# OpenBMB/VisRAG

Measured on AMD Instinct MI355X. Metric: page-images embedded/sec (VisRAG-Ret encode, 448x448, bf16 MFMA) + queries/sec@top-10 over 100k-page index, higher is better.
Workload: dtype bf16; 1 GPU; VisRAG-Ret (SigLIP-so400m 26 blk + resampler + MiniCPM-2B 40 layers) bf16 encode batch=32 page images 448x448 per GPU; index 100000 rows x 2304 sharded 1 way(s), 1000 queries top-10; batch_per_gpu=32, global_batch=32, parallelism=dp1 (pages sharded, no data-path collective)

## Files before the change

include/visrag_hip.h:

```cpp
#ifndef VISRAG_HIP_H
#define VISRAG_HIP_H

#include <stddef.h>
#include <stdint.h>

#ifdef __cplusplus
extern "C" {
#endif

#define VR_OK 0
#define VR_ERR_INVALID 1
#define VR_ERR_HIP 2
#define VR_ERR_STATE 3
#define VR_ERR_CAPACITY 4

#define VR_DTYPE_F32 0
#define VR_DTYPE_BF16 1

typedef struct vr_model_s* vr_model_t;
typedef struct vr_index_s* vr_index_t;

typedef struct vr_config {
    int32_t patch_size;
    int32_t vit_dim;
    int32_t vit_depth;
    int32_t vit_heads;
    int32_t vit_hidden;
    int32_t vit_pos_grid;
    float   vit_ln_eps;
    int32_t query_num;
    float   resampler_ln_eps;
    int32_t hidden_size;
    int32_t num_layers;
    int32_t num_heads;
    int32_t intermediate_size;
    int32_t vocab_size;
    float   rms_norm_eps;
    float   rope_theta;
    float   scale_emb;
    float   residual_scale;
    int32_t max_images;
    int32_t max_patches;
    int32_t max_tokens;
    int32_t max_seqs;
    int32_t text_split_precision;
} vr_config_t;

const char* vr_version(void);
const char* vr_last_error(void);
int vr_device_count(int* count);

int vr_model_create(int device_id, const vr_config_t* cfg, vr_model_t* out);
int vr_model_destroy(vr_model_t m);

int vr_model_load_weight(vr_model_t m, const char* name, const void* data,
                         const int64_t* shape, int32_t ndim, int32_t dtype, int32_t on_device);
int vr_model_finalize(vr_model_t m);
int vr_model_clone(vr_model_t src, vr_model_t* out);

int vr_encode(vr_model_t m,
              const uint8_t* const* slices, const int32_t* slice_hw, int32_t n_slices,
              int32_t slices_on_device,
              const int32_t* input_ids, const int32_t* seq_offsets, int32_t B,
              const int32_t* vision_rows,
              float* out_reps, int32_t out_on_device, void* stream);

int vr_encode_hidden(vr_model_t m,
                     const uint8_t* const* slices, const int32_t* slice_hw, int32_t n_slices,
                     int32_t slices_on_device,
                     const int32_t* input_ids, const int32_t* seq_offsets, int32_t B,
                     const int32_t* vision_rows,
                     float* out_reps, int32_t out_on_device,
                     float* out_hidden, int32_t hidden_len, void* stream);

#define VR_POOL_WMEAN 0
#define VR_POOL_MEAN 1
#define VR_POOL_LASTTOKEN 2
#define VR_POOL_CLS 3
int vr_model_set_pooling(vr_model_t m, int32_t mode);

int vr_model_tap(vr_model_t m, const char* name, float* out, int64_t rows, int64_t cols);
int vr_model_set_taps(vr_model_t m, int32_t enable);

#define VR_PROF_VIT_QKV 0
#define VR_PROF_VIT_ATTN 1
#define VR_PROF_VIT_PROJ 2
#define VR_PROF_VIT_FC1 3
#define VR_PROF_VIT_FC2 4
#define VR_PROF_RESAMPLER 5
#define VR_PROF_DECODER 6
#define VR_PROF_DEC_QKV 7
#define VR_PROF_DEC_ATTN 8
#define VR_PROF_DEC_O 9
#define VR_PROF_DEC_GU 10
#define VR_PROF_DEC_DOWN 11
#define VR_PROF_DEC_NORM 12
#define VR_PROF_CLASSES 13
int vr_model_set_profile(vr_model_t m, int32_t enable);
int vr_model_get_profile(vr_model_t m, int32_t cls, double* total_ms, int64_t* launches,
                         double* total_flops);

typedef struct vr_chat_s* vr_chat_t;
typedef struct vr_chat_config {
    int32_t max_len;
    int32_t max_rows;
    float   dim_model_base;
    int32_t max_slots;
    int32_t max_new;
} vr_chat_config_t;
#define VR_CHAT_GREEDY 0
#define VR_CHAT_BEAM 1
#define VR_CHAT_SAMPLE 2
int vr_chat_create(vr_model_t m, const vr_chat_config_t* cfg, vr_chat_t* out);
int vr_chat_destroy(vr_chat_t ch);
int vr_chat_load_head(vr_chat_t ch, const void* data, const int64_t* shape, int32_t ndim, int32_t dtype, int32_t on_device);
int vr_chat_prefill(vr_chat_t ch, int32_t slot, int32_t row, const uint8_t* const* slices, const int32_t* slice_hw,
                    int32_t n_slices, int32_t slices_on_device, const int32_t* input_ids, int32_t T,
                    const int32_t* vision_rows, void* stream);
int vr_chat_prefill_batch(vr_chat_t ch, int32_t B, const int32_t* slots, const int32_t* rows, const uint8_t* const* slices,
                          const int32_t* slice_hw, int32_t n_slices, int32_t slices_on_device, const int32_t* input_ids,
                          const int32_t* seq_offsets, const int32_t* vision_rows, void* stream);
int vr_chat_step(vr_chat_t ch, int32_t n, const int32_t* slots, const int32_t* rows, const int32_t* tokens, void* stream);
int vr_chat_select(vr_chat_t ch, int32_t mode, int32_t n_groups, const int32_t* group_offsets, const int32_t* rows,
                   const float* beam_scores, int32_t k, float repetition_penalty, float temperature, int32_t top_k,
                   uint64_t seed, int32_t step, float* out_scores, int32_t* out_tokens, int32_t* out_parents, void* stream);
int vr_chat_sample(vr_chat_t ch, int32_t n, const int32_t* rows, float repetition_penalty, float temperature, int32_t top_k,
                   double top_p, uint64_t seed, int32_t step, float* out_scores, int32_t* out_tokens, int32_t* out_kept,
                   int32_t* out_cut, void* stream);
int vr_chat_reorder(vr_chat_t ch, int32_t n, const int32_t* rows, const int32_t* parents, void* stream);
int vr_chat_logits(vr_chat_t ch, int32_t row, float* out, void* stream);
int vr_chat_row_len(vr_chat_t ch, int32_t row, int32_t* slot, int32_t* generated);

int vr_index_create(int device_id, int32_t dim, int64_t capacity, vr_index_t* out);
int vr_index_destroy(vr_index_t ix);
int vr_index_reset(vr_index_t ix);
int vr_index_add(vr_index_t ix, const float* reps, int64_t n, int32_t on_device, void* stream);
int vr_index_size(vr_index_t ix, int64_t* n);
int vr_index_search(vr_index_t ix, const float* queries, int32_t nq, int32_t k,
                    float* out_scores, int64_t* out_ids, int32_t on_device, void* stream);
int vr_index_set_search_eps(vr_index_t ix, float eps_rel);
int vr_index_error_model(vr_index_t ix, float* out4);
int vr_index_search_stats(vr_index_t ix, int64_t* out6, int32_t reset);
int vr_index_search_plan(vr_index_t ix, int32_t nq, int32_t* out5);
int vr_index_set_search_profile(vr_index_t ix, int32_t enable);
int vr_index_get_search_profile(vr_index_t ix, double* ms5, int64_t* calls);
int vr_index_search_keys(vr_index_t ix, const float* queries, int32_t nq, int32_t k, int64_t id_offset,
                         uint64_t* out_keys, int32_t on_device, void* stream);
int vr_index_set_groups(vr_index_t ix, const int64_t* group_offsets, int64_t n_groups);
int vr_index_search_groups(vr_index_t ix, const float* queries, int32_t nq, int32_t k,
                           float* out_scores, int64_t* out_ids, int64_t* out_groups,
                           int32_t on_device, void* stream);
int vr_index_group_search_stats(vr_index_t ix, int64_t* out3, int32_t reset);
int vr_index_set_filters(vr_index_t ix, const uint32_t* bits, int32_t n_filters, int32_t on_device, void* stream);
int vr_index_search_filtered(vr_index_t ix, const float* queries, int32_t nq, int32_t k,
                             const int32_t* filter_of_query,
                             float* out_scores, int64_t* out_ids, int32_t on_device, void* stream);
int vr_index_filter_search_stats(vr_index_t ix, int64_t* out3, int32_t reset);
int vr_index_search_diverse(vr_index_t ix, const float* queries, int32_t nq, int32_t k, int32_t pool, float lambda,
                            const int32_t* filter_of_query ,
                            float* out_scores, int64_t* out_ids, int32_t on_device, void* stream);
int vr_index_search_range(vr_index_t ix, const float* queries, int32_t nq,
                          const float* thresholds,
                          const int32_t* filter_of_query,
                          int64_t max_total,
                          int64_t* out_lims,
                          int64_t* total,
                          int32_t on_device, void* stream);
int vr_index_range_results(vr_index_t ix, float* out_scores, int64_t* out_ids, int64_t n,
                           int32_t on_device, void* stream);
int vr_index_range_search_stats(vr_index_t ix, int64_t* out3, int32_t reset);
int vr_index_rank_rows(vr_index_t ix, const float* queries, int32_t nq,
                       const int64_t* lims,
                       const int64_t* ids,
                       const int32_t* filter_of_query,
                       float* out_scores, int64_t* out_ranks,
                       int32_t on_device, void* stream);
int vr_index_count_range(vr_index_t ix, const float* queries, int32_t nq,
                         const int64_t* lims,
                         const float* thresholds,
                         int32_t strict,
                         const int32_t* filter_of_query,
                         int64_t* out_counts,
                         int32_t on_device, void* stream);
int vr_index_rank_search_stats(vr_index_t ix, int64_t* out3, int32_t reset);
int vr_index_search_window(vr_index_t ix, const float* queries, int32_t nq,
                           const int64_t* offsets,
                           int32_t k,
                           const int32_t* filter_of_query,
                           float* out_scores, int64_t* out_ids,
                           int32_t on_device, void* stream);
int vr_index_window_search_stats(vr_index_t ix, int64_t* out3, int32_t reset);
int vr_index_search_groups_window(vr_index_t ix, const float* queries, int32_t nq,
                                  const int64_t* offsets,
                                  int32_t k,
                                  const int32_t* filter_of_query,
                                  float* out_scores, int64_t* out_ids, int64_t* out_groups,
                                  int32_t on_device, void* stream);
int vr_index_group_window_search_stats(vr_index_t ix, int64_t* out3, int32_t reset);
int vr_index_rank_groups(vr_index_t ix, const float* queries, int32_t nq,
                         const int64_t* lims,
                         const int64_t* groups,
                         const int32_t* filter_of_query,
                         float* out_scores, int64_t* out_rows, int64_t* out_ranks,
                         int32_t on_device, void* stream);
int vr_index_count_groups_range(vr_index_t ix, const float* queries, int32_t nq,
                                const int64_t* lims,
                                const float* thresholds,
                                int32_t strict,
                                const int32_t* filter_of_query,
                                int64_t* out_counts,
                                int32_t on_device, void* stream);
int vr_index_group_rank_search_stats(vr_index_t ix, int64_t* out3, int32_t reset);
int vr_index_search_groups_range(vr_index_t ix, const float* queries, int32_t nq,
                                 const float* thresholds,
                                 const int32_t* filter_of_query,
                                 int64_t max_total,
                                 int64_t* out_lims,
                                 int64_t* total,
                                 int32_t on_device, void* stream);
int vr_index_group_range_results(vr_index_t ix, float* out_scores, int64_t* out_rows, int64_t* out_groups, int64_t n,
                                 int32_t on_device, void* stream);
int vr_index_group_range_search_stats(vr_index_t ix, int64_t* out3, int32_t reset);
int vr_index_search_multi(vr_index_t ix, const float* queries, int32_t n_sub,
                          const int64_t* lims,
                          int32_t n_groups, int32_t k,
                          int32_t fuse,
                          const int32_t* filter_of_group,
                          float* out_scores, int64_t* out_ids, int32_t* out_which,
                          int32_t on_device, void* stream);
int vr_index_multi_search_stats(vr_index_t ix, int64_t* out3, int32_t reset);
int vr_index_search_multi_groups(vr_index_t ix, const float* queries, int32_t n_sub,
                                 const int64_t* lims,
                                 int32_t n_groups, int32_t k,
                                 int32_t fuse,
                                 const int32_t* filter_of_group,
                                 float* out_scores, int64_t* out_rows, int64_t* out_docs, int32_t* out_which,
                                 float* out_ev_scores, int64_t* out_ev_rows,
                                 int32_t on_device, void* stream);
int vr_index_multi_group_search_stats(vr_index_t ix, int64_t* out3, int32_t reset);
int vr_rrf_fuse(int device_id, const int64_t* ids, int32_t n_lists, int32_t depth,
                const int64_t* lims,
                int32_t n_groups, int32_t k, float c,
                const float* weights,
                float* out_scores, int64_t* out_ids, int32_t* out_hits,
                int32_t on_device, void* stream);
int vr_rrf_max_entries(void);
int vr_index_search_rrf(vr_index_t ix, const float* queries, int32_t n_sub,
                        const int64_t* lims,
                        int32_t n_groups, int32_t k, int32_t depth, float c,
                        const float* weights,
                        const int32_t* filter_of_group,
                        int32_t by_groups,
                        float* out_scores, int64_t* out_ids, int32_t* out_hits,
                        int32_t on_device, void* stream);
int vr_index_rrf_search_stats(vr_index_t ix, int64_t* out3, int32_t reset);
int vr_index_remove(vr_index_t ix, const int64_t* ids, int64_t n, int64_t* removed, void* stream);
int vr_index_update(vr_index_t ix, const int64_t* ids, const float* reps, int64_t n, int32_t on_device, void* stream);
int vr_index_get_rows(vr_index_t ix, const int64_t* ids, int64_t n, float* out_f32, uint16_t* out_bf16, int32_t on_device,
                      void* stream);
int vr_topk_merge(int device_id, const float* scores, const int64_t* ids, int32_t n_parts,
                  int32_t nq, int32_t k, float* out_scores, int64_t* out_ids, void* stream);
int vr_topk_merge_keys(int device_id, const uint64_t* keys, int32_t n_parts, int32_t nq, int32_t k,
                       float* out_scores, int64_t* out_ids, void* stream);

int vr_synth_pages(int device_id, uint8_t* out, int32_t n, int32_t size, int64_t seed, int64_t first, void* stream);

int vr_streams_overlap(int device_id, void* stream_a, void* stream_b, int32_t* overlap);

int vr_resize_bicubic(int device_id, const uint8_t* src, int32_t src_on_device, int32_t H, int32_t W,
                      uint8_t* dst, int32_t out_h, int32_t out_w, void* stream);

int vr_op_gemm(int device_id, const void* A, int32_t lda, const void* W, int32_t ldw,
               int32_t M, int32_t N, int32_t K, int32_t epilogue, const float* bias,
               const float* resid, float alpha, void* out, int32_t ldo,
               const int32_t* rope_pos, const float* rope_table, int32_t rope_cols,
               int32_t variant, void* stream);
typedef struct vr_gemm_extras {
    const int32_t* rowmap;
    const float* rowbias;
    int32_t rowbias_period, rowbias_ld, rowbias_cols;
    float col_scale;
    int32_t col_scale_n;
    int32_t ksplit;
    int64_t split_stride;
    const int32_t* m_dev;
    int32_t m_sub;
    int32_t raster_gm;
} vr_gemm_extras_t;
int vr_op_gemm_ex(int device_id, const void* A, int32_t lda, const void* W, int32_t ldw,
                  int32_t M, int32_t N, int32_t K, int32_t epilogue, const float* bias,
                  const float* resid, float alpha, void* out, int32_t ldo,
                  const int32_t* rope_pos, const float* rope_table, int32_t rope_cols,
                  int32_t variant, const vr_gemm_extras_t* extras, void* stream);
int vr_op_gemm_warm(int device_id, const void* A, int32_t lda, const void* W, int32_t ldw,
                    int32_t M, int32_t N, int32_t K, int32_t epilogue, const float* bias,
                    const float* resid, float alpha, void* out, int32_t ldo,
                    const int32_t* rope_pos, const float* rope_table, int32_t rope_cols,
                    int32_t variant, const vr_gemm_extras_t* extras, const void* warm, uint64_t warm_bytes, void* stream);
int vr_op_norm(int device_id, int32_t kind, const float* x, int32_t rows, int32_t dim,
               const float* weight, const float* bias, float eps, void* out, int32_t ldo,
               void* stream);
int vr_op_norm_ex(int device_id, int32_t kind, const float* x, int32_t rows, int32_t dim, int32_t ldx, const float* weight,
                  const float* bias, float eps, void* out, int32_t ldo, void* stream);

int vr_op_text_rmsnorm_split(int device_id, const float* x, int32_t rows, int32_t dim, const float* weight, float eps, void* hi,
                             void* lo, void* stream);
int vr_op_text_rope(int device_id, float* qkv, int32_t T, int32_t ld, int32_t rope_cols, const int32_t* pos, const float* table,
                    void* stream);
int vr_op_text_attention(int device_id, const float* qkv, int32_t ld, int32_t E, const int32_t* seq_offsets, int32_t B, int32_t T,
                         int32_t heads, float scale, float* out, void* stream);
int vr_op_text_swiglu_split(int device_id, const float* gu, int32_t T, int32_t ld_gu, int32_t I, int32_t ld_act, void* hi, void* lo,
                            void* stream);
int vr_op_embed_gather(int device_id, const int32_t* ids, int32_t T, const void* table, const void* table_lo, int32_t dim,
                       float scale, float* out, void* stream);
int vr_op_pool(int device_id, const float* h, const int32_t* seq_offsets, int32_t B, int32_t dim, const float* norm_w, float eps,
               float* out, float* tap, int32_t mode, void* stream);
int vr_op_convert(int device_id, int32_t kind, const void* in, void* out, void* out2, int64_t n, int64_t n_total, int32_t* aux,
                  void* stream);
int vr_op_planes_sum(int device_id, const float* parts, int32_t n_parts, int64_t stride, int32_t ldp, int32_t T, int32_t N,
                     float* out, int32_t ldo, float alpha, int32_t accumulate, void* stream);
int vr_op_patch_embed(int device_id, const void* const* imgs, int32_t n, int32_t H, int32_t W, int32_t P, const float* weight,
                      int32_t D, int32_t K, const float* bias, const float* pos, int32_t ld_pos, float* out, int32_t ldo,
                      void* stream);
int vr_op_attention(int device_id, const void* q, int32_t ldq, const void* k, int32_t ldk,
                    const void* v, int32_t ldv, void* out, int32_t ldo,
                    const int32_t* cu_q, const int32_t* cu_kv, int32_t B, int32_t heads,
                    int32_t head_dim, int32_t max_q, int32_t causal, int32_t q_shared,
                    float scale, void* stream);
typedef struct vr_attn_extras {
    int32_t kv_group;
    const int32_t* kv_end;
    const int32_t* q_in_rows;
    int32_t q_head_stride;
    int32_t q_prescaled;
    float* lse;
} vr_attn_extras_t;
int vr_op_attention_ex(int device_id, const void* q, int32_t ldq, const void* k, int32_t ldk,
                       const void* v, int32_t ldv, void* out, int32_t ldo,
                       const int32_t* cu_q, const int32_t* cu_kv, int32_t B, int32_t heads,
                       int32_t head_dim, int32_t max_q, int32_t causal, int32_t q_shared,
                       float scale, const vr_attn_extras_t* extras, void* stream);
#define VR_ATTN_ROUTE_REFUSED (-1)
#define VR_ATTN_ROUTE_NONE 0
#define VR_ATTN_ROUTE_SMALL 1
#define VR_ATTN_ROUTE_72W 2
#define VR_ATTN_ROUTE_TILED(head_dim, qf, pipe) (100000 + (head_dim) * 100 + (qf) * 10 + (pipe))
int vr_op_attention_route(int device_id, const void* q, int32_t ldq, const void* k, int32_t ldk,
                          const void* v, int32_t ldv, void* out, int32_t ldo,
                          const int32_t* cu_q, const int32_t* cu_kv, int32_t B, int32_t heads,
                          int32_t head_dim, int32_t max_q, int32_t causal, int32_t q_shared,
                          float scale, const vr_attn_extras_t* extras);
int vr_op_attn_combine(int device_id, const void* part, const float* lse, int32_t S, const int32_t* S_dev, int32_t heads,
                       int32_t group, int32_t n_rows, void* out, int32_t ld_out, const void* W, int32_t ldw, int32_t M,
                       int32_t N, int32_t K, int32_t ksplit, int32_t planes, int32_t ldo, int64_t split_stride, void* stream);
int vr_op_gemm_skinny(int device_id, const void* A, int32_t lda, const void* W, int32_t ldw, int32_t M, int32_t N,
                      int32_t K, int32_t ksplit, const float* bias, int32_t swiglu, void* out, int32_t ldo,
                      int64_t split_stride, void* stream);
int vr_op_plane_sum(int device_id, int32_t kind, const float* parts, int32_t nsplit, int64_t split_stride, int32_t ldp,
                    int32_t rows, int32_t dim, float* x, int32_t ldx, float alpha, const float* weight, float eps,
                    void* out, int32_t ldo, void* stream);
int vr_op_chat_attention(int device_id, const void* q, const void* prompt, const void* tails, int32_t layers, int32_t l,
                         int32_t E, int32_t slots, int32_t max_len, int32_t rows, int32_t max_new, int32_t n,
                         const int32_t* step_row, const int32_t* step_slot, const int32_t* step_tail,
                         const int32_t* slot_plen, int32_t force_splits, void* att, void* stream);
int vr_op_chat_select(int device_id, int32_t mode, const float* logits, int32_t ld, int32_t V, const uint32_t* seen,
                      int32_t words, int32_t n_groups, const int32_t* group_offsets, const float* beam_scores, int32_t K,
                      int32_t kout, float repetition_penalty, float temperature, uint64_t seed, int32_t step,
                      float* out_scores, int32_t* out_tokens, int32_t* out_parents, void* stream);
int vr_op_chat_sample(int device_id, const float* logits, int32_t ld, int32_t V, const uint32_t* seen, int32_t words, int32_t n,
                      float repetition_penalty, float temperature, int32_t top_k, double top_p, uint64_t seed, int32_t step,
                      float* out_scores, int32_t* out_tokens, int32_t* out_kept, int32_t* out_cut, void* stream);
int vr_op_chat_prompt_scatter(int device_id, const void* qkv, int32_t ld, int32_t E, int32_t B, const int32_t* seq_offsets,
                              const int32_t* slots, int32_t n_slots, int32_t max_len, void* kplane, void* vplane, void* stream);

int vr_op_gen_mrope_cache(int device_id, const void* src_bf16, const float* parts, int32_t n_parts, int64_t plane_stride,
                          const float* bias, int32_t ld, int32_t T, int32_t H, int32_t KV, const int32_t* pos3, int32_t pos_stride,
                          int32_t sec_t, int32_t sec_h, const float* inv_freq, void* q_out, int32_t ldq, void* k_cache, void* v_cache,
                          int32_t ld_cache, int32_t cache_row0, const int32_t* row0_dev, const int32_t* cache_rows, int32_t* cu_kv,
                          void* stream);
int vr_op_gen_rope2d(int device_id, void* qkv, int32_t ld, int32_t T, int32_t n_slots, int32_t hh, const int32_t* pos_h,
                     const int32_t* pos_w, int32_t sec_h, const float* freq, void* stream);
int vr_op_gen_sample(int device_id, const float* logits, int32_t vocab, uint32_t* seen, float repetition_penalty, float temperature,
                     uint64_t seed, int32_t step, int32_t* state, int32_t step_from_state, int32_t advance, int32_t* out_token,
                     void* stream);
int vr_op_gen_mark_seen(int device_id, const int32_t* ids, int32_t n, uint32_t* seen, int32_t vocab, void* stream);
int vr_op_gen_decode_begin(int device_id, int32_t* state, int32_t q_rows, void* stream);
int vr_op_gen_rows(int device_id, int32_t kind, const float* src, const int32_t* row_idx, int32_t n, int32_t dim, void* dst,
                   int32_t ld, const void* const* pages, const int32_t* page_w, int32_t n_pages, const int32_t* img, const int32_t* ph,
                   const int32_t* pw, int32_t P, int32_t tp, const float* mean3, const float* std3, void* stream);

#ifdef __cplusplus
}
#endif
#endif
```

visrag_amd/_lib.py:

```python
from __future__ import annotations

import ctypes as C
import os
from typing import Optional

_HERE = os.path.dirname(os.path.abspath(__file__))
LIB_PATH = os.path.join(_HERE, "libvisrag_hip.so")

VR_DTYPE_F32, VR_DTYPE_BF16 = 0, 1


class VRConfig(C.Structure):
    _fields_ = [
        ("patch_size", C.c_int32), ("vit_dim", C.c_int32), ("vit_depth", C.c_int32),
        ("vit_heads", C.c_int32), ("vit_hidden", C.c_int32), ("vit_pos_grid", C.c_int32),
        ("vit_ln_eps", C.c_float), ("query_num", C.c_int32), ("resampler_ln_eps", C.c_float),
        ("hidden_size", C.c_int32), ("num_layers", C.c_int32), ("num_heads", C.c_int32),
        ("intermediate_size", C.c_int32), ("vocab_size", C.c_int32), ("rms_norm_eps", C.c_float),
        ("rope_theta", C.c_float), ("scale_emb", C.c_float), ("residual_scale", C.c_float),
        ("max_images", C.c_int32), ("max_patches", C.c_int32), ("max_tokens", C.c_int32),
        ("max_seqs", C.c_int32), ("text_split_precision", C.c_int32),
    ]


class VRChatConfig(C.Structure):
    _fields_ = [("max_len", C.c_int32), ("max_rows", C.c_int32), ("dim_model_base", C.c_float), ("max_slots", C.c_int32),
                ("max_new", C.c_int32)]


class VGConfig(C.Structure):
    _fields_ = [
        ("hidden_size", C.c_int32), ("num_layers", C.c_int32), ("num_heads", C.c_int32), ("num_kv_heads", C.c_int32),
        ("intermediate_size", C.c_int32), ("vocab_size", C.c_int32), ("max_len", C.c_int32), ("max_prefill", C.c_int32),
        ("rms_norm_eps", C.c_float), ("rope_theta", C.c_float), ("mrope_section", C.c_int32 * 3), ("max_seqs", C.c_int32),
    ]


class VGVisionConfig(C.Structure):
    _fields_ = [
        ("depth", C.c_int32), ("hidden_size", C.c_int32), ("num_heads", C.c_int32), ("intermediate_size", C.c_int32),
        ("out_hidden_size", C.c_int32), ("in_channels", C.c_int32), ("patch_size", C.c_int32), ("temporal_patch_size", C.c_int32),
        ("spatial_merge_size", C.c_int32), ("window_size", C.c_int32), ("n_fullatt", C.c_int32), ("fullatt_blocks", C.c_int32 * 16),
        ("max_rows", C.c_int32), ("rms_norm_eps", C.c_float),
    ]


class VRGemmExtras(C.Structure):
    _fields_ = [("rowmap", C.c_void_p), ("rowbias", C.c_void_p), ("rowbias_period", C.c_int32), ("rowbias_ld", C.c_int32),
                ("rowbias_cols", C.c_int32), ("col_scale", C.c_float), ("col_scale_n", C.c_int32), ("ksplit", C.c_int32),
                ("split_stride", C.c_int64), ("m_dev", C.c_void_p), ("m_sub", C.c_int32), ("raster_gm", C.c_int32)]


class VRAttnExtras(C.Structure):
    _fields_ = [("kv_group", C.c_int32), ("kv_end", C.c_void_p), ("q_in_rows", C.c_void_p), ("q_head_stride", C.c_int32),
                ("q_prescaled", C.c_int32), ("lse", C.c_void_p)]


class VisragHipError(RuntimeError):
    pass


_lib: Optional[C.CDLL] = None

_vp, _i32, _i64, _f32 = C.c_void_p, C.c_int32, C.c_int64, C.c_float
SIGNATURES = {
    "vr_version": (C.c_char_p, []),
    "vr_last_error": (C.c_char_p, []),
    "vr_device_count": (C.c_int, [C.POINTER(C.c_int)]),
    "vr_model_create": (C.c_int, [C.c_int, C.POINTER(VRConfig), C.POINTER(_vp)]),
    "vr_model_destroy": (C.c_int, [_vp]),
    "vr_model_load_weight": (C.c_int, [_vp, C.c_char_p, _vp, C.POINTER(_i64), _i32, _i32, _i32]),
    "vr_model_finalize": (C.c_int, [_vp]),
    "vr_model_clone": (C.c_int, [_vp, C.POINTER(C.c_void_p)]),
    "vr_encode": (C.c_int, [_vp, C.POINTER(_vp), C.POINTER(_i32), _i32, _i32, C.POINTER(_i32),
                            C.POINTER(_i32), _i32, C.POINTER(_i32), _vp, _i32, _vp]),
    "vr_encode_hidden": (C.c_int, [_vp, C.POINTER(_vp), C.POINTER(_i32), _i32, _i32, C.POINTER(_i32),
                                   C.POINTER(_i32), _i32, C.POINTER(_i32), _vp, _i32, _vp, _i32, _vp]),
    "vr_model_tap": (C.c_int, [_vp, C.c_char_p, _vp, _i64, _i64]),
    "vr_model_set_taps": (C.c_int, [_vp, _i32]),
    "vr_model_set_pooling": (C.c_int, [_vp, _i32]),
    "vr_model_set_profile": (C.c_int, [_vp, _i32]),
    "vr_model_get_profile": (C.c_int, [_vp, _i32, C.POINTER(C.c_double), C.POINTER(_i64), C.POINTER(C.c_double)]),
    "vr_index_create": (C.c_int, [C.c_int, _i32, _i64, C.POINTER(_vp)]),
    "vr_index_destroy": (C.c_int, [_vp]),
    "vr_index_reset": (C.c_int, [_vp]),
    "vr_index_add": (C.c_int, [_vp, _vp, _i64, _i32, _vp]),
    "vr_index_size": (C.c_int, [_vp, C.POINTER(_i64)]),
    "vr_index_search": (C.c_int, [_vp, _vp, _i32, _i32, _vp, _vp, _i32, _vp]),
    "vr_topk_merge": (C.c_int, [C.c_int, _vp, _vp, _i32, _i32, _i32, _vp, _vp, _vp]),
    "vr_index_set_search_eps": (C.c_int, [_vp, _f32]),
    "vr_index_search_stats": (C.c_int, [_vp, C.POINTER(_i64), _i32]),
    "vr_index_error_model": (C.c_int, [_vp, C.POINTER(_f32)]),
    "vr_index_search_plan": (C.c_int, [_vp, _i32, C.POINTER(_i32)]),
    "vr_synth_pages": (C.c_int, [C.c_int, _vp, _i32, _i32, _i64, _i64, _vp]),
    "vr_streams_overlap": (C.c_int, [C.c_int, _vp, _vp, C.POINTER(C.c_int32)]),
    "vr_index_set_search_profile": (C.c_int, [_vp, _i32]),
    "vr_index_get_search_profile": (C.c_int, [_vp, C.POINTER(C.c_double), C.POINTER(_i64)]),
    "vr_index_search_keys": (C.c_int, [_vp, _vp, _i32, _i32, _i64, _vp, _i32, _vp]),
    "vr_index_set_groups": (C.c_int, [_vp, C.POINTER(_i64), _i64]),
    "vr_index_search_groups": (C.c_int, [_vp, _vp, _i32, _i32, _vp, _vp, _vp, _i32, _vp]),
    "vr_index_group_search_stats": (C.c_int, [_vp, C.POINTER(_i64), _i32]),
    "vr_index_set_filters": (C.c_int, [_vp, _vp, _i32, _i32, _vp]),
    "vr_index_search_filtered": (C.c_int, [_vp, _vp, _i32, _i32, _vp, _vp, _vp, _i32, _vp]),
    "vr_index_filter_search_stats": (C.c_int, [_vp, C.POINTER(_i64), _i32]),
    "vr_index_search_range": (C.c_int, [_vp, _vp, _i32, _vp, _vp, _i64, _vp, C.POINTER(_i64), _i32, _vp]),
    "vr_index_range_results": (C.c_int, [_vp, _vp, _vp, _i64, _i32, _vp]),
    "vr_index_range_search_stats": (C.c_int, [_vp, C.POINTER(_i64), _i32]),
    "vr_index_rank_rows": (C.c_int, [_vp, _vp, _i32, _vp, _vp, _vp, _vp, _vp, _i32, _vp]),
    "vr_index_count_range": (C.c_int, [_vp, _vp, _i32, _vp, _vp, _i32, _vp, _vp, _i32, _vp]),
    "vr_index_rank_search_stats": (C.c_int, [_vp, C.POINTER(_i64), _i32]),
    "vr_index_search_window": (C.c_int, [_vp, _vp, _i32, _vp, _i32, _vp, _vp, _vp, _i32, _vp]),
    "vr_index_window_search_stats": (C.c_int, [_vp, C.POINTER(_i64), _i32]),
    "vr_index_search_groups_window": (C.c_int, [_vp, _vp, _i32, _vp, _i32, _vp, _vp, _vp, _vp, _i32, _vp]),
    "vr_index_group_window_search_stats": (C.c_int, [_vp, C.POINTER(_i64), _i32]),
    "vr_index_rank_groups": (C.c_int, [_vp, _vp, _i32, _vp, _vp, _vp, _vp, _vp, _vp, _i32, _vp]),
    "vr_index_count_groups_range": (C.c_int, [_vp, _vp, _i32, _vp, _vp, _i32, _vp, _vp, _i32, _vp]),
    "vr_index_group_rank_search_stats": (C.c_int, [_vp, C.POINTER(_i64), _i32]),
    "vr_index_search_groups_range": (C.c_int, [_vp, _vp, _i32, _vp, _vp, _i64, _vp, C.POINTER(_i64), _i32, _vp]),
    "vr_index_group_range_results": (C.c_int, [_vp, _vp, _vp, _vp, _i64, _i32, _vp]),
    "vr_index_group_range_search_stats": (C.c_int, [_vp, C.POINTER(_i64), _i32]),
    "vr_index_search_multi": (C.c_int, [_vp, _vp, _i32, _vp, _i32, _i32, _i32, _vp, _vp, _vp, _vp, _i32, _vp]),
    "vr_index_multi_search_stats": (C.c_int, [_vp, C.POINTER(_i64), _i32]),
    "vr_index_search_multi_groups": (C.c_int, [_vp, _vp, _i32, _vp, _i32, _i32, _i32, _vp, _vp, _vp, _vp, _vp, _vp, _vp, _i32, _vp]),
    "vr_index_multi_group_search_stats": (C.c_int, [_vp, C.POINTER(_i64), _i32]),
    "vr_rrf_fuse": (C.c_int, [C.c_int, _vp, _i32, _i32, _vp, _i32, _i32, _f32, _vp, _vp, _vp, _vp, _i32, _vp]),
    "vr_rrf_max_entries": (C.c_int, []),
    "vr_index_search_rrf": (C.c_int, [_vp, _vp, _i32, _vp, _i32, _i32, _i32, _f32, _vp, _vp, _i32, _vp, _vp, _vp, _i32, _vp]),
    "vr_index_rrf_search_stats": (C.c_int, [_vp, C.POINTER(_i64), _i32]),
    "vr_index_search_diverse": (C.c_int, [_vp, _vp, _i32, _i32, _i32, _f32, _vp, _vp, _vp, _i32, _vp]),
    "vr_index_remove": (C.c_int, [_vp, C.POINTER(_i64), _i64, C.POINTER(_i64), _vp]),
    "vr_index_update": (C.c_int, [_vp, C.POINTER(_i64), _vp, _i64, _i32, _vp]),
    "vr_index_get_rows": (C.c_int, [_vp, C.POINTER(_i64), _i64, _vp, _vp, _i32, _vp]),
    "vr_topk_merge_keys": (C.c_int, [C.c_int, _vp, _i32, _i32, _i32, _vp, _vp, _vp]),
    "vr_resize_bicubic": (C.c_int, [C.c_int, _vp, _i32, _i32, _i32, _vp, _i32, _i32, _vp]),
    "vr_op_gemm": (C.c_int, [C.c_int, _vp, _i32, _vp, _i32, _i32, _i32, _i32, _i32, _vp, _vp, _f32,
                             _vp, _i32, _vp, _vp, _i32, _i32, _vp]),
    "vr_op_gemm_ex": (C.c_int, [C.c_int, _vp, _i32, _vp, _i32, _i32, _i32, _i32, _i32, _vp, _vp, _f32,
                                _vp, _i32, _vp, _vp, _i32, _i32, C.POINTER(VRGemmExtras), _vp]),
    "vr_op_gemm_warm": (C.c_int, [C.c_int, _vp, _i32, _vp, _i32, _i32, _i32, _i32, _i32, _vp, _vp, _f32,
                                  _vp, _i32, _vp, _vp, _i32, _i32, C.POINTER(VRGemmExtras), _vp, C.c_uint64, _vp]),
    "vr_op_norm": (C.c_int, [C.c_int, _i32, _vp, _i32, _i32, _vp, _vp, _f32, _vp, _i32, _vp]),
    "vr_op_norm_ex": (C.c_int, [C.c_int, _i32, _vp, _i32, _i32, _i32, _vp, _vp, _f32, _vp, _i32, _vp]),
    "vr_op_text_rmsnorm_split": (C.c_int, [C.c_int, _vp, _i32, _i32, _vp, _f32, _vp, _vp, _vp]),
    "vr_op_text_rope": (C.c_int, [C.c_int, _vp, _i32, _i32, _i32, _vp, _vp, _vp]),
    "vr_op_text_attention": (C.c_int, [C.c_int, _vp, _i32, _i32, _vp, _i32, _i32, _i32, _f32, _vp, _vp]),
    "vr_op_text_swiglu_split": (C.c_int, [C.c_int, _vp, _i32, _i32, _i32, _i32, _vp, _vp, _vp]),
    "vr_op_embed_gather": (C.c_int, [C.c_int, _vp, _i32, _vp, _vp, _i32, _f32, _vp, _vp]),
    "vr_op_pool": (C.c_int, [C.c_int, _vp, _vp, _i32, _i32, _vp, _f32, _vp, _vp, _i32, _vp]),
    "vr_op_convert": (C.c_int, [C.c_int, _i32, _vp, _vp, _vp, _i64, _i64, _vp, _vp]),
    "vr_op_planes_sum": (C.c_int, [C.c_int, _vp, _i32, _i64, _i32, _i32, _i32, _vp, _i32, _f32, _i32, _vp]),
    "vr_op_patch_embed": (C.c_int, [C.c_int, C.POINTER(_vp), _i32, _i32, _i32, _i32, _vp, _i32, _i32, _vp, _vp, _i32, _vp, _i32, _vp]),
    "vr_op_attention": (C.c_int, [C.c_int, _vp, _i32, _vp, _i32, _vp, _i32, _vp, _i32, _vp, _vp, _i32,
                                  _i32, _i32, _i32, _i32, _i32, _f32, _vp]),
    "vr_op_attention_ex": (C.c_int, [C.c_int, _vp, _i32, _vp, _i32, _vp, _i32, _vp, _i32, _vp, _vp, _i32,
                                     _i32, _i32, _i32, _i32, _i32, _f32, C.POINTER(VRAttnExtras), _vp]),
    "vr_op_attention_route": (C.c_int, [C.c_int, _vp, _i32, _vp, _i32, _vp, _i32, _vp, _i32, _vp, _vp, _i32,
                                        _i32, _i32, _i32, _i32, _i32, _f32, C.POINTER(VRAttnExtras)]),
    "vr_op_attn_combine": (C.c_int, [C.c_int, _vp, _vp, _i32, _vp, _i32, _i32, _i32, _vp, _i32, _vp, _i32, _i32, _i32, _i32, _i32,
                                     _i32, _i32, _i64, _vp]),
    "vr_op_gemm_skinny": (C.c_int, [C.c_int, _vp, _i32, _vp, _i32, _i32, _i32, _i32, _i32, _vp, _i32, _vp, _i32, _i64, _vp]),
    "vr_op_plane_sum": (C.c_int, [C.c_int, _i32, _vp, _i32, _i64, _i32, _i32, _i32, _vp, _i32, _f32, _vp, _f32, _vp, _i32, _vp]),
    "vr_op_chat_attention": (C.c_int, [C.c_int, _vp, _vp, _vp, _i32, _i32, _i32, _i32, _i32, _i32, _i32, _i32, C.POINTER(_i32),
                                       C.POINTER(_i32), C.POINTER(_i32), C.POINTER(_i32), _i32, _vp, _vp]),
    "vr_op_chat_select": (C.c_int, [C.c_int, _i32, _vp, _i32, _i32, _vp, _i32, _i32, C.POINTER(_i32), C.POINTER(_f32), _i32, _i32,
                                    _f32, _f32, C.c_uint64, _i32, C.POINTER(_f32), C.POINTER(_i32), C.POINTER(_i32), _vp]),
    "vr_op_chat_sample": (C.c_int, [C.c_int, _vp, _i32, _i32, _vp, _i32, _i32, _f32, _f32, _i32, C.c_double, C.c_uint64, _i32,
                                    C.POINTER(_f32), C.POINTER(_i32), C.POINTER(_i32), C.POINTER(_i32), _vp]),
    "vr_op_chat_prompt_scatter": (C.c_int, [C.c_int, _vp, _i32, _i32, _i32, C.POINTER(_i32), C.POINTER(_i32), _i32, _i32, _vp, _vp, _vp]),
    "vr_op_gen_mrope_cache": (C.c_int, [C.c_int, _vp, _vp, _i32, _i64, _vp, _i32, _i32, _i32, _i32, _vp, _i32, _i32, _i32, _vp, _vp, _i32,
                                        _vp, _vp, _i32, _i32, _vp, _vp, _vp, _vp]),
    "vr_op_gen_rope2d": (C.c_int, [C.c_int, _vp, _i32, _i32, _i32, _i32, _vp, _vp, _i32, _vp, _vp]),
    "vr_op_gen_sample": (C.c_int, [C.c_int, _vp, _i32, _vp, _f32, _f32, C.c_uint64, _i32, _vp, _i32, _i32, C.POINTER(_i32), _vp]),
    "vr_op_gen_mark_seen": (C.c_int, [C.c_int, _vp, _i32, _vp, _i32, _vp]),
    "vr_op_gen_decode_begin": (C.c_int, [C.c_int, _vp, _i32, _vp]),
    "vr_op_gen_rows": (C.c_int, [C.c_int, _i32, _vp, _vp, _i32, _i32, _vp, _i32, C.POINTER(_vp), C.POINTER(_i32), _i32, _vp, _vp, _vp,
                                 _i32, _i32, C.POINTER(_f32), C.POINTER(_f32), _vp]),
    "vr_chat_create": (C.c_int, [_vp, C.POINTER(VRChatConfig), C.POINTER(_vp)]),
    "vr_chat_destroy": (C.c_int, [_vp]),
    "vr_chat_load_head": (C.c_int, [_vp, _vp, C.POINTER(_i64), _i32, _i32, _i32]),
    "vr_chat_prefill": (C.c_int, [_vp, _i32, _i32, C.POINTER(_vp), C.POINTER(_i32), _i32, _i32, C.POINTER(_i32), _i32,
                                  C.POINTER(_i32), _vp]),
    "vr_chat_prefill_batch": (C.c_int, [_vp, _i32, C.POINTER(_i32), C.POINTER(_i32), C.POINTER(_vp), C.POINTER(_i32), _i32, _i32,
                                        C.POINTER(_i32), C.POINTER(_i32), C.POINTER(_i32), _vp]),
    "vr_chat_step": (C.c_int, [_vp, _i32, C.POINTER(_i32), C.POINTER(_i32), C.POINTER(_i32), _vp]),
    "vr_chat_select": (C.c_int, [_vp, _i32, _i32, C.POINTER(_i32), C.POINTER(_i32), C.POINTER(_f32), _i32, _f32, _f32, _i32,
                                 C.c_uint64, _i32, C.POINTER(_f32), C.POINTER(_i32), C.POINTER(_i32), _vp]),
    "vr_chat_sample": (C.c_int, [_vp, _i32, C.POINTER(_i32), _f32, _f32, _i32, C.c_double, C.c_uint64, _i32, C.POINTER(_f32),
                                 C.POINTER(_i32), C.POINTER(_i32), C.POINTER(_i32), _vp]),
    "vr_chat_reorder": (C.c_int, [_vp, _i32, C.POINTER(_i32), C.POINTER(_i32), _vp]),
    "vr_chat_logits": (C.c_int, [_vp, _i32, _vp, _vp]),
    "vr_chat_row_len": (C.c_int, [_vp, _i32, C.POINTER(_i32), C.POINTER(_i32)]),
}
GEN_SIGNATURES = {
    "vg_create": (C.c_int, [C.c_int, C.POINTER(VGConfig), C.POINTER(_vp)]),
    "vg_destroy": (C.c_int, [_vp]),
    "vg_load_weight": (C.c_int, [_vp, C.c_char_p, _vp, C.POINTER(_i64), _i32, _i32, _i32]),
    "vg_finalize": (C.c_int, [_vp]),
    "vg_prefill": (C.c_int, [_vp, _vp, _i32, _vp, _vp, _i32, _vp, _vp]),
    "vg_sample": (C.c_int, [_vp, _f32, _f32, C.c_uint64, _i32, C.POINTER(_i32), _vp]),
    "vg_decode": (C.c_int, [_vp, _i32, C.POINTER(_i32), _vp]),
    "vg_logits": (C.c_int, [_vp, _vp, _vp]),
    "vg_select": (C.c_int, [_vp, _i32]),
    "vg_decode_batch": (C.c_int, [_vp, _i32, C.POINTER(_i32), C.POINTER(_i32), C.POINTER(_i32), _vp]),
    "vg_sample_batch": (C.c_int, [_vp, _i32, C.POINTER(_i32), _f32, _f32, C.c_uint64, _i32, C.POINTER(_i32), _vp]),
    "vg_cache_len": (C.c_int, [_vp, C.POINTER(_i32)]),
    "vg_run_begin": (C.c_int, [_vp, _i32, _f32, _f32, C.c_uint64, _i32, _vp]),
    "vg_run_step": (C.c_int, [_vp]),
    "vg_run_token": (C.c_int, [_vp, _i32, C.POINTER(_i32)]),
    "vg_run_end": (C.c_int, [_vp]),
    "vg_vision_create": (C.c_int, [_vp, C.POINTER(VGVisionConfig)]),
    "vg_vision_encode": (C.c_int, [_vp, _vp, _vp, _i32, _vp, _vp]),
    "vg_vision_encode_pages": (C.c_int, [_vp, C.POINTER(_vp), _i32, C.POINTER(_f32), C.POINTER(_f32), _vp, _i32, _vp, _vp]),
    "vg_vision_plan": (C.c_int, [C.POINTER(VGVisionConfig), _vp, _i32, _vp, _vp, C.POINTER(_i32), _vp]),
}


def load(path: Optional[str] = None) -> C.CDLL:
    global _lib
    if _lib is not None and path is None:
        return _lib
    p = path or os.environ.get("VISRAG_HIP_LIB") or LIB_PATH
    if not os.path.exists(p):
        raise VisragHipError(
            f"{p} not found: the HIP extension is not built. Run `python -m visrag_amd.build` "
            "(or __graft_entry__.build()); there is no CPU fallback.")
    import torch
    lib = C.CDLL(p)
    for name, (res, args) in list(SIGNATURES.items()) + list(GEN_SIGNATURES.items()):
        fn = getattr(lib, name)
        fn.restype = res
        fn.argtypes = args
    if path is None:
        _lib = lib
    return lib


def check(status: int, what: str = "") -> None:
    if status != 0:
        msg = load().vr_last_error()
        raise VisragHipError(f"{what or 'visrag_hip'} failed (status {status}): "
                             f"{msg.decode() if msg else '?'}")


def make_config(cfg, max_images: int, max_patches: int, max_tokens: int, max_seqs: int) -> VRConfig:
    return VRConfig(
        patch_size=cfg.patch_size, vit_dim=cfg.vit_dim, vit_depth=cfg.vit_depth, vit_heads=cfg.vit_heads,
        vit_hidden=cfg.vit_hidden, vit_pos_grid=cfg.vit_pos_grid, vit_ln_eps=cfg.vit_ln_eps,
        query_num=cfg.query_num, resampler_ln_eps=cfg.resampler_ln_eps, hidden_size=cfg.hidden_size,
        num_layers=cfg.num_layers, num_heads=cfg.num_heads, intermediate_size=cfg.intermediate_size,
        vocab_size=cfg.vocab_size, rms_norm_eps=cfg.rms_norm_eps, rope_theta=cfg.rope_theta,
        scale_emb=cfg.scale_emb, residual_scale=cfg.residual_scale, max_images=max_images,
        max_patches=max_patches, max_tokens=max_tokens, max_seqs=max_seqs,
        text_split_precision=int(getattr(cfg, "text_split_precision", True)))
```

visrag_amd/config.py:

```python
from dataclasses import dataclass, asdict
import math


@dataclass
class VisRAGRetConfig:
    patch_size: int = 14
    vit_dim: int = 1152
    vit_depth: int = 26
    vit_heads: int = 16
    vit_mlp_ratio: float = 3.7362
    vit_pos_grid: int = 27
    vit_ln_eps: float = 1e-6
    query_num: int = 64
    resampler_ln_eps: float = 1e-6
    hidden_size: int = 2304
    num_layers: int = 40
    num_heads: int = 36
    intermediate_size: int = 5760
    vocab_size: int = 122753
    rms_norm_eps: float = 1e-5
    rope_theta: float = 10000.0
    scale_emb: float = 12.0
    scale_depth: float = 1.4
    scale_resolution: int = 448
    max_slice_nums: int = 9
    slice_mode: bool = True
    text_split_precision: int = True
    pooling: str = "wmean"

    @property
    def vit_head_dim(self) -> int:
        return self.vit_dim // self.vit_heads

    @property
    def vit_hidden(self) -> int:
        return int(self.vit_dim * self.vit_mlp_ratio)

    @property
    def resampler_heads(self) -> int:
        return self.hidden_size // 128

    @property
    def head_dim(self) -> int:
        return self.hidden_size // self.num_heads

    @property
    def residual_scale(self) -> float:
        return self.scale_depth / math.sqrt(self.num_layers)

    def to_dict(self):
        return asdict(self)

    def flops_vit(self, n_patches: int) -> float:
        N, D, F = n_patches, self.vit_dim, self.vit_hidden
        pe = 2.0 * N * (3 * self.patch_size ** 2) * D
        blk = 2.0 * N * D * 3 * D + 4.0 * N * N * D + 2.0 * N * D * D + 4.0 * N * D * F
        return pe + self.vit_depth * blk

    def flops_resampler(self, n_patches: int) -> float:
        N, D, E, Q = n_patches, self.vit_dim, self.hidden_size, self.query_num
        return 2.0 * N * D * E + 4.0 * N * E * E + 6.0 * Q * E * E + 4.0 * Q * N * E

    def flops_decoder(self, L: int) -> float:
        E, I = self.hidden_size, self.intermediate_size
        return self.num_layers * (L * (8.0 * E * E + 6.0 * E * I) + 4.0 * L * L * E)

    def flops_page(self, n_patches: int = 1024, L: int = 68) -> float:
        return self.flops_vit(n_patches) + self.flops_resampler(n_patches) + self.flops_decoder(L)


def full_config() -> VisRAGRetConfig:
    return VisRAGRetConfig()


def tiny_config() -> VisRAGRetConfig:
    return VisRAGRetConfig(
        vit_dim=288, vit_depth=2, vit_heads=4, vit_pos_grid=6,
        hidden_size=256, num_layers=2, num_heads=4, intermediate_size=640,
        vocab_size=1000, scale_resolution=112,
    )
```

visrag_amd/csrc/attention.hip:

```cpp
#include "attention_body.h"

namespace vr {

template <int HD, int QF, int PIPE>
__global__ __launch_bounds__(256, QF >= 4 ? 1 : (PIPE == 3 ? 3 : 2)) void attention_kernel(AttnArgs p) {
    __shared__ __attribute__((aligned(16))) char smem[attn_smem_bytes<HD, PIPE>()];
    const int q_tiles = (p.max_q + 64 * QF - 1) / (64 * QF);
    attention_body<HD, QF, PIPE>(p, xcd_remap(blockIdx.x, p.B * p.heads * q_tiles), smem);
}

template <int HD, int QF, int PIPE>
static hipError_t launch_t(const AttnArgs& a, hipStream_t s) {
    const int q_tiles = (a.max_q + 64 * QF - 1) / (64 * QF);
    hipLaunchKernelGGL((attention_kernel<HD, QF, PIPE>), dim3(a.B * a.heads * q_tiles), dim3(256), 0, s, a);
    return hipGetLastError();
}

bool attention_small_ok(const AttnArgs& a);
hipError_t launch_attention_small(const AttnArgs& a, hipStream_t s);
bool attention72w_ok(const AttnArgs& a);
hipError_t launch_attention72w(const AttnArgs& a, hipStream_t s);

AttnRoute attention_route(const AttnArgs& a) {
    if (a.B <= 0 || a.max_q <= 0) return {ATTN_ROUTE_NONE, 0, 0, 0};
    if ((a.ldq | a.ldk | a.ldv) % 8 || a.ldo % 4) return {ATTN_ROUTE_REFUSED, 0, 0, 0};
    if (attention_small_ok(a)) return {ATTN_ROUTE_SMALL, 64, 0, 0};
    if (attention72w_ok(a)) return {ATTN_ROUTE_72W, 72, 0, 0};
    const bool big = a.max_q > 64;
    const bool tiny = a.max_q <= 128;
    switch (a.head_dim) {
        case 64: case 72: case 80:
            if (tiny) return {ATTN_ROUTE_TILED, a.head_dim, big ? 2 : 1, 0};
            return {ATTN_ROUTE_TILED, a.head_dim, 2, 3};
        case 128: return {ATTN_ROUTE_TILED, 128, 1, 0};
        default:  return {ATTN_ROUTE_REFUSED, 0, 0, 0};
    }
}

hipError_t launch_attention(const AttnArgs& a_in, hipStream_t s) {
    const AttnRoute r = attention_route(a_in);
    if (r.kind == ATTN_ROUTE_NONE) return hipSuccess;
    if (r.kind == ATTN_ROUTE_REFUSED) return hipErrorInvalidValue;
    AttnArgs a = a_in;
    if (a.q_prescaled && r.kind != ATTN_ROUTE_72W) a.scale = 1.0f / 1.44269504088896340736f;
    if (r.kind == ATTN_ROUTE_SMALL) return launch_attention_small(a, s);
    if (r.kind == ATTN_ROUTE_72W) return launch_attention72w(a, s);
#define VR_TILED(HD_, QF_, PIPE_) \
    if (r.head_dim == HD_ && r.qf == QF_ && r.pipe == PIPE_) return launch_t<HD_, QF_, PIPE_>(a, s);
    VR_TILED(64, 1, 0) VR_TILED(64, 2, 0) VR_TILED(64, 2, 3)
    VR_TILED(72, 1, 0) VR_TILED(72, 2, 0) VR_TILED(72, 2, 3)
    VR_TILED(80, 1, 0) VR_TILED(80, 2, 0) VR_TILED(80, 2, 3)
    VR_TILED(128, 1, 0)
#undef VR_TILED
    return hipErrorInvalidValue;
}

}
```

visrag_amd/csrc/attention_w.hip:

```cpp
#include <type_traits>

#include "common.h"
#include "kernels.h"

namespace vr {

#define AW_FOR_EACH_ACC(X) \
    X(0, "a[0:3]", "a0", "a1", "a2", "a3") \
    X(1, "a[4:7]", "a4", "a5", "a6", "a7") \
    X(2, "a[8:11]", "a8", "a9", "a10", "a11") \
    X(3, "a[12:15]", "a12", "a13", "a14", "a15") \
    X(4, "a[16:19]", "a16", "a17", "a18", "a19") \
    X(5, "a[20:23]", "a20", "a21", "a22", "a23") \
    X(6, "a[24:27]", "a24", "a25", "a26", "a27") \
    X(7, "a[28:31]", "a28", "a29", "a30", "a31") \
    X(8, "a[32:35]", "a32", "a33", "a34", "a35") \
    X(9, "a[36:39]", "a36", "a37", "a38", "a39") \
    X(10, "a[40:43]", "a40", "a41", "a42", "a43") \
    X(11, "a[44:47]", "a44", "a45", "a46", "a47") \
    X(12, "a[48:51]", "a48", "a49", "a50", "a51") \
    X(13, "a[52:55]", "a52", "a53", "a54", "a55") \
    X(14, "a[56:59]", "a56", "a57", "a58", "a59") \
    X(15, "a[60:63]", "a60", "a61", "a62", "a63") \
    X(16, "a[64:67]", "a64", "a65", "a66", "a67") \
    X(17, "a[68:71]", "a68", "a69", "a70", "a71") \
    X(18, "a[72:75]", "a72", "a73", "a74", "a75") \
    X(19, "a[76:79]", "a76", "a77", "a78", "a79")

namespace {

typedef short s16x4 __attribute__((ext_vector_type(4)));

constexpr int AW_HD = 72, AW_PITCH = 160, AW_KV = 64, AW_QT = 256, AW_DF = 5;
constexpr int AW_SLOT = AW_KV * AW_PITCH;
constexpr int AW_NSLOT = 6;
constexpr int AW_VRING = AW_NSLOT * AW_SLOT;
constexpr int AW_SMEM = 2 * AW_NSLOT * AW_SLOT;
constexpr int AW_OPITCH = 144;
constexpr int AW_SMEM_ALL = AW_SMEM + AW_QT * AW_OPITCH;
constexpr int AW_NPIECE = AW_SLOT / 1024;
#ifndef AW_DBG
#define AW_DBG 0
#endif
constexpr float AW_SLACK = 8.0f;

template <int I, int N, class F>
__device__ __forceinline__ void static_for(F&& f) {
    if constexpr (I < N) {
        f(std::integral_constant<int, I>{});
        static_for<I + 1, N>(f);
    }
}

__device__ __forceinline__ void aw_mfma32_first(f32x4& d, const u32x4& a, const bf16x8& b, const f32x4& c) {
    asm volatile("v_mfma_f32_16x16x32_bf16 %0, %1, %2, %3" : "=&v"(d) : "v"(a), "v"(b), "v"(c));
}
__device__ __forceinline__ void aw_mfma32_acc(f32x4& d, const u32x4& a, const bf16x8& b) {
    asm volatile("v_mfma_f32_16x16x32_bf16 %0, %1, %2, %0" : "+v"(d) : "v"(a), "v"(b));
}
__device__ __forceinline__ void aw_mfma16_acc(f32x4& d, const u32x2& a, const s16x4& b) {
    asm volatile("v_mfma_f32_16x16x16_bf16 %0, %1, %2, %0" : "+v"(d) : "v"(a), "v"(b));
}

__device__ __forceinline__ float aw_exp2(float x) { asm volatile("v_exp_f32 %0, %0" : "+v"(x)); return x; }
__device__ __forceinline__ unsigned aw_cvt_pk(float lo, float hi) {
    unsigned r;
    asm volatile("v_cvt_pk_bf16_f32 %0, %1, %2" : "=v"(r) : "v"(lo), "v"(hi));
    return r;
}
__device__ __forceinline__ void aw_max3(float& m, float a, float b, float c) { asm volatile("v_max3_f32 %0, %1, %2, %3" : "=v"(m) : "v"(a), "v"(b), "v"(c)); }
__device__ __forceinline__ void aw_max2(float& m, float a, float b) { asm volatile("v_max_f32 %0, %1, %2" : "=v"(m) : "v"(a), "v"(b)); }

__device__ __forceinline__ float aw_sub_inplace(float x, float d) { asm volatile("v_sub_f32 %0, %0, %1" : "+v"(x) : "v"(d)); return x; }
__device__ __forceinline__ float aw_mask_inplace(float x, int key, int kv_len) {
    asm volatile("v_cmp_le_i32 vcc, %2, %1\n\tv_cndmask_b32 %0, %0, %3, vcc" : "+v"(x) : "v"(key), "s"(kv_len), "v"(-INFINITY) : "vcc");
    return x;
}
__device__ __forceinline__ unsigned aw_scale_pk_inplace(unsigned w, float alpha) {
    unsigned t;
    asm volatile("v_lshlrev_b32 %1, 16, %0\n\tv_and_b32 %0, 0xffff0000, %0\n\tv_mul_f32 %1, %1, %2\n\tv_mul_f32 %0, %0, %2\n\t"
                 "v_cvt_pk_bf16_f32 %0, %1, %0" : "+v"(w), "=&v"(t) : "v"(alpha));
    return w;
}

template <int N>
__device__ __forceinline__ void aw_pv_mfma(const bf16x8& va, const u32x4& pb) {
#define AW_X(n, R, C0, C1, C2, C3) \
    if constexpr (N == n) asm volatile("v_mfma_f32_16x16x32_bf16 " R ", %0, %1, " R : : "v"(va), "v"(pb) : C0, C1, C2, C3);
    AW_FOR_EACH_ACC(AW_X)
#undef AW_X
}
template <int N>
__device__ __forceinline__ void aw_acc_zero() {
#define AW_X(n, R, C0, C1, C2, C3) \
    if constexpr (N == n) asm volatile("v_accvgpr_write_b32 " C0 ", 0\n\tv_accvgpr_write_b32 " C1 ", 0\n\tv_accvgpr_write_b32 " C2 \
                                       ", 0\n\tv_accvgpr_write_b32 " C3 ", 0" : : : C0, C1, C2, C3);
    AW_FOR_EACH_ACC(AW_X)
#undef AW_X
}
template <int N>
__device__ __forceinline__ void aw_acc_read(f32x4& v) {
#define AW_X(n, R, C0, C1, C2, C3) \
    if constexpr (N == n) asm volatile("v_accvgpr_read_b32 %0, " C0 "\n\tv_accvgpr_read_b32 %1, " C1 "\n\tv_accvgpr_read_b32 %2, " C2 \
                                       "\n\tv_accvgpr_read_b32 %3, " C3 : "=v"(v[0]), "=v"(v[1]), "=v"(v[2]), "=v"(v[3]));
    AW_FOR_EACH_ACC(AW_X)
#undef AW_X
}
template <int N>
__device__ __forceinline__ void aw_acc_write(const f32x4& v) {
#define AW_X(n, R, C0, C1, C2, C3) \
    if constexpr (N == n) asm volatile("v_accvgpr_write_b32 " C0 ", %0\n\tv_accvgpr_write_b32 " C1 ", %1\n\tv_accvgpr_write_b32 " C2 \
                                       ", %2\n\tv_accvgpr_write_b32 " C3 ", %3" : : "v"(v[0]), "v"(v[1]), "v"(v[2]), "v"(v[3]) : C0, C1, C2, C3);
    AW_FOR_EACH_ACC(AW_X)
#undef AW_X
}

__device__ __forceinline__ float aw_col4_max(float v) {
    const auto a = __builtin_amdgcn_permlane16_swap(__float_as_uint(v), __float_as_uint(v), false, false);
    v = fmaxf(__uint_as_float(a[0]), __uint_as_float(a[1]));
    const auto b = __builtin_amdgcn_permlane32_swap(__float_as_uint(v), __float_as_uint(v), false, false);
    return fmaxf(__uint_as_float(b[0]), __uint_as_float(b[1]));
}

#define AW_DS_B128(dst, addr, off) asm volatile("ds_read_b128 %0, %1 offset:%2" : "=v"(dst) : "v"(addr), "i"(off))
#define AW_DS_B64(dst, addr, off) asm volatile("ds_read_b64 %0, %1 offset:%2" : "=v"(dst) : "v"(addr), "i"(off))
#define AW_DS_TR(dst, addr, off) asm volatile("ds_read_b64_tr_b16 %0, %1 offset:%2" : "=v"(dst) : "v"(addr), "i"(off))

}

template <int NF, int NW>
__device__ __forceinline__ void attention72w_body(const AttnArgs& p) {
    static_assert(NF * NW == 16 && (NF == 2 || NF == 4), "256 query rows per workgroup");
    constexpr int NS = 11 * NF;
    constexpr int S_TAIL = 4 * NF, S_PV = 6 * NF;
    constexpr int PW = (2 * AW_NPIECE + NW - 1) / NW;
    constexpr int NV = 8 * NF;
    constexpr int S_CHECK = NF == 4 ? S_PV + 3 : S_PV + 2, S_KREAD = NF == 4 ? S_PV + 7 : S_PV + 3;
    static_assert(S_CHECK + NV / 2 <= NS && S_KREAD + 6 <= NS, "schedule fits");
    extern __shared__ __attribute__((aligned(16))) char smem[];
    const int tid = threadIdx.x, lane = tid & 63;
    const int wave = __builtin_amdgcn_readfirstlane(tid >> 6);
    const int fr = lane & 15, fq = lane >> 4;

    const int q_tiles = (p.max_q + AW_QT - 1) / AW_QT;
    const int total = p.B * p.heads * q_tiles;
    const int nwg = gridDim.x;
    const int lw = xcd_remap(blockIdx.x, nwg);
    const float sc = p.scale * 1.44269504088896340736f;
    const unsigned tile_step = (unsigned)(AW_KV * p.ldk) * 2u;
    const unsigned vdelta = (unsigned)((const char*)p.v - (const char*)p.k);

    struct Unit { int u, ok, h, qs, q_len, kv_len, q_row0, kv0, T; };
    auto get_unit = [&](int u) -> Unit {
        Unit x{u, 0, 0, 0, 0, 0, 0, 0, 0};
        if (u >= total) return x;
        const int qt = u % q_tiles, bh = u / q_tiles, b = bh / p.heads;
        x.h = bh % p.heads;
        x.kv0 = p.cu_kv[b]; x.kv_len = p.cu_kv[b + 1] - x.kv0;
        x.q_row0 = p.cu_q[b]; x.q_len = p.cu_q[b + 1] - x.q_row0;
        x.qs = qt * AW_QT;
        x.T = (x.kv_len + AW_KV - 1) / AW_KV;
        x.ok = x.qs < x.q_len && x.kv_len > 0;
        return x;
    };
    auto next_valid = [&](int u) -> Unit {
        Unit x = get_unit(u);
        while (!x.ok && u < total) { u += nwg; x = get_unit(u); }
        return x;
    };
    auto unit_rsrc = [&](const Unit& x) {
        const bf16_t* kb = (const bf16_t*)p.k + (size_t)x.kv0 * p.ldk + x.h * AW_HD;
        return __builtin_amdgcn_make_buffer_rsrc((void*)kb, 0, x.ok ? vdelta + ((x.kv_len - 1) * p.ldv + AW_HD) * 2 : 0, 0x00020000);
    };

    Unit cur = next_valid(lw);
    if (!cur.ok) return;

    unsigned doff[PW];
    int dbase[PW];
    auto doff_reset = [&]() {
#pragma unroll
        for (int i = 0; i < PW; ++i) {
            int j = wave + NW * i;
            if (j >= 2 * AW_NPIECE) j -= 2 * AW_NPIECE;
            const int isv = j >= AW_NPIECE;
            const int c = (j - isv * AW_NPIECE) * 64 + lane;
            const int row = c / 10, ch = c % 10;
            doff[i] = (unsigned)(row * p.ldk + ch * 8) * 2u + (isv ? vdelta : 0u);
            dbase[i] = __builtin_amdgcn_readfirstlane(isv * AW_VRING + (j - isv * AW_NPIECE) * 1024);
        }
    };
    auto ldrsrc = unit_rsrc(cur);
    auto dma_piece = [&](int i, int slot_off) {
        __builtin_amdgcn_raw_ptr_buffer_load_lds(ldrsrc, VR_LDS(smem + dbase[i] + slot_off), 16, doff[i], 0, 0, 0);
        doff[i] += tile_step;
    };
    constexpr int P_LEAD = (PW + 1) / 2;
    int slot_ld = 0;

    u32x4 qraw[NF][2];
    u32x2 qtraw[NF];
    auto q_load = [&](const Unit& x) {
        const bf16_t* qbase = (const bf16_t*)p.q + (size_t)x.q_row0 * p.ldq + x.h * AW_HD;
#pragma unroll
        for (int f = 0; f < NF; ++f) {
            const int q = x.qs + (wave * NF + f) * 16 + fr;
            const bool ok = x.ok && q < x.q_len && !(AW_DBG & 128);
#pragma unroll
            for (int ks = 0; ks < 2; ++ks) {
                qraw[f][ks] = u32x4{0, 0, 0, 0};
                if (ok) qraw[f][ks] = *reinterpret_cast<const u32x4*>(qbase + (size_t)q * p.ldq + ks * 32 + fq * 8);
            }
            qtraw[f] = u32x2{0, 0};
            if (ok && 64 + fq * 4 < AW_HD) qtraw[f] = *reinterpret_cast<const u32x2*>(qbase + (size_t)q * p.ldq + 64 + fq * 4);
        }
    };
    bf16x8 qf[NF][2];
    s16x4 qtail[NF];
    auto q_scale = [&]() {
        if (p.q_prescaled) {
#pragma unroll
            for (int f = 0; f < NF; ++f) {
                qf[f][0] = __builtin_bit_cast(bf16x8, qraw[f][0]); qf[f][1] = __builtin_bit_cast(bf16x8, qraw[f][1]);
                qtail[f] = __builtin_bit_cast(s16x4, qtraw[f]);
            }
            return;
        }
#pragma unroll
        for (int f = 0; f < NF; ++f) {
#pragma unroll
            for (int ks = 0; ks < 2; ++ks) {
                const bf16x8 v = __builtin_bit_cast(bf16x8, qraw[f][ks]);
#pragma unroll
                for (int e = 0; e < 8; ++e) qf[f][ks][e] = f2bf(bf2f(v[e]) * sc);
            }
            const bf16x4 t4 = __builtin_bit_cast(bf16x4, qtraw[f]);
            bf16x4 t;
#pragma unroll
            for (int e = 0; e < 4; ++e) t[e] = f2bf(bf2f(t4[e]) * sc);
            qtail[f] = __builtin_bit_cast(s16x4, t);
        }
    };

    f32x4 negm4[NF];
    f32x4 sA[NF][2], sB[NF][2];
    u32x4 pbA[NF], pbB[NF];

    const unsigned lds0 = (unsigned)(uintptr_t)(__attribute__((address_space(3))) char*)VR_LDS(smem);
    const unsigned k_lane = lds0 + (unsigned)(fr * AW_PITCH + fq * 16);
    const unsigned kt_lane = lds0 + (unsigned)(fr * AW_PITCH + 128 + fq * 8);
    const unsigned v_lane = lds0 + (unsigned)(AW_VRING + (fq * 4 + (fr >> 2)) * AW_PITCH + (fr & 3) * 8);
    const bool row8 = fr == 8;
    int kv_len = cur.kv_len;

#ifdef AW_TIMING
    unsigned long long tm_start = __builtin_amdgcn_s_memtime(), tm_wait = 0, tm_loop0 = 0, tm_loop1 = 0;
    unsigned long long* tmrec = (unsigned long long*)p.lse + ((size_t)cur.u * NW + wave) * 64;
    int tm_nb = 0;
#endif
    u32x4 ka[2][2];
    u32x2 kt[2];
    u32x2 vlo[AW_DF], vhi[AW_DF];
    float mxall = 0.f, mxb = 0.f;

    auto k_read = [&](auto u_c, auto hf_c, unsigned ka_addr, unsigned kta_addr) {
        (void)&ka; (void)&kt;
        constexpr int u = decltype(u_c)::value, hf = decltype(hf_c)::value;
        constexpr int kf = u / 3, pc = u % 3, row = (hf * 2 + kf) * 16 * AW_PITCH;
        if constexpr (pc == 0) AW_DS_B128(ka[kf][0], ka_addr, row);
        else if constexpr (pc == 1) AW_DS_B128(ka[kf][1], ka_addr, row + 64);
        else AW_DS_B64(kt[kf], kta_addr, row);
    };
    auto k_wait = [&]() {
        asm volatile("s_waitcnt lgkmcnt(0)" : "+v"(ka[0][0]), "+v"(ka[0][1]), "+v"(ka[1][0]), "+v"(ka[1][1]), "+v"(kt[0]), "+v"(kt[1]));
    };
    auto v_read = [&](auto u_c, auto hf_c, unsigned v_addr) {
        (void)&vlo; (void)&vhi;
        constexpr int u = decltype(u_c)::value, hf = decltype(hf_c)::value;
        constexpr int d = u / 2, off = hf * 32 * AW_PITCH + d * 32;
        if constexpr ((u & 1) == 0) AW_DS_TR(vlo[d], v_addr, off);
        else AW_DS_TR(vhi[d], v_addr, off + 16 * AW_PITCH);
    };
    auto v_wait = [&]() {
        asm volatile("s_waitcnt lgkmcnt(0)" : "+v"(vlo[0]), "+v"(vhi[0]), "+v"(vlo[1]), "+v"(vhi[1]), "+v"(vlo[2]), "+v"(vhi[2]),
                     "+v"(vlo[3]), "+v"(vhi[3]), "+v"(vlo[4]), "+v"(vhi[4]));
    };

    auto mask_half = [&](f32x4 (&s)[NF][2], int hh) {
        float mx = -INFINITY;
#pragma unroll
        for (int f = 0; f < NF; ++f)
#pragma unroll
            for (int kf = 0; kf < 2; ++kf)
#pragma unroll
                for (int r = 0; r < 4; ++r) {
                    s[f][kf][r] = aw_mask_inplace(s[f][kf][r], hh * 32 + kf * 16 + fq * 4 + r, kv_len);
                    mx = fmaxf(mx, s[f][kf][r]);
                }
        mxall = mx;
    };

    auto raise = [&](f32x4 (&s)[NF][2], u32x4 (&pbn)[NF], auto force_c) {
        constexpr bool force = decltype(force_c)::value;
        if constexpr (!force) asm volatile("s_nop 15\n\ts_nop 15\n\ts_nop 15" ::: "memory");
#pragma unroll
        for (int f = 0; f < NF; ++f) {
            float mx = fmaxf(fmaxf(fmaxf(s[f][0][0], s[f][0][1]), fmaxf(s[f][0][2], s[f][0][3])),
                             fmaxf(fmaxf(s[f][1][0], s[f][1][1]), fmaxf(s[f][1][2], s[f][1][3])));
            mx = aw_col4_max(mx);
// ... 334 lines not shown
```

visrag_amd/csrc/encode.hip:

```cpp
#include <hip/hip_runtime.h>

#include <algorithm>
#include <cmath>
#include <cstring>
#include <vector>

#include "model.h"

static int run_vision_group(vr_model_s* m, const uint8_t* const* dev_imgs_hostarray, int n, int H, int W,
                            const int32_t* rowmap_host , bool first_group, hipStream_t s) {
    const vr_config_t& c = m->c;
    const int P = c.patch_size, gh = H / P, gw = W / P, N = gh * gw;
    const int D = m->D, Dp = m->Dp, E = m->E, Q = m->Q;
    const int M = n * N;
    GridTables* g = nullptr;
    VRCHK(get_grid(m, gh, gw, &g));

    HIPCHK(hipMemcpyAsync(m->w_imgptr.p, dev_imgs_hostarray, (size_t)n * 8, hipMemcpyHostToDevice, s));
    int* cu = (int*)arena_take(m, (size_t)2 * (n + 1) * 4);
    for (int i = 0; i <= n; ++i) { cu[i] = i * N; cu[n + 1 + i] = i * Q; }
    HIPCHK(hipMemcpyAsync(m->w_cu.p, cu, (size_t)2 * (n + 1) * 4, hipMemcpyHostToDevice, s));
    HIPCHK(hipMemcpyAsync(m->w_rowmap.p, rowmap_host, (size_t)n * Q * 4, hipMemcpyHostToDevice, s));
    const int* cu_tok = m->w_cu.as<int>();
    const int* cu_qry = m->w_cu.as<int>() + (n + 1);

    float* h = m->w_hvit.as<float>();
    {
        GemmArgs a = gemm_args(nullptr, 0, m->patch, M, h, Dp);
        a.rowbias = g->vit_pos.as<float>(); a.rowbias_period = N; a.rowbias_ld = Dp; a.rowbias_cols = Dp;
        HIPCHK(launch_patch_embed((const uint8_t* const*)m->w_imgptr.p, n, H, W, P, a, m->Kpe, s));
    }
    if (first_group) VRCHK(tap_store(m, "vit_embed", h, N, D, Dp, false, s));
    const int ldqkv = pad128(3 * D);
    const int vit_hd = c.vit_dim / c.vit_heads;
    const int vit_qscale_n = D % 64 == 0 ? D : 0;
    const float vit_qscale = (1.0f / sqrtf((float)vit_hd)) * 1.44269504088896340736f;
    for (int l = 0; l < c.vit_depth; ++l) {
        const VitBlock& b = m->blocks[l];
        HIPCHK(launch_layernorm(h, M, D, Dp, b.n1w.v.as<float>(), b.n1b.v.as<float>(), c.vit_ln_eps, m->w_xn.p, Dp, s));
        VRCHK(prof_begin(m, VR_PROF_VIT_QKV, s));
        {
            GemmArgs a = gemm_args(m->w_xn.p, Dp, b.qkv, M, m->w_qkv.p, ldqkv);
            a.col_scale = vit_qscale; a.col_scale_n = vit_qscale_n;
            HIPCHK(launch_gemm(a, EPI_BF16, GEMM_VARIANT_AUTO, s));
        }
        VRCHK(prof_end(m, VR_PROF_VIT_QKV, 2.0 * M * D * 3 * D, s));
        {
            AttnArgs a{};
            a.q = m->w_qkv.p; a.ldq = ldqkv;
            a.k = (const char*)m->w_qkv.p + (size_t)D * 2; a.ldk = ldqkv;
            a.v = (const char*)m->w_qkv.p + (size_t)2 * D * 2; a.ldv = ldqkv;
            a.out = m->w_att.p; a.ldo = Dp; a.cu_q = cu_tok; a.cu_kv = cu_tok; a.B = n; a.heads = c.vit_heads;
            a.head_dim = vit_hd; a.max_q = N; a.causal = 0; a.q_shared = 0; a.scale = 1.0f / sqrtf((float)vit_hd); a.q_prescaled = vit_qscale_n > 0;
            VRCHK(prof_begin(m, VR_PROF_VIT_ATTN, s));
            HIPCHK(launch_attention(a, s));
            VRCHK(prof_end(m, VR_PROF_VIT_ATTN, 4.0 * n * (double)N * N * D, s));
        }
        VRCHK(prof_begin(m, VR_PROF_VIT_PROJ, s));
        {
            GemmArgs a = gemm_args(m->w_att.p, Dp, b.proj, M, h, Dp); a.resid = h;
            HIPCHK(launch_gemm(a, EPI_RESID, GEMM_VARIANT_AUTO, s));
        }
        VRCHK(prof_end(m, VR_PROF_VIT_PROJ, 2.0 * M * D * D, s));
        HIPCHK(launch_layernorm(h, M, D, Dp, b.n2w.v.as<float>(), b.n2b.v.as<float>(), c.vit_ln_eps, m->w_xn.p, Dp, s));
        VRCHK(prof_begin(m, VR_PROF_VIT_FC1, s));
        { GemmArgs a = gemm_args(m->w_xn.p, Dp, b.fc1, M, m->w_mlp.p, m->Fp); HIPCHK(launch_gemm(a, EPI_GELU, GEMM_VARIANT_AUTO, s)); }
        VRCHK(prof_end(m, VR_PROF_VIT_FC1, 2.0 * M * D * m->F, s));
        VRCHK(prof_begin(m, VR_PROF_VIT_FC2, s));
        {
            GemmArgs a = gemm_args(m->w_mlp.p, m->Fp, b.fc2, M, h, Dp); a.resid = h;
            HIPCHK(launch_gemm(a, EPI_RESID, GEMM_VARIANT_AUTO, s));
        }
        VRCHK(prof_end(m, VR_PROF_VIT_FC2, 2.0 * M * D * m->F, s));
        if (l == 0 && first_group) VRCHK(tap_store(m, "vit_block0", h, N, D, Dp, false, s));
    }
    HIPCHK(launch_layernorm(h, M, D, Dp, m->vit_nw.v.as<float>(), m->vit_nb.v.as<float>(), c.vit_ln_eps, m->w_xn.p, Dp, s));
    if (first_group) VRCHK(tap_store(m, "vit_out", m->w_xn.p, N, D, Dp, true, s));

    VRCHK(prof_begin(m, VR_PROF_RESAMPLER, s));
    { GemmArgs a = gemm_args(m->w_xn.p, Dp, m->r_kvproj, M, m->w_kv32.p, E); HIPCHK(launch_gemm(a, EPI_F32, GEMM_VARIANT_AUTO, s)); }
    HIPCHK(launch_layernorm(m->w_kv32.as<float>(), M, E, E, m->r_lnkv_w.v.as<float>(), m->r_lnkv_b.v.as<float>(),
                            c.resampler_ln_eps, m->w_xkv.p, E, s));
    {
        GemmArgs a = gemm_args(m->w_xkv.p, E, m->r_kv, M, m->w_KV.p, 2 * E);
        a.rowbias = g->pos_k.as<float>(); a.rowbias_period = N; a.rowbias_ld = E; a.rowbias_cols = E;
        HIPCHK(launch_gemm(a, EPI_BF16, GEMM_VARIANT_AUTO, s));
    }
    {
        AttnArgs a{};
        a.q = m->r_q.p; a.ldq = E; a.k = m->w_KV.p; a.ldk = 2 * E; a.v = (const char*)m->w_KV.p + (size_t)E * 2; a.ldv = 2 * E;
        a.out = m->w_ratt.p; a.ldo = E; a.cu_q = cu_qry; a.cu_kv = cu_tok; a.B = n; a.heads = E / 128; a.head_dim = 128;
        a.max_q = Q; a.causal = 0; a.q_shared = 1; a.scale = 1.0f / sqrtf(128.0f);
        HIPCHK(launch_attention(a, s));
    }
    const int R = n * Q;
    { GemmArgs a = gemm_args(m->w_ratt.p, E, m->r_out, R, m->w_rout.p, E); HIPCHK(launch_gemm(a, EPI_F32, GEMM_VARIANT_AUTO, s)); }
    HIPCHK(launch_layernorm(m->w_rout.as<float>(), R, E, E, m->r_lnpost_w.v.as<float>(), m->r_lnpost_b.v.as<float>(),
                            c.resampler_ln_eps, m->w_rln.p, E, s));
    if (first_group && m->taps_on) {
        GemmArgs a = gemm_args(m->w_rln.p, E, m->r_proj, Q, m->w_rout.p, E);
        HIPCHK(launch_gemm(a, EPI_F32, GEMM_VARIANT_AUTO, s));
        VRCHK(tap_store(m, "resampler_out", m->w_rout.p, Q, E, E, false, s));
    }
    {
        GemmArgs a = gemm_args(m->w_rln.p, E, m->r_proj, R, m->w_h.p, E);
        a.rowmap = m->w_rowmap.as<int>();
        HIPCHK(launch_gemm(a, EPI_F32, GEMM_VARIANT_AUTO, s));
    }
    VRCHK(prof_end(m, VR_PROF_RESAMPLER, 2.0 * M * D * E + 4.0 * M * E * (double)E + 4.0 * R * (double)N * E + 4.0 * R * E * (double)E, s));
    return VR_OK;
}

static int hp_gemm_tiles(vr_model_s* m, const void* a_hi, const void* a_lo, const Linear& L, const Linear& Llo, int lda, int T, float* out,
                         int ldo, bool into_resid, float alpha, hipStream_t s) {
    const size_t plane = (size_t)T * L.n_pad;
    const int n_planes = Llo.has_w ? 3 : 2;
    if (!L.has_b && (const char*)a_lo == (const char*)a_hi + (size_t)T * lda * 2 && m->w_hp_planes.reserve((size_t)n_planes * plane * 4) == VR_OK) {
        float* part = m->w_hp_planes.as<float>();
        {
            GemmArgs a = gemm_args(a_hi, lda, L, 2 * T, part, L.n_pad);
            a.bias = nullptr;
            HIPCHK(launch_gemm(a, EPI_F32, GEMM_VARIANT_AUTO, s));
        }
        if (Llo.has_w) {
            GemmArgs a = gemm_args(a_hi, lda, Llo, T, part + 2 * plane, L.n_pad);
            a.bias = nullptr;
            HIPCHK(launch_gemm(a, EPI_F32, GEMM_VARIANT_AUTO, s));
        }
        HIPCHK(launch_planes_sum(part, n_planes, plane, L.n_pad, T, std::min(L.n_pad, ldo), out, ldo, into_resid ? alpha : 1.0f, into_resid, s));
        return VR_OK;
    }
    {
        GemmArgs a = gemm_args(a_hi, lda, L, T, out, ldo);
        if (into_resid) { a.resid = out; a.alpha = alpha; }
        HIPCHK(launch_gemm(a, into_resid ? EPI_RESID : EPI_F32, GEMM_VARIANT_AUTO, s));
    }
    {
        GemmArgs a = gemm_args(a_lo, lda, L, T, out, ldo);
        a.bias = nullptr;
        a.resid = out; a.alpha = into_resid ? alpha : 1.0f;
        HIPCHK(launch_gemm(a, EPI_RESID, GEMM_VARIANT_AUTO, s));
    }
    if (Llo.has_w) {
        GemmArgs a = gemm_args(a_hi, lda, Llo, T, out, ldo);
        a.bias = nullptr;
        a.resid = out; a.alpha = into_resid ? alpha : 1.0f;
        HIPCHK(launch_gemm(a, EPI_RESID, GEMM_VARIANT_AUTO, s));
    }
    return VR_OK;
}

static int hp_gemm_stream(vr_model_s* m, const void* a_hi, const void* a_lo, const Linear& L, const Linear& Llo, int lda, int T, float* out,
                          int ldo, bool into_resid, float alpha, hipStream_t s) {
    const int ks = stream_ksplit(L.n_pad, L.k_pad);
    const size_t plane = (size_t)T * L.n_pad;
    const int n_pass = Llo.has_w ? 3 : 2;
    if ((size_t)n_pass * ks * plane * 4 > m->w_hp_part.bytes) return fail(VR_ERR_CAPACITY, "split-K planes exceed the workspace");
    float* part = m->w_hp_part.as<float>();
    for (int pass = 0; pass < n_pass; ++pass) {
        GemmArgs a = gemm_args(pass == 1 ? a_lo : a_hi, lda, pass == 2 ? Llo : L, T, part + (size_t)pass * ks * plane, L.n_pad);
        a.bias = nullptr;
        a.ksplit = ks; a.split_stride = plane;
        HIPCHK(launch_gemm_skinny(a, s));
    }
    HIPCHK(launch_planes_sum(part, n_pass * ks, plane, L.n_pad, T, std::min(L.n_pad, ldo), out, ldo, into_resid ? alpha : 1.0f, into_resid, s));
    return VR_OK;
}
static bool hp_stream_ok(const vr_model_s* m, int T) {
    if (T > 32) return false;
    for (const DecLayer& L : m->layers)
        for (const Linear* l : {&L.qkv, &L.o, &L.gu, &L.down})
            if (l->n_pad % 256 || l->k_pad % 64 || l->has_b) return false;
    return true;
}

static int run_decoder_hp(vr_model_s* m, int T, int B, int max_len, hipStream_t s) {
    (void)max_len;
    const vr_config_t& c = m->c;
    const int E = m->E, I = m->I, Ip = m->Ip;
    float* h = m->w_h.as<float>();
    float* qkv = m->w_hp_qkv.as<float>();
    float* att = m->w_hp_att.as<float>();
    float* gu = m->w_hp_gu.as<float>();
    const int ld_gu = pad128(2 * I);
    HIPCHK(launch_seq_of(m->w_seq.as<int>(), B, m->w_seqof.as<int>(), s));
    const bool stream = hp_stream_ok(m, T);
    void* const hi = m->w_hp_hi.p;
    auto lo = [&](int lda) -> void* { return (char*)hi + (size_t)T * lda * 2; };
    auto hp_gemm = [&](vr_model_s* mm, const Linear& L, const Linear& Llo, int lda, int TT, float* out, int ldo, bool into_resid,
                       float alpha, hipStream_t ss) -> int {
        return stream ? hp_gemm_stream(mm, hi, lo(lda), L, Llo, lda, TT, out, ldo, into_resid, alpha, ss)
                      : hp_gemm_tiles(mm, hi, lo(lda), L, Llo, lda, TT, out, ldo, into_resid, alpha, ss);
    };
    for (int l = 0; l < c.num_layers; ++l) {
        const DecLayer& L = m->layers[l];
        HIPCHK(launch_rmsnorm_split(h, T, E, L.ln1.v.as<float>(), c.rms_norm_eps, hi, lo(E), s));
        VRCHK(hp_gemm(m, L.qkv, L.qkv_lo, E, T, qkv, 3 * E, false, 1.0f, s));
        HIPCHK(launch_rope_f32(qkv, T, 3 * E, 2 * E, m->w_pos.as<int>(), m->rope.as<float>(), s));
        HIPCHK(launch_attn_f32(qkv, 3 * E, E, m->w_seqof.as<int>(), m->w_seq.as<int>(), T, c.num_heads, 1.0f / sqrtf(64.0f), att, s));
        HIPCHK(launch_split_bf16(att, hi, lo(E), (size_t)T * E, s));
        VRCHK(hp_gemm(m, L.o, L.o_lo, E, T, h, E, true, c.residual_scale, s));
        HIPCHK(launch_rmsnorm_split(h, T, E, L.ln2.v.as<float>(), c.rms_norm_eps, hi, lo(E), s));
        VRCHK(hp_gemm(m, L.gu, L.gu_lo, E, T, gu, ld_gu, false, 1.0f, s));
        HIPCHK(launch_swiglu_split(gu, T, ld_gu, I, Ip, hi, lo(Ip), s));
        VRCHK(hp_gemm(m, L.down, L.down_lo, Ip, T, h, E, true, c.residual_scale, s));
        if (l == 0) VRCHK(tap_store(m, "dec_layer0", h, T, E, E, false, s));
    }
    return VR_OK;
}


struct DecRoute { int ks; int proj_variant; bool proj_128w; };
static DecRoute dec_route(int T, int E, int Ip, bool taps_on) {
    DecRoute r{1, GEMM_VARIANT_256W, false};
    const long t192 = (long)((T + 255) / 256) * (E / 192);
    if (E % 192 == 0 && t192 * 2 <= 256 && t192 * 2 > 160 && E % 128 == 0 && Ip % 128 == 0) {
        r.ks = 2;
        r.proj_variant = GEMM_VARIANT_192W;
    } else {
        const long tiles = (long)((T + 255) / 256) * ((E + 255) / 256);
        for (int cand = DEC_KSPLIT_MAX; cand > 1; --cand)
            if (tiles * cand <= 256 && E % (cand * 64) == 0 && Ip % (cand * 64) == 0) { r.ks = cand; break; }
    }
    if (taps_on) r.ks = 1;
    const long t128 = (long)((T + 127) / 128) * (E / 192);
    r.proj_128w = E % 192 == 0 && t128 > 128 && t128 <= 256;
    if (r.proj_128w) r.ks = 1;
    return r;
}

extern "C" int vr_encode(vr_model_t m, const uint8_t* const* slices, const int32_t* slice_hw, int32_t n_slices,
                         int32_t slices_on_device, const int32_t* input_ids, const int32_t* seq_offsets, int32_t B,
                         const int32_t* vision_rows, float* out_reps, int32_t out_on_device, void* stream) {
    if (!m) return fail(VR_ERR_INVALID, "NULL model");
    m->arena_open = false;
    const int rc = encode_impl(m, slices, slice_hw, n_slices, slices_on_device, input_ids, seq_offsets, B, vision_rows,
                               out_reps, out_on_device, stream);
    arena_close(m, stream);
// ... 222 lines not shown
```

visrag_amd/csrc/gemm.hip:

```cpp
#include "gemm_core.h"
#include "gemm_core_il.h"
#include "kernels.h"
#include "gemm_epilogue.h"

namespace vr {

template <int EPI>
__global__ __launch_bounds__(256) void gemm_bf16_kernel(GemmArgs p) {
    extern __shared__ __attribute__((aligned(16))) char smem[];
    const int tiles_n = p.N / GEMM_BN;
    const int tiles_m = (p.M + GEMM_BM - 1) / GEMM_BM;
    const int t = xcd_remap(blockIdx.x, tiles_m * tiles_n);
    const int GM = p.raster_gm > 0 ? p.raster_gm : 1;
    const int gsz = GM * tiles_n;
    const int g = t / gsz, r = t % gsz;
    const int gm = min(GM, tiles_m - g * GM);
    const int m0 = (g * GM + r % gm) * GEMM_BM, n0 = (r / gm) * GEMM_BN;

    gemm_acc_t acc;
    gemm_zero(acc);
    gemm_mainloop(acc, (const bf16_t*)p.A, p.lda, (const bf16_t*)p.W, p.ldw, m0, n0, p.K, smem);

    const int lane = threadIdx.x & 63, wave = threadIdx.x >> 6;
    const int wm = wave >> 1, wn = wave & 1;
    if constexpr (EPI == EPI_RESID) {
        if (!p.rowmap) { gemm_epilogue_resid_tile<4, 4, 4>(acc, p, m0 + wm * 64 + (lane & 15), n0 + wn * 64, lane >> 4); return; }
    }
    if constexpr (EPI == EPI_BF16 || EPI == EPI_GELU || EPI == EPI_SWIGLU || EPI == EPI_ROPE) {
        if ((p.N & 7) == 0 && (p.ldo & 7) == 0) {
            gemm_epilogue_tile_lds<EPI, 4>(acc, p, m0 + wm * 64, n0 + wn * 64, lane, smem + wave * 8192);
            return;
        }
    }
#pragma unroll
    for (int i = 0; i < 4; ++i)
        gemm_epilogue_row<EPI>(acc[i], p, m0 + wm * 64 + i * 16 + (lane & 15), n0 + wn * 64, lane >> 4);
}

template <int EPI>
__global__ __launch_bounds__(512, 2) void gemm256_bf16_kernel(GemmArgs p) {
    extern __shared__ __attribute__((aligned(16))) char smem[];
    const int tiles_n = (p.N + G256_BN - 1) / G256_BN;
    const int tiles_m = (p.M + G256_BM - 1) / G256_BM;
    const int ks = p.ksplit > 1 ? p.ksplit : 1;
    const int tt = xcd_remap(blockIdx.x, tiles_m * tiles_n * ks);
    const int split = tt / (tiles_m * tiles_n);
    const int t = tt - split * (tiles_m * tiles_n);
    const int GM = p.raster_gm > 0 ? p.raster_gm : 1;
    const int gsz = GM * tiles_n;
    const int g = t / gsz, r = t % gsz;
    const int gm = min(GM, tiles_m - g * GM);
    const int m0 = (g * GM + r % gm) * G256_BM, n0 = (r / gm) * G256_BN;
    if (p.m_dev && m0 >= p.m_dev[0] - p.m_sub) return;

    gemm256_acc_t acc;
    gemm256_zero(acc);
    const int Ks = p.K / ks;
    const bf16_t* Ap = (const bf16_t*)p.A + (size_t)split * Ks;
    const bf16_t* Wp = (const bf16_t*)p.W + (size_t)split * Ks;
    gemm256_mainloop_il(acc, Ap, p.lda, Wp, p.ldw, m0, n0, Ks, smem);

    if constexpr (EPI == EPI_F32) {
        if (ks > 1) {
            GemmArgs ps = p;
            ps.out = (float*)p.out + (size_t)split * p.split_stride;
            if (split > 0) ps.bias = nullptr;
            const int lane = threadIdx.x & 63, wave = threadIdx.x >> 6;
#pragma unroll
            for (int i = 0; i < 8; ++i)
                gemm_epilogue_row<EPI_F32>(acc[i], ps, m0 + (wave >> 2) * 128 + i * 16 + (lane & 15), n0 + (wave & 3) * 64, lane >> 4);
            return;
        }
    }

    const int lane = threadIdx.x & 63, wave = threadIdx.x >> 6;
    const int wm = wave >> 2, wn = wave & 3;
    if constexpr (EPI == EPI_RESID) {
        if (!p.rowmap) { gemm_epilogue_resid_tile<8, 4, 4>(acc, p, m0 + wm * 128 + (lane & 15), n0 + wn * 64, lane >> 4); return; }
    }
    if constexpr (EPI == EPI_BF16 || EPI == EPI_GELU || EPI == EPI_SWIGLU || EPI == EPI_ROPE) {
        if ((p.N & 7) == 0 && (p.ldo & 7) == 0) {
            gemm_epilogue_tile_lds<EPI, 8>(acc, p, m0 + wm * 128, n0 + wn * 64, lane, smem + wave * 16384);
            return;
        }
    }
#pragma unroll
    for (int i = 0; i < 8; ++i)
        gemm_epilogue_row<EPI>(acc[i], p, m0 + wm * 128 + i * 16 + (lane & 15), n0 + wn * 64, lane >> 4);
}

template <int EPI>
static hipError_t launch_epi(const GemmArgs& a_in, int variant, hipStream_t s) {
    GemmArgs a = a_in;
    if (variant == GEMM_VARIANT_256IL) {
        const int tn = (a.N + G256_BN - 1) / G256_BN, tm = (a.M + G256_BM - 1) / G256_BM;
        if (a.raster_gm <= 0) a.raster_gm = tm <= 16 ? tm : 4;
        auto k = gemm256_bf16_kernel<EPI>;
        static unsigned long long attr = 0;
        set_max_dynamic_lds((const void*)k, G256_SMEM_BYTES, attr);
        int grid = tn * tm;
        if (a.ksplit > 1) grid *= a.ksplit;
        hipLaunchKernelGGL(k, dim3(grid), dim3(512), G256_SMEM_BYTES, s, a);
        return hipGetLastError();
    }
    if (variant != GEMM_VARIANT_GLDS) return hipErrorInvalidValue;
    const int tiles = (a.N / GEMM_BN) * ((a.M + GEMM_BM - 1) / GEMM_BM);
    if (a.raster_gm <= 0) {
        const int tm = (a.M + GEMM_BM - 1) / GEMM_BM;
        a.raster_gm = tm <= 32 ? tm : 4;
    }
    auto k = gemm_bf16_kernel<EPI>;
    static unsigned long long attr = 0;
    set_max_dynamic_lds((const void*)k, GEMM_SMEM_BYTES, attr);
    hipLaunchKernelGGL(k, dim3(tiles), dim3(256), GEMM_SMEM_BYTES, s, a);
    return hipGetLastError();
}

bool gemm_args_refused(const GemmArgs& a, int epi, int variant) {
    if (a.col_scale_n != 0 && (epi != EPI_BF16 || a.col_scale_n < 0 || a.col_scale_n % 64 != 0)) return true;
    const bool half_tile = variant == GEMM_VARIANT_128W_192 || variant == GEMM_VARIANT_128W_256;
    const bool split_tile = variant == GEMM_VARIANT_256IL || variant == GEMM_VARIANT_256W || variant == GEMM_VARIANT_192W;
    if (half_tile && (a.rowmap || a.rowbias)) return true;
    if (a.rowbias && ((epi != EPI_BF16 && epi != EPI_GELU && epi != EPI_F32) || a.rowbias_period < 1)) return true;
    if (a.ksplit > 1 && (!split_tile || epi != EPI_F32 || a.K % (a.ksplit * GEMM_BK) || a.rowmap || a.rowbias)) return true;
    if (a.m_dev && variant != GEMM_VARIANT_256IL) return true;
    if (a.warm && a.warm_bytes && (variant != GEMM_VARIANT_256W || a.warm_bytes >= WARM_MAX_BYTES)) return true;
    return false;
}

int gemm_auto_variant(const GemmArgs& a, int epi) {
    if (a.N % 192 == 0 && a.N % 256 != 0 && a.N <= 1536 && a.M >= 4096 && epi <= EPI_RESID) {
        if (epi == EPI_RESID && !a.rowmap && gemm256w_fits(a, 192)) return GEMM_VARIANT_192W;
        return GEMM_VARIANT_192;
    }
    const bool n_ok = (a.N % 256 == 0) || a.N >= 2048;
    const long t256 = (long)((a.N + 255) / 256) * ((a.M + 255) / 256);
    const long t128 = (long)(a.N / 128) * ((a.M + 127) / 128);
    const double e256 = 1.45 * (double)t256 / (double)(((t256 + 255) / 256) * 256);
    const double e128 = (double)t128 / (double)(((t128 + 511) / 512) * 512);
    const bool w_ok = gemm256w_fits(a, 256);
    return (n_ok && e256 > e128) ? (w_ok ? GEMM_VARIANT_256W : GEMM_VARIANT_256IL) : GEMM_VARIANT_GLDS;
}

hipError_t launch_gemm(const GemmArgs& a, int epi, int variant, hipStream_t s) {
    if (a.M <= 0) return hipSuccess;
    if (variant == GEMM_VARIANT_AUTO) variant = gemm_auto_variant(a, epi);
    if (variant == GEMM_VARIANT_192) return launch_gemm192(a, epi, s);
    if (variant == GEMM_VARIANT_256W) return launch_gemm256w(a, epi, s);
    if (variant == GEMM_VARIANT_192W) return launch_gemm192w(a, epi, s);
    if (variant == GEMM_VARIANT_128W_192) return launch_gemm128w(a, epi, 192, s);
    if (variant == GEMM_VARIANT_128W_256) return launch_gemm128w(a, epi, 256, s);
    if (gemm_args_refused(a, epi, variant)) return hipErrorInvalidValue;
    switch (epi) {
        case EPI_BF16: return launch_epi<EPI_BF16>(a, variant, s);
        case EPI_GELU: return launch_epi<EPI_GELU>(a, variant, s);
        case EPI_F32: return launch_epi<EPI_F32>(a, variant, s);
        case EPI_RESID: return launch_epi<EPI_RESID>(a, variant, s);
        case EPI_SWIGLU: return launch_epi<EPI_SWIGLU>(a, variant, s);
        case EPI_ROPE: return launch_epi<EPI_ROPE>(a, variant, s);
        default: return hipErrorInvalidValue;
    }
}

}
```

visrag_amd/csrc/gemm256w_kernel.h:

```cpp
W_KERNEL_TEMPLATE
__global__ __launch_bounds__(256) __attribute__((amdgpu_waves_per_eu(1, 1))) void W_KERNEL_NAME(GemmArgs p) {
    static_assert(NJ == 8 || (NJ == 6 && !PLAIN), "wave tile 128 x 128 or 128 x 96");
    constexpr int BN = 32 * NJ;
    constexpr int NS = 8 * NJ;
    constexpr int NR = 8 + NJ;
    constexpr int DS = NJ == 8 ? 5 : 4;
    constexpr int SB1 = NS * 5 / 8;
    constexpr int D1 = (NS - 1 - (SB1 + 2)) / DS + 1;
    constexpr int SB2 = NJ;
    constexpr int NF = NJ / 2;
    static_assert(SB2 + 3 + DS * (NR - D1 - 1) < NS && SB2 + 2 + 2 * (NR - 1) < NS && 2 * NR - 2 < SB1, "schedule fits");
    extern __shared__ __attribute__((aligned(16))) char smem[];
#ifdef VR_W_TIMING
    const unsigned long long tm0 = __builtin_amdgcn_s_memrealtime();
    unsigned long long tm1 = 0, tm2 = 0, cy1 = 0, cy2 = 0;
#endif
    const int tiles_n = (p.N + BN - 1) / BN;
    const int tiles_m = (p.M + G256_BM - 1) / G256_BM;
    const int ks = p.ksplit > 1 ? p.ksplit : 1;
    const int total = tiles_m * tiles_n * ks;
    const int Ks = p.K / ks;
    const int nk = Ks / GEMM_BK;

    const int my_first = xcd_remap(blockIdx.x, total);
    const int GM = p.raster_gm > 0 ? p.raster_gm : 1;
    auto coords = [&](int tt, int& m0, int& n0, int& split) {
        split = tt / (tiles_m * tiles_n);
        const int t = tt - split * (tiles_m * tiles_n);
        const int gsz = GM * tiles_n;
        const int g = t / gsz, r = t % gsz;
        const int gm = min(GM, tiles_m - g * GM);
        m0 = __builtin_amdgcn_readfirstlane((g * GM + r % gm) * G256_BM);
        n0 = __builtin_amdgcn_readfirstlane((r / gm) * BN);
        split = __builtin_amdgcn_readfirstlane(split);
    };

    const int lane = threadIdx.x & 63, wave = __builtin_amdgcn_readfirstlane(threadIdx.x >> 6);
    const int wm = wave >> 1, wn = wave & 1, fr = lane & 15, fq = lane >> 4;

    const auto arsrc = __builtin_amdgcn_make_buffer_rsrc((void*)p.A, 0, 0x7FFFFFFF, 0x00020000);
    const auto wrsrc = __builtin_amdgcn_make_buffer_rsrc((void*)p.W, 0, 0x7FFFFFFF, 0x00020000);
    const unsigned lchunk = (unsigned)(((lane & 7) ^ (lane >> 3)) << 4);
    const unsigned lofA = (unsigned)(lane >> 3) * (unsigned)p.lda * 2u + lchunk;
    const unsigned lofW = (unsigned)(lane >> 3) * (unsigned)p.ldw * 2u + lchunk;
    const unsigned rgA = (unsigned)p.lda * 16u, rgW = (unsigned)p.ldw * 16u;
    const unsigned sA0 = (unsigned)wave * 8u * rgA, sW0 = (unsigned)wave * (unsigned)NJ * rgW;
    char* const dmaA = smem + wave * 8192;
    char* const dmaW = smem + G256_TILE_BYTES + wave * (NJ * 1024);
    auto tile_off_a = [&](int m0, int split) { return ((unsigned)m0 * (unsigned)p.lda + (unsigned)split * (unsigned)Ks) * 2u; };
    auto tile_off_w = [&](int n0, int split) { return ((unsigned)n0 * (unsigned)p.ldw + (unsigned)split * (unsigned)Ks) * 2u; };

    auto dma = [&](int stage, int d, unsigned vA, unsigned vW) {
        if (d < 8) __builtin_amdgcn_raw_ptr_buffer_load_lds(arsrc, VR_LDS(dmaA + stage * W_STAGE + d * 1024), 16, vA, sA0 + d * rgA, 0, 0);
        else __builtin_amdgcn_raw_ptr_buffer_load_lds(wrsrc, VR_LDS(dmaW + stage * W_STAGE + (d - 8) * 1024), 16, vW, sW0 + (d - 8) * rgW, 0, 0);
    };

    typedef const __attribute__((address_space(3))) bf16x8* frag_p;
    frag_p pA[2][2], pW[2][2];
#pragma unroll
    for (int st = 0; st < 2; ++st)
#pragma unroll
        for (int kk = 0; kk < 2; ++kk) {
            const int ch = ((kk * 4 + fq) ^ (fr & 7)) << 4;
            pA[st][kk] = (frag_p)VR_LDS(smem + st * W_STAGE + (wm * 128 + fr) * 128 + ch);
            pW[st][kk] = (frag_p)VR_LDS(smem + st * W_STAGE + G256_TILE_BYTES + (wn * 16 * NJ + fr) * 128 + ch);
            asm volatile("" : "+v"(pA[st][kk]), "+v"(pW[st][kk]));
        }

    bf16x8 a0[8], w0[NJ], a1[8], w1[NJ];
    int m0, n0, split;
    coords(my_first, m0, n0, split);
    unsigned curA = tile_off_a(m0, split), curW = tile_off_w(n0, split);
    unsigned warm_lo = 0, warm_hi = 0;

    {
        const unsigned k1 = nk > 1 ? (unsigned)(GEMM_BK * 2) : W_OOB;
#pragma unroll
        for (int d = 0; d < NR; ++d) dma(0, d, lofA + curA, lofW + curW);
#pragma unroll
        for (int d = 0; d < NR; ++d) dma(1, d, lofA + curA + k1, lofW + curW + k1);
        if constexpr (NJ == 8) {
            if (p.warm && p.warm_bytes) {
                const WarmShare sh = warm_share(p.warm_bytes, (unsigned)my_first, (unsigned)total, (unsigned)wave);
                warm_lo = (unsigned)__builtin_amdgcn_readfirstlane((int)sh.first);
                warm_hi = (unsigned)__builtin_amdgcn_readfirstlane((int)sh.end);
            }
        }
        W_FOR_EACH_ACC(W_ZERO)
        if constexpr (NJ == 8) VR_WAIT_VM_BARRIER(16); else VR_WAIT_VM_BARRIER(14);
#pragma unroll
        for (int j = 0; j < NJ; ++j) w0[j] = pW[0][0][j * 128];
#pragma unroll
        for (int i = 0; i < 8; ++i) a0[i] = pA[0][0][i * 128];
    }
#ifdef VR_W_TIMING
    asm volatile("s_waitcnt lgkmcnt(0)" ::: "memory");
    tm1 = __builtin_amdgcn_s_memrealtime();
    cy1 = __builtin_amdgcn_s_memtime();
#endif

    {
        const unsigned nxtA = W_OOB, nxtW = W_OOB;

        auto step = [&](auto stage_c, int kt) {
            constexpr int S = decltype(stage_c)::value;
            const int k2 = kt + 2;
            const unsigned vA = lofA + (k2 < nk ? curA + (unsigned)k2 * (GEMM_BK * 2) : nxtA + (unsigned)(k2 - nk) * (GEMM_BK * 2));
            const unsigned vW = lofW + (k2 < nk ? curW + (unsigned)k2 * (GEMM_BK * 2) : nxtW + (unsigned)(k2 - nk) * (GEMM_BK * 2));
            __builtin_amdgcn_sched_barrier(0);
            auto aux1 = [&](int sl) {
                if (sl < 2 * NR && (sl & 1) == 0) {
                    const int q = sl >> 1;
                    if (q < NJ) w1[q] = pW[S][1][q * 128];
                    else a1[q - NJ] = pA[S][1][(q - NJ) * 128];
                }
                if (sl == SB1) asm volatile("s_waitcnt lgkmcnt(0)\n\ts_barrier" ::: "memory");
                if (sl >= SB1 + 2 && (sl - (SB1 + 2)) % DS == 0) dma(S, (sl - (SB1 + 2)) / DS, vA, vW);
                __builtin_amdgcn_sched_barrier(0);
            };
            auto aux2 = [&](int sl) {
                if (sl == SB2) { if constexpr (D1 == 5) VR_WAIT_VM_BARRIER(5); else VR_WAIT_VM_BARRIER(4); }
                if (sl >= SB2 + 3 && (sl - (SB2 + 3)) % DS == 0 && D1 + (sl - (SB2 + 3)) / DS < NR)
                    dma(S, D1 + (sl - (SB2 + 3)) / DS, vA, vW);
                if (sl >= SB2 + 2 && sl < SB2 + 2 + 2 * NR && ((sl - SB2) & 1) == 0) {
                    const int q = (sl - (SB2 + 2)) >> 1;
                    if (q < NJ) w0[q] = pW[S ^ 1][0][q * 128];
                    else a0[q - NJ] = pA[S ^ 1][0][(q - NJ) * 128];
                }
                __builtin_amdgcn_sched_barrier(0);
            };
#define W_P1(n, R, C0, C1, C2, C3) \
            if (((n) & 7) < NJ) { W_MFMA(R, C0, C1, C2, C3, w0[(n) & 7], a0[(n) >> 3]); aux1(((n) >> 3) * NJ + ((n) & 7)); }
#define W_P2(n, R, C0, C1, C2, C3) \
            if (((n) & 7) < NJ) { W_MFMA(R, C0, C1, C2, C3, w1[(n) & 7], a1[(n) >> 3]); aux2(((n) >> 3) * NJ + ((n) & 7)); }
            W_FOR_EACH_ACC(W_P1)
            W_FOR_EACH_ACC(W_P2)
#undef W_P1
#undef W_P2
        };

        for (int kt = 0; kt < nk; kt += 2) {
            step(std::integral_constant<int, 0>{}, kt);
            if (kt + 1 >= nk) break;
            step(std::integral_constant<int, 1>{}, kt + 1);
        }
        asm volatile("s_nop 15\n\ts_nop 15" ::: "memory");
#ifdef VR_W_TIMING
        tm2 = __builtin_amdgcn_s_memrealtime();
        cy2 = __builtin_amdgcn_s_memtime();
#endif

        const int mrow0 = m0 + wm * 128, nb0 = n0 + wn * (16 * NJ);
        char* const wl0 = smem + 2 * W_STAGE + wave * W_STAGING;
        bool plain_resid = false;
        if constexpr (EPI == EPI_RESID) plain_resid = !p.rowmap;
        auto uni32 = [](unsigned v) { return (unsigned)__builtin_amdgcn_readfirstlane((int)v); };
        auto uni_ptr = [&](const void* q) {
            const unsigned long long a = (unsigned long long)q;
            return (void*)(((unsigned long long)uni32((unsigned)(a >> 32)) << 32) | uni32((unsigned)a));
        };
        auto warm_requests = [&]() {
            if constexpr (NJ == 8) {
                if (warm_lo < warm_hi) {
                    const unsigned long long wa = (unsigned long long)uni_ptr(p.warm);
                    const auto wrs = __builtin_amdgcn_make_buffer_rsrc((void*)wa, 0, uni32((unsigned)p.warm_bytes), 0x00020000);
                    const unsigned pad = (0u - (unsigned)wa) & 3u;
                    char* const dump = smem + 2 * W_STAGE + 4 * W_STAGING + wave * W_WARM_DUMP;
                    auto request = [&](unsigned l) {
                        const unsigned line = l + (unsigned)lane;
                        __builtin_amdgcn_raw_ptr_buffer_load_lds(wrs, VR_LDS(dump), 4, line < warm_hi ? line * WARM_LINE + pad : W_OOB, 0, 0, 0);
                    };
                    __builtin_amdgcn_sched_barrier(0);
                    request(warm_lo);
                    request(warm_lo + 64);
                    __builtin_amdgcn_sched_barrier(0);
#pragma nounroll
                    for (unsigned l = warm_lo + 128; l < warm_hi; l += 64) request(l);
                }
            }
        };
        bool buf_tile = false;
        if constexpr (EPI == EPI_RESID) buf_tile = plain_resid && n0 + BN <= p.N;
        if constexpr (EPI == EPI_F32) buf_tile = !p.rowmap && !p.rowbias && n0 + BN <= p.N;
        if constexpr (EPI == EPI_RESID || EPI == EPI_F32) {
            if (buf_tile) {
// ... 233 lines not shown
```

visrag_amd/csrc/kernels.h:

```cpp
#pragma once
#include <hip/hip_runtime.h>
#include <stdint.h>

#include "gemm_warm.h"

namespace vr {

enum GemmEpilogue { EPI_BF16 = 0, EPI_GELU = 1, EPI_F32 = 2, EPI_RESID = 3, EPI_SWIGLU = 4, EPI_ROPE = 5 };
enum GemmVariant { GEMM_VARIANT_GLDS = 0, GEMM_VARIANT_AUTO = 3, GEMM_VARIANT_192 = 7, GEMM_VARIANT_256IL = 9, GEMM_VARIANT_256W = 12,
                   GEMM_VARIANT_192W = 13, GEMM_VARIANT_128W_192 = 14, GEMM_VARIANT_128W_256 = 15 };

struct GemmArgs {
    const void* A; int lda;
    const void* W; int ldw;
    int M, N, K;
    const float* bias;
    const float* resid;
    float alpha;
    void* out; int ldo;
    const int* rowmap;
    const float* rowbias;
    int rowbias_period, rowbias_ld, rowbias_cols;
    const int* rope_pos;
    const float* rope_table;
    int rope_cols;
    int raster_gm;
    int ksplit;
    size_t split_stride;
    float col_scale; int col_scale_n;
    const int* m_dev; int m_sub;
    const void* warm; size_t warm_bytes;
};
hipError_t launch_gemm(const GemmArgs& a, int epilogue, int variant, hipStream_t s);
bool gemm_args_refused(const GemmArgs& a, int epilogue, int variant);
int gemm_auto_variant(const GemmArgs& a, int epilogue);
hipError_t launch_gemm192(const GemmArgs& a, int epilogue, hipStream_t s);
hipError_t launch_gemm256w(const GemmArgs& a, int epilogue, hipStream_t s);
bool gemm256w_fits(const GemmArgs& a, int tile_cols);
hipError_t launch_gemm192w(const GemmArgs& a, int epilogue, hipStream_t s);
hipError_t launch_gemm128w(const GemmArgs& a, int epilogue, int tile_cols, hipStream_t s);
bool gemm128w_fits(const GemmArgs& a, int tile_cols);

struct SkinnyCombine { const void* part; const float* lse; int S; int heads; int group; const int* S_dev; };
hipError_t launch_gemm_skinny(const GemmArgs& a, hipStream_t s, bool swiglu = false, const struct SkinnyCombine* combine = nullptr);
hipError_t launch_swiglu_sum(const float* parts, int n_parts, size_t plane_stride, int ldp, int M, int I, void* act, int lda,
                             hipStream_t s);

hipError_t launch_layernorm(const float* x, int rows, int dim, int ldx, const float* w, const float* b,
                            float eps, void* out, int ldo, hipStream_t s);
hipError_t launch_rmsnorm_accum(float* x, int rows, int dim, int ldx, const float* partial, int nsplit,
                                size_t split_stride, int ldp, float alpha, const float* w, float eps, void* out,
                                int ldo, hipStream_t s);
hipError_t launch_rmsnorm(const float* x, int rows, int dim, int ldx, const float* w, float eps,
                          void* out, int ldo, hipStream_t s);

struct AttnArgs {
    const void* q; int ldq;
    const void* k; int ldk;
    const void* v; int ldv;
    void* out; int ldo;
    const int* cu_q;
    const int* cu_kv;
    int B, heads, head_dim, max_q;
    int causal, q_shared;
    float scale;
    int kv_group;
    const int* kv_end;
    const int* q_in_rows;
    int q_head_stride;
    int q_prescaled;
    float* lse;
};
hipError_t launch_attention(const AttnArgs& a, hipStream_t s);
enum AttnRouteKind { ATTN_ROUTE_REFUSED = -1, ATTN_ROUTE_NONE = 0, ATTN_ROUTE_SMALL = 1, ATTN_ROUTE_72W = 2, ATTN_ROUTE_TILED = 3 };
struct AttnRoute { int kind, head_dim, qf, pipe; };
AttnRoute attention_route(const AttnArgs& a);

constexpr int CHAT_MAX_ROWS = 16;
constexpr int CHAT_ATT_SPLITS = 8;
constexpr int CHAT_KEYS = 256;
constexpr int CHAT_SEL_WGS = 64;
constexpr int CHAT_TOPK_MAX = 64;
enum ChatSelMode { CHAT_SEL_GREEDY = 0, CHAT_SEL_BEAM = 1, CHAT_SEL_SAMPLE = 2 };
struct ChatStep {
    int n, groups;
    int row[CHAT_MAX_ROWS], slot[CHAT_MAX_ROWS], tail[CHAT_MAX_ROWS], pos[CHAT_MAX_ROWS], token[CHAT_MAX_ROWS];
    int g_lo[CHAT_MAX_ROWS + 1], plen[CHAT_MAX_ROWS];
    int gsplit[CHAT_MAX_ROWS], rsplit[CHAT_MAX_ROWS];
};
struct ChatCaps { int slots, len, rows, tail; };
struct ChatMove { int n; int src[CHAT_MAX_ROWS], dst[CHAT_MAX_ROWS], len[CHAT_MAX_ROWS]; };
struct ChatSel {
    int n, groups;
    int lrow[CHAT_MAX_ROWS], srow[CHAT_MAX_ROWS], g_lo[CHAT_MAX_ROWS + 1];
    float bscore[CHAT_MAX_ROWS];
};
int chat_step_groups(ChatStep& st, const int* slot_plen, int max_slots, int force_splits = 0);
hipError_t launch_chat_embed(const ChatStep& st, const void* table, int E, float scale, float* h, unsigned* seen, int words, hipStream_t s);
hipError_t launch_chat_qkv(const ChatStep& st, const float* parts, int n_parts, size_t plane, int ldp, const float* rope, int E, int heads,
                           void* q_out, void* tails, int l, int max_rows, int max_new, hipStream_t s);
hipError_t launch_chat_attn(const ChatStep& st, const void* q, const void* prompt, const void* tails, int l, int E, int heads,
                            const ChatCaps& cap, int S_max, float* po, float* pml, void* att, hipStream_t s);
hipError_t launch_chat_prompt_kv(const void* qkv, int ld, int T, int E, void* kdst, void* vdst, hipStream_t s);
struct ChatBatch { int n; int off[CHAT_MAX_ROWS + 1], idx[CHAT_MAX_ROWS]; };
hipError_t launch_chat_prompt_scatter(const ChatBatch& bt, const void* qkv, int ld, int E, int max_len, void* kplane, void* vplane,
                                      hipStream_t s);
hipError_t launch_chat_last_rows(const ChatBatch& bt, const float* h, int E, const float* w, float eps, void* out, hipStream_t s);
hipError_t launch_chat_move(const ChatMove& mv, void* tails, void* scratch, int layers, int max_rows, int max_new, int E, int max_tail,
                            unsigned* seen, unsigned* seen_scratch, int words, hipStream_t s);
hipError_t launch_chat_select(const ChatSel& sel, int mode, const float* logits, int ld, int V, const unsigned* seen, int words, float pen,
                              float temperature, int K, int kout, unsigned long long seed, unsigned step, float* lse,
                              unsigned long long* part, float* o_score, int* o_tok, int* o_par, hipStream_t s);
hipError_t launch_chat_sample(const ChatSel& sel, const float* logits, int ld, int V, const unsigned* seen, int words, float pen,
                              float temperature, int top_k, double top_p, unsigned long long seed, unsigned step, float* o_score,
                              int* o_tok, int* o_kept, int* o_cut, hipStream_t s);

constexpr int GEN_ATT_SPLITS = 16;
struct GenState {
    int token;
    int pos[3];
    int len;
    int step;
    int splits;
    int pad;
    int cu_q[GEN_ATT_SPLITS + 1], cu_kv[GEN_ATT_SPLITS + 1];
};
struct KvSplit { int splits, chunk; };
__host__ __device__ inline KvSplit gen_kv_split(int L) {
    int splits = min(GEN_ATT_SPLITS, max(1, (L + 127) / 128));
    const int chunk = ((L + splits - 1) / splits + 63) / 64 * 64;
    splits = (L + chunk - 1) / chunk;
    return KvSplit{splits, chunk};
}
struct GenBatch {
    int token[16];
    int pos[3][16];
    int cache_row[16];
    int splits[16];
    int cu_q[16 * GEN_ATT_SPLITS + 1];
    int kv_lo[16 * GEN_ATT_SPLITS], kv_hi[16 * GEN_ATT_SPLITS];
    int q_in[16 * GEN_ATT_SPLITS];
    int sampled[16];
};
hipError_t launch_decode_begin(GenState* st, int q_rows, hipStream_t s);
hipError_t launch_mrope_cache(const void* src_bf16, const float* parts, int n_parts, size_t plane_stride, const float* bias,
                              int ld, int T, int H, int KV, const int* pos3, int pos_stride, int sec_t, int sec_h,
                              const float* inv_freq, void* q_out, int ldq, void* k_cache, void* v_cache, int ld_cache,
                              int cache_row0, int* cu_kv, hipStream_t s, const int* row0_dev = nullptr,
                              const int* cache_rows = nullptr);
hipError_t launch_rope2d_table(const int* pos_h, const int* pos_w, int T, int sec_h, const float* freq, void* cs, hipStream_t s);
hipError_t launch_rope2d_inplace(void* qkv, int ld, int T, int n_slots, int hh, const void* cs, hipStream_t s);
hipError_t launch_mark_seen(const int* ids, int n, unsigned* seen, int vocab, hipStream_t s);
hipError_t launch_sample(const float* logits, int vocab, unsigned* seen, float penalty, float temperature,
                         unsigned long long seed, unsigned step, int* token_out, unsigned long long* scratch64, hipStream_t s,
                         GenState* st = nullptr, int step_from_state = 0, int advance = 0);
hipError_t launch_scatter_rows(const float* src, const int* row_idx, int n, int dim, float* dst, int ld, hipStream_t s);
hipError_t launch_gather_rows_bf16(const float* src, const int* row_idx, int n, int dim, void* dst, int ld, hipStream_t s);
hipError_t launch_patch_rows_u8(const uint8_t* const* pages, const int* page_w, const int* img, const int* ph, const int* pw, int n,
                                int P, int tp, const float* mean3, const float* std3, void* dst, int ld, hipStream_t s);
hipError_t launch_attn_combine(const void* part, const float* lse, int S, int heads, int group, void* out, hipStream_t s,
                               const int* S_dev = nullptr,
                               int n_rows = 1, int ld_out = 0);

hipError_t launch_patch_embed(const uint8_t* const* imgs, int n_imgs, int H, int W, int P, const GemmArgs& g, int Kreal,
                              hipStream_t s);
hipError_t launch_embed_gather(const int* ids, int T, const void* table, int dim, float scale,
                               float* out, hipStream_t s);
hipError_t launch_pool(const float* h, const int* seq_offsets, int B, int dim, const float* norm_w,
                       float eps, float* out, float* tap_hidden, hipStream_t s, int mode = 0);
hipError_t launch_f32_to_bf16(const float* in, void* out, size_t n, hipStream_t s);
hipError_t launch_f32_to_bf16_pad(const float* in, void* out, size_t n, size_t n_total, hipStream_t s,
                                  int* zero_word = nullptr);
hipError_t launch_split_bf16(const float* in, void* hi, void* lo, size_t n, hipStream_t s);
hipError_t launch_iota_pos(const int* seq_offsets, int B, int* pos, hipStream_t s);
hipError_t launch_any_nonzero16(const void* p, size_t n, int* flag, hipStream_t s);

hipError_t launch_rmsnorm_split(const float* x, int rows, int dim, const float* w, float eps, void* hi, void* lo, hipStream_t s);
hipError_t launch_rope_f32(float* qkv, int T, int ld, int rope_cols, const int* pos, const float* table, hipStream_t s);
hipError_t launch_attn_f32(const float* qkv, int ld, int E, const int* seq_of, const int* seq_offsets, int T, int heads,
                           float scale, float* out, hipStream_t s);
hipError_t launch_swiglu_split(const float* gu, int T, int ld_gu, int I, int ld_act, void* hi, void* lo, hipStream_t s);
hipError_t launch_embed_gather_hp(const int* ids, int T, const void* table_hi, const void* table_lo, int dim, float scale,
                                  float* out, hipStream_t s);
hipError_t launch_seq_of(const int* seq_offsets, int B, int* seq_of, hipStream_t s);
hipError_t launch_planes_sum(const float* parts, int n_parts, size_t stride, int ldp, int T, int N, float* out, int ldo, float alpha,
                             bool accumulate, hipStream_t s);

hipError_t launch_synth_pages(uint8_t* out, int n, int size, long long seed, long long first, hipStream_t s);

}
#include <vector>
namespace vr {
int resize_coeffs(int in_size, int out_size, std::vector<int>& bounds, std::vector<int>& kk);
hipError_t launch_resize_h(const uint8_t* in, int in_w, int rows, uint8_t* out, int out_w, const int* bounds,
                           const int* kk, int ksize, hipStream_t s);
hipError_t launch_resize_v(const uint8_t* in, int w, uint8_t* out, int out_h, const int* bounds, const int* kk,
                           int ksize, hipStream_t s);

struct SearchArgs {
    const void* index_bf16;
    const float* index_f32;
    int64_t n_docs;
    int dim;
    const void* q_bf16;
    int convert_q;
    const float* q_f32;
    int nq, k;
    float* cand_scores; int* cand_ids; int n_chunks;
    float* out_scores; int64_t* out_ids;
    float* thr_init;
    int pre_own_chunks;
    float* thr_cert;
    unsigned long long* cand_keys;
    float* score_rows; size_t ld_scores;
    int exact_follows;
    int* huge_seen;
    const float* thr_used;
    float eps_rel;
    int eps_data;
    float acc_rel;
    const float* dmax;
    int* flag_count; int* flag_list;
    float* flag_tau;
    void* flag_q;
// ... 238 lines not shown
```

visrag_amd/csrc/model.hip:

```cpp
#include <hip/hip_runtime.h>

#include <algorithm>
#include <cmath>
#include <cstdio>
#include <cstring>

#include "model.h"

extern "C" const char* vr_version(void) { return "visrag_hip 0.1.0 (gfx950)"; }
extern "C" const char* vr_last_error(void) { return g_err.c_str(); }
extern "C" int vr_device_count(int* count) {
    if (!count) return fail(VR_ERR_INVALID, "count is NULL");
    HIPCHK(hipGetDeviceCount(count));
    return VR_OK;
}

extern "C" int vr_model_create(int device_id, const vr_config_t* cfg, vr_model_t* out) {
    if (!cfg || !out) return fail(VR_ERR_INVALID, "cfg/out is NULL");
    const vr_config_t& c = *cfg;
    if (c.vit_dim % c.vit_heads || c.vit_dim / c.vit_heads != 72)
        return fail(VR_ERR_INVALID, "ViT head_dim must be 72 (vit_dim %d / heads %d)", c.vit_dim, c.vit_heads);
    if (c.hidden_size % 128) return fail(VR_ERR_INVALID, "hidden_size %d must be a multiple of 128", c.hidden_size);
    if (c.hidden_size % c.num_heads || c.hidden_size / c.num_heads != 64)
        return fail(VR_ERR_INVALID, "decoder head_dim must be 64");
    if (c.intermediate_size % 64) return fail(VR_ERR_INVALID, "intermediate_size must be a multiple of 64");
    if (c.query_num != 64) return fail(VR_ERR_INVALID, "query_num must be 64");
    if (c.vit_dim % 4 || c.hidden_size > 2560 || c.vit_dim > 2560) return fail(VR_ERR_INVALID, "dims out of range");
    if (c.max_images <= 0 || c.max_patches <= 0 || c.max_tokens <= 0 || c.max_seqs <= 0)
        return fail(VR_ERR_INVALID, "workspace limits must be positive");
    VRCHK(set_dev(device_id));
    vr_model_s* m = new vr_model_s();
    m->device = device_id;
    m->c = c;
    m->D = c.vit_dim; m->Dp = pad128(c.vit_dim);
    m->F = c.vit_hidden; m->Fp = pad128(c.vit_hidden);
    m->E = c.hidden_size; m->I = c.intermediate_size; m->Ip = pad128(c.intermediate_size);
    m->Kpe = 3 * c.patch_size * c.patch_size; m->Kpe_p = pad128(m->Kpe);
    m->Q = c.query_num;
    m->blocks.resize(c.vit_depth);
    m->layers.resize(c.num_layers);
    *out = m;
    return VR_OK;
}

extern "C" int vr_model_destroy(vr_model_t m) {
    if (!m) return VR_OK;
    (void)hipSetDevice(m->device);
    (void)hipDeviceSynchronize();
    if (!m->borrowed) {
        auto fl = [](Linear& l) { l.w.free(); l.b.free(); };
        fl(m->patch); fl(m->r_kvproj); fl(m->r_kv); fl(m->r_out); fl(m->r_proj);
        for (auto& b : m->blocks) {
            fl(b.qkv); fl(b.proj); fl(b.fc1); fl(b.fc2); b.n1w.v.free(); b.n1b.v.free(); b.n2w.v.free(); b.n2b.v.free();
        }
        for (auto& l : m->layers) { fl(l.qkv); fl(l.o); fl(l.gu); fl(l.down); fl(l.qkv_lo); fl(l.o_lo); fl(l.gu_lo); fl(l.down_lo); l.ln1.v.free(); l.ln2.v.free(); }
        for (Vec* v : {&m->vit_nw, &m->vit_nb, &m->r_lnq_w, &m->r_lnq_b, &m->r_lnkv_w, &m->r_lnkv_b, &m->r_lnpost_w, &m->r_lnpost_b, &m->final_norm}) v->v.free();
        for (DevBuf* b : {&m->r_q, &m->embed, &m->embed_lo, &m->rope}) b->free();
    }
    for (auto& g : m->grids) { g.second.vit_pos.free(); g.second.pos_k.free(); }
    for (auto& pc : m->prof) for (hipEvent_t e : pc.ev) (void)hipEventDestroy(e);
    if (m->arena) (void)hipHostFree(m->arena);
    if (m->arena_ev) (void)hipEventDestroy(m->arena_ev);
    for (DevBuf* b : {&m->w_hvit, &m->w_xn, &m->w_qkv, &m->w_att, &m->w_mlp,
                      &m->w_kv32, &m->w_xkv, &m->w_KV, &m->w_ratt, &m->w_rout, &m->w_rln, &m->w_h, &m->w_dxn, &m->w_part, &m->w_dqkv,
                      &m->w_datt, &m->w_dact, &m->w_cu, &m->w_ids, &m->w_seq, &m->w_pos, &m->w_rowmap, &m->w_imgptr,
                      &m->w_pix, &m->w_out, &m->w_hp_hi, &m->w_hp_planes, &m->w_hp_qkv, &m->w_hp_att, &m->w_hp_gu, &m->w_seqof, &m->w_hp_part, &m->w_hidden})
        b->free();
    delete m;
    return VR_OK;
}

extern "C" int vr_model_load_weight(vr_model_t m, const char* name_c, const void* data, const int64_t* shape,
                                    int32_t ndim, int32_t dtype, int32_t on_device) {
    if (!m || !name_c || !data || !shape) return fail(VR_ERR_INVALID, "NULL argument");
    if (dtype != VR_DTYPE_F32 && dtype != VR_DTYPE_BF16) return fail(VR_ERR_INVALID, "bad dtype %d", dtype);
    VRCHK(set_dev(m->device));
    const std::string name(name_c);
    const int bf = dtype == VR_DTYPE_BF16;
    size_t numel = 1;
    for (int i = 0; i < ndim; ++i) numel *= (size_t)shape[i];
    const vr_config_t& c = m->c;
    const int D = m->D, F = m->F, E = m->E, I = m->I;
    auto bad_shape = [&]() { return fail(VR_ERR_INVALID, "unexpected shape for %s", name_c); };

    if (name.rfind("llm.lm_head.", 0) == 0 || name.rfind("vpm.attn_pool.", 0) == 0 ||
        name == "resampler.pos_embed" || name.find("rotary_emb") != std::string::npos)
        return VR_OK;

    Staged st;
    VRCHK(stage(data, numel * (bf ? 2 : 4), on_device, st));
    const void* src = st.dev;
    m->finalized = false;

    if (name == "vpm.patch_embed.proj.weight") {
        if (!shape_is(shape, ndim, {D, 3, c.patch_size, c.patch_size})) return bad_shape();
        Linear& L = m->patch;
        if (!L.w.p) { L.n = D; L.k = m->Kpe; L.n_pad = pad128(D); L.k_pad = pad128(m->Kpe); VRCHK(L.w.alloc((size_t)pad256(D) * L.k_pad * 2)); }
        HIPCHK(launch_pack_patch_weight(src, bf, D, c.patch_size, L.w.p, L.k_pad, 0));
        HIPCHK(hipDeviceSynchronize());
        L.has_w = true;
        return VR_OK;
    }
    if (name == "vpm.patch_embed.proj.bias") { if (numel != (size_t)D) return bad_shape(); return load_bias_part(m->patch, D, src, bf, D, 0); }
    if (name == "vpm.pos_embed") {
        if (numel != (size_t)c.vit_pos_grid * c.vit_pos_grid * D) return bad_shape();
        m->has_pos = true;
        m->grids.clear();
        return to_host_f32(src, bf, numel, m->pos_embed_host);
    }
    if (name == "vpm.norm.weight") { if (numel != (size_t)D) return bad_shape(); return load_vec(m->vit_nw, src, bf, D, m->Dp); }
    if (name == "vpm.norm.bias") { if (numel != (size_t)D) return bad_shape(); return load_vec(m->vit_nb, src, bf, D, m->Dp); }
    if (name.rfind("vpm.blocks.", 0) == 0) {
        int n = -1, off = 0;
        if (sscanf(name.c_str(), "vpm.blocks.%d.%n", &n, &off) < 1) return fail(VR_ERR_INVALID, "bad key %s", name_c);
        if (n >= c.vit_depth) return VR_OK;
        const std::string sub = name.substr(off);
        VitBlock& b = m->blocks[n];
        if (sub == "norm1.weight") { if (numel != (size_t)D) return bad_shape(); return load_vec(b.n1w, src, bf, D, m->Dp); }
        if (sub == "norm1.bias") { if (numel != (size_t)D) return bad_shape(); return load_vec(b.n1b, src, bf, D, m->Dp); }
        if (sub == "norm2.weight") { if (numel != (size_t)D) return bad_shape(); return load_vec(b.n2w, src, bf, D, m->Dp); }
        if (sub == "norm2.bias") { if (numel != (size_t)D) return bad_shape(); return load_vec(b.n2b, src, bf, D, m->Dp); }
        if (sub == "attn.qkv.weight") { if (!shape_is(shape, ndim, {3 * D, D})) return bad_shape(); return load_linear_part(b.qkv, 3 * D, D, src, bf, 3 * D, D, 0, 3 * D, 0, 0); }
        if (sub == "attn.qkv.bias") { if (numel != (size_t)3 * D) return bad_shape(); return load_bias_part(b.qkv, 3 * D, src, bf, 3 * D, 0); }
        if (sub == "attn.proj.weight") { if (!shape_is(shape, ndim, {D, D})) return bad_shape(); return load_linear_part(b.proj, D, D, src, bf, D, D, 0, D, 0, 0); }
        if (sub == "attn.proj.bias") { if (numel != (size_t)D) return bad_shape(); return load_bias_part(b.proj, D, src, bf, D, 0); }
        if (sub == "mlp.fc1.weight") { if (!shape_is(shape, ndim, {F, D})) return bad_shape(); return load_linear_part(b.fc1, F, D, src, bf, F, D, 0, F, 0, 0); }
        if (sub == "mlp.fc1.bias") { if (numel != (size_t)F) return bad_shape(); return load_bias_part(b.fc1, F, src, bf, F, 0); }
        if (sub == "mlp.fc2.weight") { if (!shape_is(shape, ndim, {D, F})) return bad_shape(); return load_linear_part(b.fc2, D, F, src, bf, D, F, 0, D, 0, 0); }
        if (sub == "mlp.fc2.bias") { if (numel != (size_t)D) return bad_shape(); return load_bias_part(b.fc2, D, src, bf, D, 0); }
        return fail(VR_ERR_INVALID, "unknown ViT key %s", name_c);
    }
    if (name.rfind("resampler.", 0) == 0) {
        const std::string sub = name.substr(10);
        if (sub == "query") { if (!shape_is(shape, ndim, {m->Q, E})) return bad_shape(); m->has_query = true; return to_host_f32(src, bf, numel, m->r_query_host); }
        if (sub == "kv_proj.weight") { if (!shape_is(shape, ndim, {E, D})) return bad_shape(); return load_linear_part(m->r_kvproj, E, D, src, bf, E, D, 0, E, 0, 0); }
        if (sub == "attn.in_proj_weight") {
            if (!shape_is(shape, ndim, {3 * E, E})) return bad_shape();
            std::vector<float> all;
            VRCHK(to_host_f32(src, bf, (size_t)E * E, all));
            m->r_wq_host.swap(all);
            m->has_inproj = true;
            const char* kv_src = (const char*)src + (size_t)E * E * (bf ? 2 : 4);
            return load_linear_part(m->r_kv, 2 * E, E, kv_src, bf, 2 * E, E, 0, 2 * E, 0, 0);
        }
        if (sub == "attn.in_proj_bias") {
            if (numel != (size_t)3 * E) return bad_shape();
            VRCHK(to_host_f32(src, bf, (size_t)E, m->r_bq_host));
            m->has_inproj_b = true;
            const char* kv_src = (const char*)src + (size_t)E * (bf ? 2 : 4);
            return load_bias_part(m->r_kv, 2 * E, kv_src, bf, 2 * E, 0);
        }
        if (sub == "attn.out_proj.weight") { if (!shape_is(shape, ndim, {E, E})) return bad_shape(); return load_linear_part(m->r_out, E, E, src, bf, E, E, 0, E, 0, 0); }
        if (sub == "attn.out_proj.bias") { if (numel != (size_t)E) return bad_shape(); return load_bias_part(m->r_out, E, src, bf, E, 0); }
        if (sub == "proj") { if (!shape_is(shape, ndim, {E, E})) return bad_shape(); return load_linear_part(m->r_proj, E, E, src, bf, E, E, 1, E, 0, 0); }
        Vec* v = nullptr;
        if (sub == "ln_q.weight") v = &m->r_lnq_w; else if (sub == "ln_q.bias") v = &m->r_lnq_b;
        else if (sub == "ln_kv.weight") v = &m->r_lnkv_w; else if (sub == "ln_kv.bias") v = &m->r_lnkv_b;
        else if (sub == "ln_post.weight") v = &m->r_lnpost_w; else if (sub == "ln_post.bias") v = &m->r_lnpost_b;
        if (!v) return fail(VR_ERR_INVALID, "unknown resampler key %s", name_c);
        if (numel != (size_t)E) return bad_shape();
        return load_vec(*v, src, bf, E, E);
    }
    if (name == "llm.model.embed_tokens.weight") {
        if (!shape_is(shape, ndim, {c.vocab_size, E})) return bad_shape();
        VRCHK(m->embed.alloc(numel * 2));
        HIPCHK(launch_pack_weight(src, bf, c.vocab_size, E, E, 0, m->embed.p, E, c.vocab_size, 0, 0, 0));
        m->has_embed_lo = false;
        if (!bf && c.text_split_precision) {
            VRCHK(m->embed_lo.alloc(numel * 2));
            HIPCHK(launch_pack_weight(src, bf, c.vocab_size, E, E, 0, m->embed_lo.p, E, c.vocab_size, 0, 0, 0, 1));
            m->has_embed_lo = true;
        }
        HIPCHK(hipDeviceSynchronize());
        m->has_embed = true;
        return VR_OK;
    }
    if (name == "llm.model.norm.weight") { if (numel != (size_t)E) return bad_shape(); return load_vec(m->final_norm, src, bf, E, E); }
    if (name.rfind("llm.model.layers.", 0) == 0) {
        int n = -1, off = 0;
        if (sscanf(name.c_str(), "llm.model.layers.%d.%n", &n, &off) < 1) return fail(VR_ERR_INVALID, "bad key %s", name_c);
        if (n >= c.num_layers) return fail(VR_ERR_INVALID, "layer index %d out of range", n);
        const std::string sub = name.substr(off);
// ... 379 lines not shown
```

visrag_amd/csrc/norm.hip:

```cpp
#include "common.h"
#include "gen_math.h"
#include "kernels.h"

namespace vr {

constexpr int NORM_MAXV = 14;
constexpr int NORM_STDV = 10;
constexpr int NORM_VITV = 5;

template <bool RMS, int MAXV = NORM_STDV, int RPW = 1>
__global__ __launch_bounds__(256) void norm_kernel(const float* __restrict__ x, int rows, int dim, int ldx,
                                                   const float* __restrict__ w,
                                                   const float* __restrict__ b, float eps,
                                                   bf16_t* __restrict__ out, int ldo) {
    const int lane = threadIdx.x & 63;
    const int row0 = (blockIdx.x * 4 + (threadIdx.x >> 6)) * RPW;
    if (row0 >= rows) return;
    const int nv = dim >> 2;
    f32x4 v[RPW][MAXV];
    float mu[RPW], rstd[RPW];
#pragma unroll
    for (int r = 0; r < RPW; ++r) {
        const f32x4* xr = reinterpret_cast<const f32x4*>(x + (size_t)min(row0 + r, rows - 1) * ldx);
#pragma unroll
        for (int i = 0; i < MAXV; ++i) {
            const int c = lane + i * 64;
            v[r][i] = (c < nv) ? xr[c] : f32x4{0.f, 0.f, 0.f, 0.f};
        }
    }
#pragma unroll
    for (int r = 0; r < RPW; ++r) {
        float s = 0.f;
#pragma unroll
        for (int i = 0; i < MAXV; ++i) {
            if constexpr (RMS) s += v[r][i][0] * v[r][i][0] + v[r][i][1] * v[r][i][1] + v[r][i][2] * v[r][i][2] + v[r][i][3] * v[r][i][3];
            else s += v[r][i][0] + v[r][i][1] + v[r][i][2] + v[r][i][3];
        }
        s = wave_sum(s);
        mu[r] = 0.f;
        if constexpr (RMS) {
            rstd[r] = rsqrtf(s / dim + eps);
        } else {
            mu[r] = s / dim;
            float q = 0.f;
#pragma unroll
            for (int i = 0; i < MAXV; ++i) {
                const int c = lane + i * 64;
                if (c < nv) {
#pragma unroll
                    for (int e = 0; e < 4; ++e) { const float d = v[r][i][e] - mu[r]; q += d * d; }
                }
            }
            q = wave_sum(q);
            rstd[r] = 1.0f / sqrtf(q / dim + eps);
        }
    }
#pragma unroll
    for (int i = 0; i < MAXV; ++i) {
        const int c = lane + i * 64;
        if (c < nv) {
            const f32x4 ww = reinterpret_cast<const f32x4*>(w)[c];
            f32x4 bb = {0.f, 0.f, 0.f, 0.f};
            if constexpr (!RMS) bb = reinterpret_cast<const f32x4*>(b)[c];
#pragma unroll
            for (int r = 0; r < RPW; ++r) {
                if (row0 + r < rows) {
                    f32x4 y = (v[r][i] - mu[r]) * rstd[r] * ww;
                    if constexpr (!RMS) y += bb;
                    bf16x4 o;
#pragma unroll
                    for (int e = 0; e < 4; ++e) o[e] = f2bf(y[e]);
                    reinterpret_cast<bf16x4*>(out + (size_t)(row0 + r) * ldo)[c] = o;
                }
            }
        } else if (c * 4 < ldo) {
#pragma unroll
            for (int r = 0; r < RPW; ++r)
                if (row0 + r < rows) reinterpret_cast<bf16x4*>(out + (size_t)(row0 + r) * ldo)[c] = bf16x4{(bf16_t)0.f, (bf16_t)0.f, (bf16_t)0.f, (bf16_t)0.f};
        }
    }
}

hipError_t launch_layernorm(const float* x, int rows, int dim, int ldx, const float* w, const float* b,
                            float eps, void* out, int ldo, hipStream_t s) {
    if (rows <= 0) return hipSuccess;
    if (dim % 4 || ldo % 4 || ldx % 4 || ldo > 64 * 4 * NORM_MAXV || dim > ldo || dim > ldx) return hipErrorInvalidValue;
    if (ldo <= 64 * 4 * NORM_VITV)
        hipLaunchKernelGGL((norm_kernel<false, NORM_VITV, 2>), dim3((rows + 7) / 8), dim3(256), 0, s, x, rows, dim, ldx, w, b, eps, (bf16_t*)out, ldo);
    else if (ldo <= 64 * 4 * NORM_STDV)
        hipLaunchKernelGGL((norm_kernel<false, NORM_STDV>), dim3((rows + 3) / 4), dim3(256), 0, s, x, rows, dim, ldx, w, b, eps, (bf16_t*)out, ldo);
    else
        hipLaunchKernelGGL((norm_kernel<false, NORM_MAXV>), dim3((rows + 3) / 4), dim3(256), 0, s, x, rows, dim, ldx, w, b, eps, (bf16_t*)out, ldo);
    return hipGetLastError();
}

hipError_t launch_rmsnorm(const float* x, int rows, int dim, int ldx, const float* w, float eps, void* out,
                          int ldo, hipStream_t s) {
    if (rows <= 0) return hipSuccess;
    if (dim % 4 || ldo % 4 || ldx % 4 || ldo > 64 * 4 * NORM_MAXV || dim > ldo || dim > ldx) return hipErrorInvalidValue;
    if (ldo <= 64 * 4 * NORM_STDV)
        hipLaunchKernelGGL((norm_kernel<true, NORM_STDV>), dim3((rows + 3) / 4), dim3(256), 0, s, x, rows, dim, ldx, w, (const float*)nullptr, eps, (bf16_t*)out, ldo);
    else
        hipLaunchKernelGGL((norm_kernel<true, NORM_MAXV>), dim3((rows + 3) / 4), dim3(256), 0, s, x, rows, dim, ldx, w, (const float*)nullptr, eps, (bf16_t*)out, ldo);
    return hipGetLastError();
}

template <int MAXV>
__global__ __launch_bounds__(256) void rmsnorm_accum_kernel(float* __restrict__ x, int rows, int dim, int ldx,
                                                            const float* __restrict__ partial, int nsplit,
                                                            size_t split_stride, int ldp, float alpha,
                                                            const float* __restrict__ w, float eps,
                                                            bf16_t* __restrict__ out, int ldo) {
    const int lane = threadIdx.x & 63;
    const int row = blockIdx.x * 4 + (threadIdx.x >> 6);
    if (row >= rows) return;
    const int nv = dim >> 2;
    f32x4* xr = reinterpret_cast<f32x4*>(x + (size_t)row * ldx);
    f32x4 v[MAXV];
    float s = 0.f;
#pragma unroll
    for (int i = 0; i < MAXV; ++i) {
        const int c = lane + i * 64;
        if (c < nv) {
            f32x4 acc = reinterpret_cast<const f32x4*>(partial + (size_t)row * ldp)[c];
            for (int sp = 1; sp < nsplit; ++sp)
                acc += reinterpret_cast<const f32x4*>(partial + sp * split_stride + (size_t)row * ldp)[c];
            v[i] = xr[c] + alpha * acc;
            xr[c] = v[i];
        } else {
            v[i] = f32x4{0.f, 0.f, 0.f, 0.f};
        }
        s += v[i][0] * v[i][0] + v[i][1] * v[i][1] + v[i][2] * v[i][2] + v[i][3] * v[i][3];
    }
    if (!out) return;
    s = wave_sum(s);
    const float rstd = rsqrtf(s / dim + eps);
    bf16_t* orow = out + (size_t)row * ldo;
#pragma unroll
    for (int i = 0; i < MAXV; ++i) {
        const int c = lane + i * 64;
        if (c < nv) {
            const f32x4 y = v[i] * rstd * reinterpret_cast<const f32x4*>(w)[c];
            bf16x4 o;
#pragma unroll
            for (int r = 0; r < 4; ++r) o[r] = f2bf(y[r]);
            reinterpret_cast<bf16x4*>(orow)[c] = o;
        } else if (c * 4 < ldo) {
            reinterpret_cast<bf16x4*>(orow)[c] = bf16x4{(bf16_t)0.f, (bf16_t)0.f, (bf16_t)0.f, (bf16_t)0.f};
        }
    }
}

__global__ __launch_bounds__(1024) void rmsnorm_accum_row_kernel(float* __restrict__ x, int dim, int ldx,
                                                                 const float* __restrict__ partial, int nsplit,
                                                                 size_t split_stride, int ldp, float alpha,
                                                                 const float* __restrict__ w, float eps,
                                                                 bf16_t* __restrict__ out, int ldo) {
    __shared__ float red[16];
    const int row = blockIdx.x, c = threadIdx.x, nv = dim >> 2;
    f32x4 v = {0.f, 0.f, 0.f, 0.f};
    if (c < nv) {
        const float* pc = partial + (size_t)row * ldp + (size_t)c * 4;
        f32x4 acc = *reinterpret_cast<const f32x4*>(pc);
        int sp = 1;
        for (; sp + 8 <= nsplit; sp += 8) {
            f32x4 t[8];
#pragma unroll
            for (int i = 0; i < 8; ++i) t[i] = *reinterpret_cast<const f32x4*>(pc + (size_t)(sp + i) * split_stride);
#pragma unroll
            for (int i = 0; i < 8; ++i) acc += t[i];
        }
        for (; sp < nsplit; ++sp) acc += *reinterpret_cast<const f32x4*>(pc + (size_t)sp * split_stride);
        f32x4* xr = reinterpret_cast<f32x4*>(x + (size_t)row * ldx);
        v = xr[c] + alpha * acc;
        xr[c] = v;
    }
    if (!out) return;
    float s = wave_sum(sumsq4(v));
    if ((threadIdx.x & 63) == 0) red[threadIdx.x >> 6] = s;
    __syncthreads();
    float tot = 0.f;
#pragma unroll
    for (int i = 0; i < 16; ++i) tot += red[i];
    const float rstd = rsqrtf(tot / dim + eps);
    bf16_t* orow = out + (size_t)row * ldo;
    if (c < nv) {
        const f32x4 y = v * rstd * reinterpret_cast<const f32x4*>(w)[c];
        bf16x4 o;
#pragma unroll
        for (int r = 0; r < 4; ++r) o[r] = f2bf(y[r]);
        reinterpret_cast<bf16x4*>(orow)[c] = o;
    } else if (c * 4 < ldo) {
        reinterpret_cast<bf16x4*>(orow)[c] = bf16x4{(bf16_t)0.f, (bf16_t)0.f, (bf16_t)0.f, (bf16_t)0.f};
    }
}

hipError_t launch_rmsnorm_accum(float* x, int rows, int dim, int ldx, const float* partial, int nsplit,
                                size_t split_stride, int ldp, float alpha, const float* w, float eps, void* out,
                                int ldo, hipStream_t s) {
    if (rows <= 0) return hipSuccess;
    if (dim % 4 || ldx % 4 || ldp % 4 || dim > 64 * 4 * NORM_MAXV || dim > ldx || dim > ldp || nsplit < 1) return hipErrorInvalidValue;
    if (out && (ldo % 4 || ldo > 64 * 4 * NORM_MAXV || dim > ldo)) return hipErrorInvalidValue;
    if (rows <= 16 && dim <= 4096 && (!out || ldo <= 4096)) {
        hipLaunchKernelGGL(rmsnorm_accum_row_kernel, dim3(rows), dim3(1024), 0, s, x, dim, ldx, partial, nsplit, split_stride, ldp,
                           alpha, w, eps, (bf16_t*)out, ldo);
        return hipGetLastError();
    }
    if (dim <= 64 * 4 * NORM_STDV && (!out || ldo <= 64 * 4 * NORM_STDV))
        hipLaunchKernelGGL(rmsnorm_accum_kernel<NORM_STDV>, dim3((rows + 3) / 4), dim3(256), 0, s, x, rows, dim, ldx, partial, nsplit,
                           split_stride, ldp, alpha, w, eps, (bf16_t*)out, ldo);
    else
        hipLaunchKernelGGL(rmsnorm_accum_kernel<NORM_MAXV>, dim3((rows + 3) / 4), dim3(256), 0, s, x, rows, dim, ldx, partial, nsplit,
                           split_stride, ldp, alpha, w, eps, (bf16_t*)out, ldo);
    return hipGetLastError();
}

}
```

visrag_amd/csrc/ops.hip:

```cpp
#include <hip/hip_runtime.h>

#include <algorithm>
#include <chrono>
#include <cstring>
#include <map>
#include <tuple>
#include <vector>

#include "engine_common.h"

struct ResizeTab { DevBuf bounds, kk; int ksize = 0; };
static std::map<std::tuple<int, int, int>, ResizeTab> g_resize_tabs;

static int get_resize_tab(int dev, int in_size, int out_size, ResizeTab** out) {
    auto key = std::make_tuple(dev, in_size, out_size);
    auto it = g_resize_tabs.find(key);
    if (it == g_resize_tabs.end()) {
        std::vector<int> b, k;
        ResizeTab t;
        t.ksize = resize_coeffs(in_size, out_size, b, k);
        VRCHK(t.bounds.alloc(b.size() * 4));
        VRCHK(t.kk.alloc(k.size() * 4));
        HIPCHK(hipMemcpy(t.bounds.p, b.data(), b.size() * 4, hipMemcpyHostToDevice));
        HIPCHK(hipMemcpy(t.kk.p, k.data(), k.size() * 4, hipMemcpyHostToDevice));
        it = g_resize_tabs.emplace(key, std::move(t)).first;
    }
    *out = &it->second;
    return VR_OK;
}

struct ResizeScratch { DevBuf in, tmp; };
static std::map<std::pair<int, void*>, ResizeScratch> g_resize_scratch;

extern "C" int vr_resize_bicubic(int device_id, const uint8_t* src, int32_t src_on_device, int32_t H, int32_t W,
                                 uint8_t* dst, int32_t out_h, int32_t out_w, void* stream) {
    if (!src || !dst || H <= 0 || W <= 0 || out_h <= 0 || out_w <= 0) return fail(VR_ERR_INVALID, "bad resize arguments");
    VRCHK(set_dev(device_id));
    hipStream_t s = (hipStream_t)stream;
    ResizeScratch& sc = g_resize_scratch[std::make_pair(device_id, stream)];
    const uint8_t* in = src;
    if (!src_on_device) {
        VRCHK(sc.in.reserve((size_t)H * W * 3));
        HIPCHK(hipMemcpyAsync(sc.in.p, src, (size_t)H * W * 3, hipMemcpyHostToDevice, s));
        in = sc.in.as<uint8_t>();
    }
    const bool need_h = out_w != W, need_v = out_h != H;
    if (!need_h && !need_v) {
        HIPCHK(hipMemcpyAsync(dst, in, (size_t)H * W * 3, hipMemcpyDeviceToDevice, s));
    } else {
        const uint8_t* mid = in;
        if (need_h) {
            ResizeTab* th = nullptr;
            VRCHK(get_resize_tab(device_id, W, out_w, &th));
            uint8_t* hout = dst;
            if (need_v) { VRCHK(sc.tmp.reserve((size_t)H * out_w * 3)); hout = sc.tmp.as<uint8_t>(); }
            HIPCHK(launch_resize_h(in, W, H, hout, out_w, th->bounds.as<int>(), th->kk.as<int>(), th->ksize, s));
            mid = hout;
        }
        if (need_v) {
            ResizeTab* tv = nullptr;
            VRCHK(get_resize_tab(device_id, H, out_h, &tv));
            HIPCHK(launch_resize_v(mid, out_w, dst, out_h, tv->bounds.as<int>(), tv->kk.as<int>(), tv->ksize, s));
        }
    }
    if (!src_on_device) HIPCHK(hipStreamSynchronize(s));
    return VR_OK;
}

extern "C" int vr_synth_pages(int device_id, uint8_t* out, int32_t n, int32_t size, int64_t seed, int64_t first, void* stream) {
    if (!out || n < 0 || size < 64 || size > 4096) return fail(VR_ERR_INVALID, "bad synth_pages arguments");
    VRCHK(set_dev(device_id));
    HIPCHK(launch_synth_pages(out, n, size, seed, first, (hipStream_t)stream));
    return VR_OK;
}

__global__ void spin_kernel(long long ticks) {
    const long long t0 = wall_clock64();
    while (wall_clock64() - t0 < ticks) __builtin_amdgcn_s_sleep(8);
}

extern "C" int vr_streams_overlap(int device_id, void* stream_a, void* stream_b, int32_t* overlap) {
    if (!overlap) return fail(VR_ERR_INVALID, "NULL argument");
    VRCHK(set_dev(device_id));
    const hipStream_t a = (hipStream_t)stream_a, b = (hipStream_t)stream_b;
    constexpr int usec = 400;
    int votes = 0;
    for (int rep = 0; rep < 3; ++rep) {
        HIPCHK(hipStreamSynchronize(a));
        HIPCHK(hipStreamSynchronize(b));
        const auto t0 = std::chrono::steady_clock::now();
        hipLaunchKernelGGL(spin_kernel, dim3(1), dim3(1), 0, a, (long long)usec * 100);
        hipLaunchKernelGGL(spin_kernel, dim3(1), dim3(1), 0, b, (long long)usec * 100);
        HIPCHK(hipGetLastError());
        HIPCHK(hipStreamSynchronize(a));
        HIPCHK(hipStreamSynchronize(b));
        const double us = std::chrono::duration<double, std::micro>(std::chrono::steady_clock::now() - t0).count();
        if (rep > 0) votes += us < 1.6 * usec ? 1 : 0;
    }
    *overlap = votes == 2 ? 1 : 0;
    return VR_OK;
}

extern "C" int vr_op_gemm_warm(int device_id, const void* A, int32_t lda, const void* W, int32_t ldw, int32_t M, int32_t N,
                               int32_t K, int32_t epilogue, const float* bias, const float* resid, float alpha, void* out,
                               int32_t ldo, const int32_t* rope_pos, const float* rope_table, int32_t rope_cols,
                               int32_t variant, const vr_gemm_extras_t* extras, const void* warm, uint64_t warm_bytes, void* stream) {
    if (!A || !W || !out) return fail(VR_ERR_INVALID, "NULL argument");
    if (variant != GEMM_VARIANT_GLDS && variant != GEMM_VARIANT_AUTO && variant != GEMM_VARIANT_192 && variant != GEMM_VARIANT_256IL && variant != GEMM_VARIANT_256W && variant != GEMM_VARIANT_192W &&
        variant != GEMM_VARIANT_128W_192 && variant != GEMM_VARIANT_128W_256)
        return fail(VR_ERR_INVALID, "variant %d: 0 (128^2 tile), 3 (auto), 7 (256x192 tile), 9 (256^2 tile), 12 / 13 (256^2 / 256x192 tile, one wave per SIMD), 14 / 15 (128x192 / 128x256 tile, one wave per SIMD)", variant);
    if (((variant == 7 || variant == 13 || variant == 14) ? N % 192 : N % 128) || K % 64 || M <= 0) return fail(VR_ERR_INVALID, "need N %% 128 == 0 (192 for variant 7), K %% 64 == 0");
    if (epilogue == EPI_RESID && !resid) return fail(VR_ERR_INVALID, "EPI_RESID needs resid");
    if (epilogue == EPI_ROPE && (!rope_pos || !rope_table)) return fail(VR_ERR_INVALID, "EPI_ROPE needs tables");
    VRCHK(set_dev(device_id));
    GemmArgs a{};
    a.A = A; a.lda = lda; a.W = W; a.ldw = ldw; a.M = M; a.N = N; a.K = K; a.bias = bias; a.resid = resid;
    a.alpha = alpha; a.out = out; a.ldo = ldo; a.rope_pos = rope_pos; a.rope_table = rope_table; a.rope_cols = rope_cols;
    if (extras) {
        a.rowmap = extras->rowmap;
        a.rowbias = extras->rowbias; a.rowbias_period = extras->rowbias_period; a.rowbias_ld = extras->rowbias_ld; a.rowbias_cols = extras->rowbias_cols;
        a.col_scale = extras->col_scale; a.col_scale_n = extras->col_scale_n;
        a.ksplit = extras->ksplit; a.split_stride = (size_t)extras->split_stride;
        a.m_dev = extras->m_dev; a.m_sub = extras->m_sub;
        a.raster_gm = extras->raster_gm;
    }
    a.warm = warm; a.warm_bytes = (size_t)warm_bytes;
    HIPCHK(launch_gemm(a, epilogue, variant, (hipStream_t)stream));
    return VR_OK;
}

extern "C" int vr_op_gemm_ex(int device_id, const void* A, int32_t lda, const void* W, int32_t ldw, int32_t M, int32_t N,
                             int32_t K, int32_t epilogue, const float* bias, const float* resid, float alpha, void* out,
                             int32_t ldo, const int32_t* rope_pos, const float* rope_table, int32_t rope_cols,
                             int32_t variant, const vr_gemm_extras_t* extras, void* stream) {
    return vr_op_gemm_warm(device_id, A, lda, W, ldw, M, N, K, epilogue, bias, resid, alpha, out, ldo, rope_pos, rope_table, rope_cols,
                           variant, extras, nullptr, 0, stream);
}

extern "C" int vr_op_gemm(int device_id, const void* A, int32_t lda, const void* W, int32_t ldw, int32_t M, int32_t N,
                          int32_t K, int32_t epilogue, const float* bias, const float* resid, float alpha, void* out,
                          int32_t ldo, const int32_t* rope_pos, const float* rope_table, int32_t rope_cols,
                          int32_t variant, void* stream) {
    return vr_op_gemm_ex(device_id, A, lda, W, ldw, M, N, K, epilogue, bias, resid, alpha, out, ldo, rope_pos, rope_table, rope_cols,
                         variant, nullptr, stream);
}

extern "C" int vr_op_norm(int device_id, int32_t kind, const float* x, int32_t rows, int32_t dim, const float* weight,
                          const float* bias, float eps, void* out, int32_t ldo, void* stream) {
    if (!x || !weight || !out || (kind == 0 && !bias)) return fail(VR_ERR_INVALID, "NULL argument");
    VRCHK(set_dev(device_id));
    if (kind == 0) HIPCHK(launch_layernorm(x, rows, dim, dim, weight, bias, eps, out, ldo, (hipStream_t)stream));
    else HIPCHK(launch_rmsnorm(x, rows, dim, dim, weight, eps, out, ldo, (hipStream_t)stream));
    return VR_OK;
}

static AttnArgs attn_args_of(const void* q, int32_t ldq, const void* k, int32_t ldk, const void* v, int32_t ldv, void* out,
                             int32_t ldo, const int32_t* cu_q, const int32_t* cu_kv, int32_t B, int32_t heads, int32_t head_dim,
                             int32_t max_q, int32_t causal, int32_t q_shared, float scale, const vr_attn_extras_t* extras) {
    AttnArgs a{};
    a.q = q; a.ldq = ldq; a.k = k; a.ldk = ldk; a.v = v; a.ldv = ldv; a.out = out; a.ldo = ldo; a.cu_q = cu_q;
    a.cu_kv = cu_kv; a.B = B; a.heads = heads; a.head_dim = head_dim; a.max_q = max_q; a.causal = causal;
    a.q_shared = q_shared; a.scale = scale;
    if (extras) {
        a.kv_group = extras->kv_group; a.kv_end = extras->kv_end; a.q_in_rows = extras->q_in_rows;
        a.q_head_stride = extras->q_head_stride; a.q_prescaled = extras->q_prescaled; a.lse = extras->lse;
    }
    return a;
}

extern "C" int vr_op_attention_ex(int device_id, const void* q, int32_t ldq, const void* k, int32_t ldk, const void* v,
                                  int32_t ldv, void* out, int32_t ldo, const int32_t* cu_q, const int32_t* cu_kv, int32_t B,
                                  int32_t heads, int32_t head_dim, int32_t max_q, int32_t causal, int32_t q_shared,
                                  float scale, const vr_attn_extras_t* extras, void* stream) {
    if (!q || !k || !v || !out || !cu_q || !cu_kv) return fail(VR_ERR_INVALID, "NULL argument");
    VRCHK(set_dev(device_id));
    const AttnArgs a = attn_args_of(q, ldq, k, ldk, v, ldv, out, ldo, cu_q, cu_kv, B, heads, head_dim, max_q, causal, q_shared, scale,
                                    extras);
    HIPCHK(launch_attention(a, (hipStream_t)stream));
    return VR_OK;
}

extern "C" int vr_op_attention_route(int device_id, const void* q, int32_t ldq, const void* k, int32_t ldk, const void* v,
                                     int32_t ldv, void* out, int32_t ldo, const int32_t* cu_q, const int32_t* cu_kv, int32_t B,
                                     int32_t heads, int32_t head_dim, int32_t max_q, int32_t causal, int32_t q_shared,
                                     float scale, const vr_attn_extras_t* extras) {
    (void)device_id;
    if (!q || !k || !v || !out || !cu_q || !cu_kv) return VR_ATTN_ROUTE_REFUSED;
    const AttnRoute r = attention_route(attn_args_of(q, ldq, k, ldk, v, ldv, out, ldo, cu_q, cu_kv, B, heads, head_dim, max_q, causal,
                                                     q_shared, scale, extras));
    switch (r.kind) {
        case ATTN_ROUTE_NONE:  return VR_ATTN_ROUTE_NONE;
        case ATTN_ROUTE_SMALL: return VR_ATTN_ROUTE_SMALL;
        case ATTN_ROUTE_72W:   return VR_ATTN_ROUTE_72W;
        case ATTN_ROUTE_TILED: return VR_ATTN_ROUTE_TILED(r.head_dim, r.qf, r.pipe);
        default:               return VR_ATTN_ROUTE_REFUSED;
    }
}

extern "C" int vr_op_attention(int device_id, const void* q, int32_t ldq, const void* k, int32_t ldk, const void* v,
                               int32_t ldv, void* out, int32_t ldo, const int32_t* cu_q, const int32_t* cu_kv, int32_t B,
                               int32_t heads, int32_t head_dim, int32_t max_q, int32_t causal, int32_t q_shared,
                               float scale, void* stream) {
    return vr_op_attention_ex(device_id, q, ldq, k, ldk, v, ldv, out, ldo, cu_q, cu_kv, B, heads, head_dim, max_q, causal, q_shared,
                              scale, nullptr, stream);
}

extern "C" int vr_op_attn_combine(int device_id, const void* part, const float* lse, int32_t S, const int32_t* S_dev, int32_t heads,
                                  int32_t group, int32_t n_rows, void* out, int32_t ld_out, const void* W, int32_t ldw, int32_t M,
                                  int32_t N, int32_t K, int32_t ksplit, int32_t planes, int32_t ldo, int64_t split_stride, void* stream) {
    if (!part || !lse || !out) return fail(VR_ERR_INVALID, "NULL argument");
    if (heads < 1 || n_rows < 1 || n_rows > 16) return fail(VR_ERR_INVALID, "need heads >= 1 and 1..16 rows");
    if (!S_dev && (S < 1 || S > GEN_ATT_SPLITS)) return fail(VR_ERR_INVALID, "S must be 1..%d", GEN_ATT_SPLITS);
    VRCHK(set_dev(device_id));
    if (!W) {
        if (ld_out < heads * 128 && n_rows > 1) return fail(VR_ERR_INVALID, "ld_out must cover heads * 128");
        HIPCHK(launch_attn_combine(part, lse, S, heads, group, out, (hipStream_t)stream, S_dev, n_rows, ld_out));
        return VR_OK;
    }
    if (n_rows != 1) return fail(VR_ERR_INVALID, "the fused form merges one row");
    if (N < 1 || N % 4 || K < 64 || K % 64 || ldw < K || ldw % 8) return fail(VR_ERR_INVALID, "need N %% 4 == 0, K %% 64 == 0, ldw >= K, ldw %% 8 == 0");
    if (ksplit < 1 || ksplit > planes) return fail(VR_ERR_INVALID, "ksplit must be 1..planes");
    if (ldo < N || ldo % 4 || (ksplit > 1 && (split_stride < (int64_t)(M > 0 ? M : 1) * ldo || split_stride % 4)))
        return fail(VR_ERR_INVALID, "ldo must cover N, split_stride a plane of M x ldo; both multiples of 4");
    if (((uintptr_t)W | (uintptr_t)out) & 15) return fail(VR_ERR_INVALID, "pointers must be 16-byte aligned");
    GemmArgs a{};
    a.A = nullptr; a.lda = K; a.W = W; a.ldw = ldw; a.M = M; a.N = N; a.K = K; a.out = out; a.ldo = ldo;
    a.ksplit = ksplit; a.split_stride = (size_t)split_stride;
    const SkinnyCombine cb{part, lse, S, heads, group, S_dev};
    HIPCHK(launch_gemm_skinny(a, (hipStream_t)stream, false, &cb));
    return VR_OK;
}

extern "C" int vr_op_gemm_skinny(int device_id, const void* A, int32_t lda, const void* W, int32_t ldw, int32_t M, int32_t N,
                                 int32_t K, int32_t ksplit, const float* bias, int32_t swiglu, void* out, int32_t ldo,
                                 int64_t split_stride, void* stream) {
    if (!A || !W || !out) return fail(VR_ERR_INVALID, "NULL argument");
    if (M < 1 || N < 1 || K < 64 || K % 64 || N % 4) return fail(VR_ERR_INVALID, "need M >= 1, N %% 4 == 0, K %% 64 == 0");
    if (M > 32 || (swiglu && M > 16)) return fail(VR_ERR_CAPACITY, "%d rows: at most 32 (16 with swiglu)", M);
    if (ksplit < 1 || ksplit > 64) return fail(VR_ERR_INVALID, "ksplit must be 1..64");
    if (lda < K || ldw < K || lda % 8 || ldw % 8) return fail(VR_ERR_INVALID, "lda / ldw must cover K and be multiples of 8");
    if (((uintptr_t)A | (uintptr_t)W | (uintptr_t)out | (uintptr_t)bias) & 15) return fail(VR_ERR_INVALID, "pointers must be 16-byte aligned");
    if (swiglu) {
        if (ksplit != 1 || N % 32) return fail(VR_ERR_INVALID, "swiglu needs ksplit 1 and N %% 32 == 0");
        if (ldo < N / 2 || ldo % 8) return fail(VR_ERR_INVALID, "swiglu: ldo must cover N / 2 and be a multiple of 8");
    } else {
        if (ldo < N || ldo % 4) return fail(VR_ERR_INVALID, "ldo must cover N and be a multiple of 4");
        if (ksplit > 1 && (split_stride < (int64_t)M * ldo || split_stride % 4)) return fail(VR_ERR_INVALID, "split_stride must cover a plane of M x ldo and be a multiple of 4");
    }
    VRCHK(set_dev(device_id));
    GemmArgs a{};
    a.A = A; a.lda = lda; a.W = W; a.ldw = ldw; a.M = M; a.N = N; a.K = K; a.bias = bias; a.out = out; a.ldo = ldo;
    a.ksplit = ksplit; a.split_stride = (size_t)split_stride;
    HIPCHK(launch_gemm_skinny(a, (hipStream_t)stream, swiglu != 0));
    return VR_OK;
}

extern "C" int vr_op_plane_sum(int device_id, int32_t kind, const float* parts, int32_t nsplit, int64_t split_stride, int32_t ldp,
                               int32_t rows, int32_t dim, float* x, int32_t ldx, float alpha, const float* weight, float eps,
                               void* out, int32_t ldo, void* stream) {
    if (!parts) return fail(VR_ERR_INVALID, "NULL argument");
    if (kind != 0 && kind != 1) return fail(VR_ERR_INVALID, "kind %d: 0 (residual + RMSNorm), 1 (SwiGLU)", kind);
    if (rows < 1 || dim < 1 || nsplit < 1 || nsplit > 64) return fail(VR_ERR_INVALID, "need rows, dim >= 1 and nsplit 1..64");
    if (split_stride % 4 || (nsplit > 1 && split_stride < (int64_t)rows * ldp)) return fail(VR_ERR_INVALID, "split_stride must cover a plane of rows x ldp and be a multiple of 4");
    VRCHK(set_dev(device_id));
    if (kind == 0) {
        if (!x || (out && !weight)) return fail(VR_ERR_INVALID, "NULL argument");
        if (dim > 3584 || (out && ldo > 3584)) return fail(VR_ERR_CAPACITY, "rows of at most 3584 columns");
        if (dim % 4 || ldx % 4 || ldp % 4 || ldx < dim || ldp < dim || (out && (ldo % 4 || ldo < dim)))
            return fail(VR_ERR_INVALID, "dim, ldx, ldp, ldo must be multiples of 4 and the strides cover dim");
        if (((uintptr_t)parts | (uintptr_t)x | (uintptr_t)weight) & 15 || (uintptr_t)out & 7) return fail(VR_ERR_INVALID, "misaligned pointer");
        HIPCHK(launch_rmsnorm_accum(x, rows, dim, ldx, parts, nsplit, (size_t)split_stride, ldp, alpha, weight, eps, out, ldo, (hipStream_t)stream));
    } else {
        if (!out) return fail(VR_ERR_INVALID, "NULL argument");
        if (dim % 16 || ldp < 2 * dim || ldo < dim) return fail(VR_ERR_INVALID, "swiglu: dim %% 16 == 0, ldp >= 2 dim, ldo >= dim");
        HIPCHK(launch_swiglu_sum(parts, nsplit, (size_t)split_stride, ldp, rows, dim, out, ldo, (hipStream_t)stream));
    }
    return VR_OK;
}

static std::map<int, DevBuf> g_chat_op_scratch;

extern "C" int vr_op_chat_attention(int device_id, const void* q, const void* prompt, const void* tails, int32_t layers, int32_t l,
                                    int32_t E, int32_t slots, int32_t max_len, int32_t rows, int32_t max_new, int32_t n,
                                    const int32_t* step_row, const int32_t* step_slot, const int32_t* step_tail,
                                    const int32_t* slot_plen, int32_t force_splits, void* att, void* stream) {
    if (!q || !prompt || !tails || !step_row || !step_slot || !step_tail || !slot_plen || !att) return fail(VR_ERR_INVALID, "NULL argument");
    if (E < 64 || E % 64) return fail(VR_ERR_INVALID, "E must be a multiple of the head dim 64");
    if (layers < 1 || l < 0 || l >= layers) return fail(VR_ERR_INVALID, "layer %d of %d", l, layers);
    if (slots < 1 || max_len < 1 || rows < 1 || max_new < 1) return fail(VR_ERR_INVALID, "bad cache geometry");
    if (force_splits < 0 || force_splits > CHAT_ATT_SPLITS) return fail(VR_ERR_INVALID, "force_splits must be 0..%d", CHAT_ATT_SPLITS);
    if (n < 1) return fail(VR_ERR_INVALID, "n must be positive");
    if (n > CHAT_MAX_ROWS) return fail(VR_ERR_CAPACITY, "%d rows exceed %d", n, CHAT_MAX_ROWS);
    if (((uintptr_t)q | (uintptr_t)prompt | (uintptr_t)tails | (uintptr_t)att) & 15) return fail(VR_ERR_INVALID, "pointers must be 16-byte aligned");
    ChatStep st{};
    st.n = n;
    std::vector<char> used(rows, 0);
    for (int i = 0; i < n; ++i) {
        const int r = step_row[i], sl = step_slot[i], t = step_tail[i];
        if (sl < 0 || sl >= slots || slot_plen[sl] < 1) return fail(VR_ERR_INVALID, "step row %d: slot %d holds no prompt", i, sl);
        if (slot_plen[sl] > max_len) return fail(VR_ERR_CAPACITY, "slot %d: %d prompt keys exceed max_len=%d", sl, slot_plen[sl], max_len);
        if (r < 0 || r >= rows || used[r]) return fail(VR_ERR_INVALID, "step row %d: row %d out of range or repeated", i, r);
        if (t < 0) return fail(VR_ERR_INVALID, "step row %d: negative tail index", i);
        if (t >= max_new) return fail(VR_ERR_CAPACITY, "step row %d: tail index %d exceeds max_new=%d", i, t, max_new);
        used[r] = 1;
        st.row[i] = r; st.slot[i] = sl; st.tail[i] = t; st.pos[i] = slot_plen[sl] + t;
    }
    const int S = chat_step_groups(st, slot_plen, slots, force_splits);
    if (!S) return fail(VR_ERR_INVALID, "the rows of a slot must be adjacent");
    VRCHK(set_dev(device_id));
    hipStream_t s = (hipStream_t)stream;
    const int H = E / 64;
    const size_t po = (size_t)CHAT_MAX_ROWS * H * CHAT_ATT_SPLITS * 64 * 4, pml = (size_t)CHAT_MAX_ROWS * H * CHAT_ATT_SPLITS * 2 * 4;
    DevBuf& sc = g_chat_op_scratch[device_id];
    if (sc.bytes < po + pml) { HIPCHK(hipStreamSynchronize(s)); VRCHK(sc.reserve(po + pml)); }
    const ChatCaps caps{slots, max_len, rows, max_new};
    HIPCHK(launch_chat_attn(st, q, prompt, tails, l, E, H, caps, S, sc.as<float>(), (float*)((char*)sc.p + po), att, s));
    HIPCHK(hipStreamSynchronize(s));
    return VR_OK;
}

extern "C" int vr_op_chat_select(int device_id, int32_t mode, const float* logits, int32_t ld, int32_t V, const uint32_t* seen,
                                 int32_t words, int32_t n_groups, const int32_t* group_offsets, const float* beam_scores, int32_t K,
                                 int32_t kout, float repetition_penalty, float temperature, uint64_t seed, int32_t step,
                                 float* out_scores, int32_t* out_tokens, int32_t* out_parents, void* stream) {
    if (!logits || !seen || !group_offsets || !out_scores || !out_tokens || !out_parents) return fail(VR_ERR_INVALID, "NULL argument");
    if (mode < VR_CHAT_GREEDY || mode > VR_CHAT_SAMPLE) return fail(VR_ERR_INVALID, "mode %d", mode);
    if (V < 1 || ld < V || words < (V + 31) / 32) return fail(VR_ERR_INVALID, "need V >= 1, ld >= V, words >= ceil(V / 32)");
    if (n_groups < 1 || n_groups > CHAT_MAX_ROWS || group_offsets[0] != 0) return fail(VR_ERR_INVALID, "bad groups");
    const int n = group_offsets[n_groups];
    if (n > CHAT_MAX_ROWS) return fail(VR_ERR_CAPACITY, "%d rows exceed %d", n, CHAT_MAX_ROWS);
    if (K < 1 || kout < 1) return fail(VR_ERR_INVALID, "K / kout must be positive");
    if (K > CHAT_TOPK_MAX || kout > CHAT_TOPK_MAX) return fail(VR_ERR_CAPACITY, "K / kout exceed %d", CHAT_TOPK_MAX);
    if (!(repetition_penalty > 0.f)) return fail(VR_ERR_INVALID, "repetition_penalty must be positive");
    if (mode == VR_CHAT_SAMPLE && !(temperature > 0.f)) return fail(VR_ERR_INVALID, "sampling: temperature must be positive");
    ChatSel sel{};
    sel.n = n; sel.groups = n_groups;
    for (int g = 0; g <= n_groups; ++g) sel.g_lo[g] = group_offsets[g];
    for (int g = 0; g < n_groups; ++g) {
        const int nb = group_offsets[g + 1] - group_offsets[g];
        if (nb < 1) return fail(VR_ERR_INVALID, "empty group %d", g);
        if (mode != VR_CHAT_BEAM && nb != 1) return fail(VR_ERR_INVALID, "greedy / sampling groups hold one row");
    }
    for (int i = 0; i < n; ++i) {
        sel.lrow[i] = i; sel.srow[i] = i;
        sel.bscore[i] = mode == VR_CHAT_BEAM && beam_scores ? beam_scores[i] : 0.f;
    }
    VRCHK(set_dev(device_id));
    hipStream_t s = (hipStream_t)stream;
    const size_t b_lse = CHAT_MAX_ROWS * 4, b_part = (size_t)CHAT_MAX_ROWS * CHAT_SEL_WGS * CHAT_TOPK_MAX * 8, b_out = (size_t)CHAT_MAX_ROWS * CHAT_TOPK_MAX * 4;
    DevBuf& sc = g_chat_op_scratch[device_id];
    if (sc.bytes < b_part + b_lse + 3 * b_out) { HIPCHK(hipStreamSynchronize(s)); VRCHK(sc.reserve(b_part + b_lse + 3 * b_out)); }
    unsigned long long* part = sc.as<unsigned long long>();
    float* lse = (float*)((char*)sc.p + b_part);
    float* o_score = (float*)((char*)lse + b_lse);
    int* o_tok = (int*)((char*)o_score + b_out);
    int* o_par = (int*)((char*)o_tok + b_out);
    const int cm = mode == VR_CHAT_BEAM ? CHAT_SEL_BEAM : mode == VR_CHAT_SAMPLE ? CHAT_SEL_SAMPLE : CHAT_SEL_GREEDY;
    HIPCHK(launch_chat_select(sel, cm, logits, ld, V, (const unsigned*)seen, words, repetition_penalty, temperature, K, kout,
                              (unsigned long long)seed, (unsigned)step, lse, part, o_score, o_tok, o_par, s));
    const size_t cnt = (size_t)n_groups * kout;
    HIPCHK(hipMemcpyAsync(out_scores, o_score, cnt * 4, hipMemcpyDeviceToHost, s));
    HIPCHK(hipMemcpyAsync(out_tokens, o_tok, cnt * 4, hipMemcpyDeviceToHost, s));
    HIPCHK(hipMemcpyAsync(out_parents, o_par, cnt * 4, hipMemcpyDeviceToHost, s));
    HIPCHK(hipStreamSynchronize(s));
    return VR_OK;
}

extern "C" int vr_op_chat_sample(int device_id, const float* logits, int32_t ld, int32_t V, const uint32_t* seen, int32_t words, int32_t n,
                                 float repetition_penalty, float temperature, int32_t top_k, double top_p, uint64_t seed, int32_t step,
                                 float* out_scores, int32_t* out_tokens, int32_t* out_kept, int32_t* out_cut, void* stream) {
    if (!logits || !seen || !out_scores || !out_tokens || !out_kept || !out_cut) return fail(VR_ERR_INVALID, "NULL argument");
    if (V < 1 || ld < V || words < (V + 31) / 32) return fail(VR_ERR_INVALID, "need V >= 1, ld >= V, words >= ceil(V / 32)");
    if (n < 1) return fail(VR_ERR_INVALID, "n must be positive");
    if (n > CHAT_MAX_ROWS) return fail(VR_ERR_CAPACITY, "%d rows exceed %d", n, CHAT_MAX_ROWS);
    if (!(repetition_penalty > 0.f)) return fail(VR_ERR_INVALID, "repetition_penalty must be positive");
    if (!(temperature > 0.f)) return fail(VR_ERR_INVALID, "temperature must be positive");
    if (top_k < 0) return fail(VR_ERR_INVALID, "top_k must be 0 (off) or positive");
    if (!(top_p > 0.0 && top_p <= 1.0)) return fail(VR_ERR_INVALID, "top_p must be in (0, 1]");
    ChatSel sel{};
    sel.n = n; sel.groups = n;
    for (int i = 0; i < n; ++i) { sel.lrow[i] = i; sel.srow[i] = i; sel.g_lo[i] = i; }
    sel.g_lo[n] = n;
    VRCHK(set_dev(device_id));
    hipStream_t s = (hipStream_t)stream;
    const size_t b_out = (size_t)4 * CHAT_MAX_ROWS * 4;
    DevBuf& sc = g_chat_op_scratch[device_id];
    if (sc.bytes < b_out) { HIPCHK(hipStreamSynchronize(s)); VRCHK(sc.reserve(b_out)); }
    float* o_score = sc.as<float>();
    int* o_tok = (int*)(o_score + CHAT_MAX_ROWS);
    HIPCHK(launch_chat_sample(sel, logits, ld, V, (const unsigned*)seen, words, repetition_penalty, temperature, top_k, top_p,
                              (unsigned long long)seed, (unsigned)step, o_score, o_tok, o_tok + CHAT_MAX_ROWS, o_tok + 2 * CHAT_MAX_ROWS, s));
    int32_t host[4 * CHAT_MAX_ROWS];
    HIPCHK(hipMemcpyAsync(host, o_score, sizeof(host), hipMemcpyDeviceToHost, s));
    HIPCHK(hipStreamSynchronize(s));
    memcpy(out_scores, host, (size_t)n * 4);
    memcpy(out_tokens, host + CHAT_MAX_ROWS, (size_t)n * 4);
    memcpy(out_kept, host + 2 * CHAT_MAX_ROWS, (size_t)n * 4);
    memcpy(out_cut, host + 3 * CHAT_MAX_ROWS, (size_t)n * 4);
    return VR_OK;
}

extern "C" int vr_op_chat_prompt_scatter(int device_id, const void* qkv, int32_t ld, int32_t E, int32_t B, const int32_t* seq_offsets,
                                         const int32_t* slots, int32_t n_slots, int32_t max_len, void* kplane, void* vplane, void* stream) {
    if (!qkv || !seq_offsets || !slots || !kplane || !vplane) return fail(VR_ERR_INVALID, "NULL argument");
    if (E < 8 || E % 8 || ld % 8 || ld < 3 * E) return fail(VR_ERR_INVALID, "E and ld must be multiples of 8 and ld >= 3 E");
    if (n_slots < 1 || max_len < 1) return fail(VR_ERR_INVALID, "bad cache geometry");
    if (B < 1) return fail(VR_ERR_INVALID, "B must be positive");
    if (B > CHAT_MAX_ROWS || B > n_slots) return fail(VR_ERR_CAPACITY, "%d prompts exceed %d / the %d slots", B, CHAT_MAX_ROWS, n_slots);
    if (((uintptr_t)qkv | (uintptr_t)kplane | (uintptr_t)vplane) & 15) return fail(VR_ERR_INVALID, "pointers must be 16-byte aligned");
    if (seq_offsets[0] != 0) return fail(VR_ERR_INVALID, "seq_offsets[0] must be 0");
    ChatBatch bt{};
    bt.n = B;
    std::vector<char> used(n_slots, 0);
    for (int b = 0; b < B; ++b) {
        const int T = seq_offsets[b + 1] - seq_offsets[b], sl = slots[b];
        if (T < 1) return fail(VR_ERR_INVALID, "empty prompt %d", b);
        if (T > max_len) return fail(VR_ERR_CAPACITY, "prompt %d: %d rows exceed max_len=%d", b, T, max_len);
        if (sl < 0 || sl >= n_slots || used[sl]) return fail(VR_ERR_INVALID, "prompt %d: slot %d out of range or repeated", b, sl);
        used[sl] = 1;
        bt.off[b] = seq_offsets[b]; bt.idx[b] = sl;
    }
    bt.off[B] = seq_offsets[B];
    VRCHK(set_dev(device_id));
    hipStream_t s = (hipStream_t)stream;
    HIPCHK(launch_chat_prompt_scatter(bt, qkv, ld, E, max_len, kplane, vplane, s));
    HIPCHK(hipStreamSynchronize(s));
    return VR_OK;
}

extern "C" int vr_op_norm_ex(int device_id, int32_t kind, const float* x, int32_t rows, int32_t dim, int32_t ldx, const float* weight,
                             const float* bias, float eps, void* out, int32_t ldo, void* stream) {
    if (!x || !weight || !out || (kind == 0 && !bias)) return fail(VR_ERR_INVALID, "NULL argument");
    VRCHK(set_dev(device_id));
    if (kind == 0) HIPCHK(launch_layernorm(x, rows, dim, ldx, weight, bias, eps, out, ldo, (hipStream_t)stream));
    else HIPCHK(launch_rmsnorm(x, rows, dim, ldx, weight, eps, out, ldo, (hipStream_t)stream));
    return VR_OK;
}

extern "C" int vr_op_text_rmsnorm_split(int device_id, const float* x, int32_t rows, int32_t dim, const float* weight, float eps,
                                        void* hi, void* lo, void* stream) {
    if (!x || !weight || !hi || !lo) return fail(VR_ERR_INVALID, "NULL argument");
    VRCHK(set_dev(device_id));
    HIPCHK(launch_rmsnorm_split(x, rows, dim, weight, eps, hi, lo, (hipStream_t)stream));
    return VR_OK;
}

extern "C" int vr_op_text_rope(int device_id, float* qkv, int32_t T, int32_t ld, int32_t rope_cols, const int32_t* pos,
                               const float* table, void* stream) {
    if (!qkv || !pos || !table) return fail(VR_ERR_INVALID, "NULL argument");
    VRCHK(set_dev(device_id));
    HIPCHK(launch_rope_f32(qkv, T, ld, rope_cols, pos, table, (hipStream_t)stream));
    return VR_OK;
}

extern "C" int vr_op_text_attention(int device_id, const float* qkv, int32_t ld, int32_t E, const int32_t* seq_offsets, int32_t B,
                                    int32_t T, int32_t heads, float scale, float* out, void* stream) {
    if (!qkv || !seq_offsets || !out) return fail(VR_ERR_INVALID, "NULL argument");
    VRCHK(set_dev(device_id));
    hipStream_t s = (hipStream_t)stream;
    DevBuf seq_of;
    VRCHK(seq_of.alloc((size_t)(T > 0 ? T : 1) * 4));
    HIPCHK(launch_seq_of(seq_offsets, B, seq_of.as<int>(), s));
    HIPCHK(launch_attn_f32(qkv, ld, E, seq_of.as<int>(), seq_offsets, T, heads, scale, out, s));
    HIPCHK(hipStreamSynchronize(s));
    return VR_OK;
}

extern "C" int vr_op_text_swiglu_split(int device_id, const float* gu, int32_t T, int32_t ld_gu, int32_t I, int32_t ld_act, void* hi,
                                       void* lo, void* stream) {
    if (!gu || !hi || !lo) return fail(VR_ERR_INVALID, "NULL argument");
    VRCHK(set_dev(device_id));
    HIPCHK(launch_swiglu_split(gu, T, ld_gu, I, ld_act, hi, lo, (hipStream_t)stream));
    return VR_OK;
}

extern "C" int vr_op_embed_gather(int device_id, const int32_t* ids, int32_t T, const void* table, const void* table_lo, int32_t dim,
                                  float scale, float* out, void* stream) {
    if (!ids || !table || !out) return fail(VR_ERR_INVALID, "NULL argument");
    VRCHK(set_dev(device_id));
    if (!table_lo) HIPCHK(launch_embed_gather(ids, T, table, dim, scale, out, (hipStream_t)stream));
    else HIPCHK(launch_embed_gather_hp(ids, T, table, table_lo, dim, scale, out, (hipStream_t)stream));
    return VR_OK;
}

extern "C" int vr_op_pool(int device_id, const float* h, const int32_t* seq_offsets, int32_t B, int32_t dim, const float* norm_w,
                          float eps, float* out, float* tap, int32_t mode, void* stream) {
    if (!h || !seq_offsets || !norm_w || !out) return fail(VR_ERR_INVALID, "NULL argument");
    VRCHK(set_dev(device_id));
    HIPCHK(launch_pool(h, seq_offsets, B, dim, norm_w, eps, out, tap, (hipStream_t)stream, mode));
    return VR_OK;
}

extern "C" int vr_op_convert(int device_id, int32_t kind, const void* in, void* out, void* out2, int64_t n, int64_t n_total,
                             int32_t* aux, void* stream) {
    if (kind < 0 || kind > 5) return fail(VR_ERR_INVALID, "kind %d: 0 f32->bf16, 1 f32->bf16 + zero pad, 2 hi/lo split, 3 any non-zero, 4 positions, 5 sequence of a token", kind);
    if (!in || (kind != 3 && !out) || (kind == 2 && !out2) || (kind == 3 && !aux)) return fail(VR_ERR_INVALID, "NULL argument");
    VRCHK(set_dev(device_id));
    hipStream_t s = (hipStream_t)stream;
    switch (kind) {
        case 0: HIPCHK(launch_f32_to_bf16((const float*)in, out, (size_t)n, s)); break;
        case 1: HIPCHK(launch_f32_to_bf16_pad((const float*)in, out, (size_t)n, (size_t)n_total, s, aux)); break;
        case 2: HIPCHK(launch_split_bf16((const float*)in, out, out2, (size_t)n, s)); break;
        case 3: HIPCHK(launch_any_nonzero16(in, (size_t)n, aux, s)); break;
        case 4: HIPCHK(launch_iota_pos((const int*)in, (int)n, (int*)out, s)); break;
        default: HIPCHK(launch_seq_of((const int*)in, (int)n, (int*)out, s)); break;
    }
    return VR_OK;
}

extern "C" int vr_op_planes_sum(int device_id, const float* parts, int32_t n_parts, int64_t stride, int32_t ldp, int32_t T, int32_t N,
                                float* out, int32_t ldo, float alpha, int32_t accumulate, void* stream) {
    if (!parts || !out) return fail(VR_ERR_INVALID, "NULL argument");
    VRCHK(set_dev(device_id));
    HIPCHK(launch_planes_sum(parts, n_parts, (size_t)stride, ldp, T, N, out, ldo, alpha, accumulate != 0, (hipStream_t)stream));
    return VR_OK;
}

extern "C" int vr_op_patch_embed(int device_id, const void* const* imgs, int32_t n, int32_t H, int32_t W, int32_t P, const float* weight,
                                 int32_t D, int32_t K, const float* bias, const float* pos, int32_t ld_pos, float* out, int32_t ldo,
                                 void* stream) {
    if (!imgs || !weight || !bias || !pos || !out) return fail(VR_ERR_INVALID, "NULL argument");
    for (int i = 0; i < n; ++i)
        if (!imgs[i]) return fail(VR_ERR_INVALID, "NULL argument");
    VRCHK(set_dev(device_id));
    hipStream_t s = (hipStream_t)stream;
    const int Kreal = 3 * P * P, patches = P > 0 ? (H / P) * (W / P) : 0;
    DevBuf wp, ptrs;
    VRCHK(wp.alloc((size_t)pad256(D > 0 ? D : 1) * (size_t)std::max(std::max(K, Kreal), 1) * 2));
    VRCHK(ptrs.alloc((size_t)(n > 0 ? n : 1) * sizeof(void*)));
    HIPCHK(launch_pack_patch_weight(weight, 0, D, P, wp.p, K, s));
    if (n > 0) HIPCHK(hipMemcpyAsync(ptrs.p, imgs, (size_t)n * sizeof(void*), hipMemcpyHostToDevice, s));
    GemmArgs a{};
    a.W = wp.p; a.ldw = K; a.M = n * patches; a.N = D; a.K = K; a.bias = bias; a.out = out; a.ldo = ldo; a.alpha = 1.0f;
    a.rowbias = pos; a.rowbias_period = patches; a.rowbias_ld = ld_pos; a.rowbias_cols = D;
    const hipError_t e = launch_patch_embed((const uint8_t* const*)ptrs.p, n, H, W, P, a, Kreal, s);
    HIPCHK(hipStreamSynchronize(s));
    if (e != hipSuccess) return fail(VR_ERR_HIP, "launch_patch_embed(...) failed: %s", hipGetErrorString(e));
    return VR_OK;
}

extern "C" int vr_op_gen_mrope_cache(int device_id, const void* src_bf16, const float* parts, int32_t n_parts, int64_t plane_stride,
                                     const float* bias, int32_t ld, int32_t T, int32_t H, int32_t KV, const int32_t* pos3,
                                     int32_t pos_stride, int32_t sec_t, int32_t sec_h, const float* inv_freq, void* q_out, int32_t ldq,
                                     void* k_cache, void* v_cache, int32_t ld_cache, int32_t cache_row0, const int32_t* row0_dev,
                                     const int32_t* cache_rows, int32_t* cu_kv, void* stream) {
    if ((!src_bf16 && !parts) || !pos3 || !inv_freq || !q_out || !k_cache || !v_cache) return fail(VR_ERR_INVALID, "NULL argument");
    if (T < 1 || H < 1 || KV < 1 || (parts && n_parts < 1)) return fail(VR_ERR_INVALID, "need T, H, KV >= 1 (and n_parts >= 1 with planes)");
    VRCHK(set_dev(device_id));
    HIPCHK(launch_mrope_cache(parts ? nullptr : src_bf16, parts, n_parts, (size_t)plane_stride, bias, ld, T, H, KV, pos3, pos_stride,
                              sec_t, sec_h, inv_freq, q_out, ldq, k_cache, v_cache, ld_cache, cache_row0, cu_kv, (hipStream_t)stream,
                              row0_dev, cache_rows));
    return VR_OK;
}

extern "C" int vr_op_gen_rope2d(int device_id, void* qkv, int32_t ld, int32_t T, int32_t n_slots, int32_t hh, const int32_t* pos_h,
                                const int32_t* pos_w, int32_t sec_h, const float* freq, void* stream) {
    if (!qkv || !pos_h || !pos_w || !freq) return fail(VR_ERR_INVALID, "NULL argument");
    if (T < 1 || n_slots < 1) return fail(VR_ERR_INVALID, "need T, n_slots >= 1");
    VRCHK(set_dev(device_id));
    hipStream_t s = (hipStream_t)stream;
    DevBuf cs;
    VRCHK(cs.alloc((size_t)T * 64 * 8));
    hipError_t e = launch_rope2d_table(pos_h, pos_w, T, sec_h, freq, cs.p, s);
    if (e == hipSuccess) e = launch_rope2d_inplace(qkv, ld, T, n_slots, hh, cs.p, s);
    HIPCHK(hipStreamSynchronize(s));
    if (e != hipSuccess) return fail(VR_ERR_HIP, "launch_rope2d_table / launch_rope2d_inplace(...) failed: %s", hipGetErrorString(e));
    return VR_OK;
}

static_assert(sizeof(GenState) == 42 * 4 && GEN_ATT_SPLITS == 16, "vr_op_gen_sample / vr_op_gen_decode_begin document 42 words");
static std::map<int, DevBuf> g_gen_op_scratch;

extern "C" int vr_op_gen_sample(int device_id, const float* logits, int32_t vocab, uint32_t* seen, float repetition_penalty,
                                float temperature, uint64_t seed, int32_t step, int32_t* state, int32_t step_from_state,
                                int32_t advance, int32_t* out_token, void* stream) {
    if (!logits || !seen || !out_token || ((step_from_state || advance) && !state)) return fail(VR_ERR_INVALID, "NULL argument");
    if (vocab < 1) return fail(VR_ERR_INVALID, "vocab must be positive");
    VRCHK(set_dev(device_id));
    hipStream_t s = (hipStream_t)stream;
    DevBuf& sc = g_gen_op_scratch[device_id];
    if (sc.bytes < 64 * 8 + 16) { HIPCHK(hipStreamSynchronize(s)); VRCHK(sc.reserve(64 * 8 + 16)); }
    int* tok = (int*)((char*)sc.p + 64 * 8);
    HIPCHK(launch_sample(logits, vocab, (unsigned*)seen, repetition_penalty, temperature, (unsigned long long)seed, (unsigned)step, tok,
                         sc.as<unsigned long long>(), s, (GenState*)state, step_from_state, advance));
    HIPCHK(hipMemcpyAsync(out_token, tok, 4, hipMemcpyDeviceToHost, s));
    HIPCHK(hipStreamSynchronize(s));
    return VR_OK;
}

// ... 47 lines not shown
```

Baseline: 756.5 pages/s.

## Reverse tile/row traversal order in selected ViT kernels for cache reuse

Adds a row-order option that makes chosen ViT-stage kernels (LayerNorm, 256W/192W GEMMs, 72W attention) walk their row tiles or work units in reverse. The default library order flips FC2 and the resampler LN-kv, so the next kernel starts on the rows the previous one just wrote, which should still be in L2/MALL instead of being refetched from HBM. It adds a flip flag to the GEMM, norm and attention argument structs and new API entry points. The risk is little gain if the working set already exceeds the cache, plus extra branches in tile-index math.

```diff
diff --git a/include/visrag_hip.h b/include/visrag_hip.h
--- a/include/visrag_hip.h
+++ b/include/visrag_hip.h
@@ -44,7 +44,13 @@
     int32_t max_tokens;
     int32_t max_seqs;
     int32_t text_split_precision;
+    int32_t vit_row_order;
 } vr_config_t;
+#define VR_ROW_ORDER_DEFAULT 0
+#define VR_ROW_ORDER_FORWARD 1
+#define VR_ROW_ORDER_ALTERNATE 2
+#define VR_ROW_ORDER_FC2_LNKV 3
+#define VR_ROW_ORDER_ATTN 4
 
 const char* vr_version(void);
 const char* vr_last_error(void);
@@ -286,6 +292,7 @@
     const int32_t* m_dev;
     int32_t m_sub;
     int32_t raster_gm;
+    int32_t row_flip;
 } vr_gemm_extras_t;
 int vr_op_gemm_ex(int device_id, const void* A, int32_t lda, const void* W, int32_t ldw,
                   int32_t M, int32_t N, int32_t K, int32_t epilogue, const float* bias,
@@ -297,11 +304,15 @@
                     const float* resid, float alpha, void* out, int32_t ldo,
                     const int32_t* rope_pos, const float* rope_table, int32_t rope_cols,
                     int32_t variant, const vr_gemm_extras_t* extras, const void* warm, uint64_t warm_bytes, void* stream);
+int vr_op_gemm_route(int32_t lda, int32_t ldw, int32_t M, int32_t N, int32_t K, int32_t epilogue, int32_t ldo,
+                     const vr_gemm_extras_t* extras);
 int vr_op_norm(int device_id, int32_t kind, const float* x, int32_t rows, int32_t dim,
                const float* weight, const float* bias, float eps, void* out, int32_t ldo,
                void* stream);
 int vr_op_norm_ex(int device_id, int32_t kind, const float* x, int32_t rows, int32_t dim, int32_t ldx, const float* weight,
                   const float* bias, float eps, void* out, int32_t ldo, void* stream);
+int vr_op_norm_flip(int device_id, int32_t kind, const float* x, int32_t rows, int32_t dim, int32_t ldx, const float* weight,
+                    const float* bias, float eps, void* out, int32_t ldo, int32_t flip, void* stream);
 
 int vr_op_text_rmsnorm_split(int device_id, const float* x, int32_t rows, int32_t dim, const float* weight, float eps, void* hi,
                              void* lo, void* stream);
@@ -340,6 +351,11 @@
                        const int32_t* cu_q, const int32_t* cu_kv, int32_t B, int32_t heads,
                        int32_t head_dim, int32_t max_q, int32_t causal, int32_t q_shared,
                        float scale, const vr_attn_extras_t* extras, void* stream);
+int vr_op_attention_flip(int device_id, const void* q, int32_t ldq, const void* k, int32_t ldk,
+                         const void* v, int32_t ldv, void* out, int32_t ldo,
+                         const int32_t* cu_q, const int32_t* cu_kv, int32_t B, int32_t heads,
+                         int32_t head_dim, int32_t max_q, int32_t causal, int32_t q_shared,
+                         float scale, const vr_attn_extras_t* extras, int32_t unit_flip, void* stream);
 #define VR_ATTN_ROUTE_REFUSED (-1)
 #define VR_ATTN_ROUTE_NONE 0
 #define VR_ATTN_ROUTE_SMALL 1
diff --git a/visrag_amd/_lib.py b/visrag_amd/_lib.py
--- a/visrag_amd/_lib.py
+++ b/visrag_amd/_lib.py
@@ -19,7 +19,7 @@
         ("intermediate_size", C.c_int32), ("vocab_size", C.c_int32), ("rms_norm_eps", C.c_float),
         ("rope_theta", C.c_float), ("scale_emb", C.c_float), ("residual_scale", C.c_float),
         ("max_images", C.c_int32), ("max_patches", C.c_int32), ("max_tokens", C.c_int32),
-        ("max_seqs", C.c_int32), ("text_split_precision", C.c_int32),
+        ("max_seqs", C.c_int32), ("text_split_precision", C.c_int32), ("vit_row_order", C.c_int32),
     ]
 
 
@@ -48,7 +48,8 @@
 class VRGemmExtras(C.Structure):
     _fields_ = [("rowmap", C.c_void_p), ("rowbias", C.c_void_p), ("rowbias_period", C.c_int32), ("rowbias_ld", C.c_int32),
                 ("rowbias_cols", C.c_int32), ("col_scale", C.c_float), ("col_scale_n", C.c_int32), ("ksplit", C.c_int32),
-                ("split_stride", C.c_int64), ("m_dev", C.c_void_p), ("m_sub", C.c_int32), ("raster_gm", C.c_int32)]
+                ("split_stride", C.c_int64), ("m_dev", C.c_void_p), ("m_sub", C.c_int32), ("raster_gm", C.c_int32),
+                ("row_flip", C.c_int32)]
 
 
 class VRAttnExtras(C.Structure):
@@ -140,7 +141,9 @@
     "vr_op_gemm_warm": (C.c_int, [C.c_int, _vp, _i32, _vp, _i32, _i32, _i32, _i32, _i32, _vp, _vp, _f32,
                                   _vp, _i32, _vp, _vp, _i32, _i32, C.POINTER(VRGemmExtras), _vp, C.c_uint64, _vp]),
     "vr_op_norm": (C.c_int, [C.c_int, _i32, _vp, _i32, _i32, _vp, _vp, _f32, _vp, _i32, _vp]),
+    "vr_op_gemm_route": (C.c_int, [_i32, _i32, _i32, _i32, _i32, _i32, _i32, C.POINTER(VRGemmExtras)]),
     "vr_op_norm_ex": (C.c_int, [C.c_int, _i32, _vp, _i32, _i32, _i32, _vp, _vp, _f32, _vp, _i32, _vp]),
+    "vr_op_norm_flip": (C.c_int, [C.c_int, _i32, _vp, _i32, _i32, _i32, _vp, _vp, _f32, _vp, _i32, _i32, _vp]),
     "vr_op_text_rmsnorm_split": (C.c_int, [C.c_int, _vp, _i32, _i32, _vp, _f32, _vp, _vp, _vp]),
     "vr_op_text_rope": (C.c_int, [C.c_int, _vp, _i32, _i32, _i32, _vp, _vp, _vp]),
     "vr_op_text_attention": (C.c_int, [C.c_int, _vp, _i32, _i32, _vp, _i32, _i32, _i32, _f32, _vp, _vp]),
@@ -154,6 +157,8 @@
                                   _i32, _i32, _i32, _i32, _i32, _f32, _vp]),
     "vr_op_attention_ex": (C.c_int, [C.c_int, _vp, _i32, _vp, _i32, _vp, _i32, _vp, _i32, _vp, _vp, _i32,
                                      _i32, _i32, _i32, _i32, _i32, _f32, C.POINTER(VRAttnExtras), _vp]),
+    "vr_op_attention_flip": (C.c_int, [C.c_int, _vp, _i32, _vp, _i32, _vp, _i32, _vp, _i32, _vp, _vp, _i32,
+                                       _i32, _i32, _i32, _i32, _i32, _f32, C.POINTER(VRAttnExtras), _i32, _vp]),
     "vr_op_attention_route": (C.c_int, [C.c_int, _vp, _i32, _vp, _i32, _vp, _i32, _vp, _i32, _vp, _vp, _i32,
                                         _i32, _i32, _i32, _i32, _i32, _f32, C.POINTER(VRAttnExtras)]),
     "vr_op_attn_combine": (C.c_int, [C.c_int, _vp, _vp, _i32, _vp, _i32, _i32, _i32, _vp, _i32, _vp, _i32, _i32, _i32, _i32, _i32,
@@ -251,4 +256,5 @@
         vocab_size=cfg.vocab_size, rms_norm_eps=cfg.rms_norm_eps, rope_theta=cfg.rope_theta,
         scale_emb=cfg.scale_emb, residual_scale=cfg.residual_scale, max_images=max_images,
         max_patches=max_patches, max_tokens=max_tokens, max_seqs=max_seqs,
-        text_split_precision=int(getattr(cfg, "text_split_precision", True)))
+        text_split_precision=int(getattr(cfg, "text_split_precision", True)),
+        vit_row_order=int(getattr(cfg, "vit_row_order", 0)))
diff --git a/visrag_amd/config.py b/visrag_amd/config.py
--- a/visrag_amd/config.py
+++ b/visrag_amd/config.py
@@ -26,6 +26,7 @@
     max_slice_nums: int = 9
     slice_mode: bool = True
     text_split_precision: int = True
+    vit_row_order: int = 0
     pooling: str = "wmean"
 
     @property
diff --git a/visrag_amd/csrc/attention.hip b/visrag_amd/csrc/attention.hip
--- a/visrag_amd/csrc/attention.hip
+++ b/visrag_amd/csrc/attention.hip
@@ -41,6 +41,7 @@
     const AttnRoute r = attention_route(a_in);
     if (r.kind == ATTN_ROUTE_NONE) return hipSuccess;
     if (r.kind == ATTN_ROUTE_REFUSED) return hipErrorInvalidValue;
+    if (a_in.unit_flip && r.kind != ATTN_ROUTE_72W) return hipErrorInvalidValue;
     AttnArgs a = a_in;
     if (a.q_prescaled && r.kind != ATTN_ROUTE_72W) a.scale = 1.0f / 1.44269504088896340736f;
     if (r.kind == ATTN_ROUTE_SMALL) return launch_attention_small(a, s);
diff --git a/visrag_amd/csrc/attention_w.hip b/visrag_amd/csrc/attention_w.hip
--- a/visrag_amd/csrc/attention_w.hip
+++ b/visrag_amd/csrc/attention_w.hip
@@ -154,7 +154,8 @@
     auto get_unit = [&](int u) -> Unit {
         Unit x{u, 0, 0, 0, 0, 0, 0, 0, 0};
         if (u >= total) return x;
-        const int qt = u % q_tiles, bh = u / q_tiles, b = bh / p.heads;
+        const int lu = p.unit_flip ? total - 1 - u : u;
+        const int qt = lu % q_tiles, bh = lu / q_tiles, b = bh / p.heads;
         x.h = bh % p.heads;
         x.kv0 = p.cu_kv[b]; x.kv_len = p.cu_kv[b + 1] - x.kv0;
         x.q_row0 = p.cu_q[b]; x.q_len = p.cu_q[b + 1] - x.q_row0;
diff --git a/visrag_amd/csrc/encode.hip b/visrag_amd/csrc/encode.hip
--- a/visrag_amd/csrc/encode.hip
+++ b/visrag_amd/csrc/encode.hip
@@ -7,6 +7,9 @@
 
 #include "model.h"
 
+#ifndef VR_ROW_ORDER_LIBRARY
+#define VR_ROW_ORDER_LIBRARY VR_ROW_ORDER_FC2_LNKV
+#endif
 static int run_vision_group(vr_model_s* m, const uint8_t* const* dev_imgs_hostarray, int n, int H, int W,
                             const int32_t* rowmap_host , bool first_group, hipStream_t s) {
     const vr_config_t& c = m->c;
@@ -24,6 +27,20 @@
     const int* cu_tok = m->w_cu.as<int>();
     const int* cu_qry = m->w_cu.as<int>() + (n + 1);
 
+    const int order = c.vit_row_order != VR_ROW_ORDER_DEFAULT ? c.vit_row_order : VR_ROW_ORDER_LIBRARY;
+    enum Site { S_OTHER, S_ATTN, S_FC2, S_LNKV };
+    bool flip = false;
+    auto turn = [&](Site site = S_OTHER) {
+        flip = order == VR_ROW_ORDER_ALTERNATE ? !flip
+             : order == VR_ROW_ORDER_FC2_LNKV ? (site == S_FC2 || site == S_LNKV)
+             : order == VR_ROW_ORDER_ATTN ? site == S_ATTN : false;
+        return flip;
+    };
+    auto gemm_flip = [&](GemmArgs& a, int epi, bool f) {
+        if (!f) return;
+        const int v = gemm_auto_variant(a, epi);
+        if (v == GEMM_VARIANT_256W || v == GEMM_VARIANT_192W) a.row_flip = 1;
+    };
     float* h = m->w_hvit.as<float>();
     {
         GemmArgs a = gemm_args(nullptr, 0, m->patch, M, h, Dp);
@@ -37,11 +54,12 @@
     const float vit_qscale = (1.0f / sqrtf((float)vit_hd)) * 1.44269504088896340736f;
     for (int l = 0; l < c.vit_depth; ++l) {
         const VitBlock& b = m->blocks[l];
-        HIPCHK(launch_layernorm(h, M, D, Dp, b.n1w.v.as<float>(), b.n1b.v.as<float>(), c.vit_ln_eps, m->w_xn.p, Dp, s));
+        HIPCHK(launch_layernorm(h, M, D, Dp, b.n1w.v.as<float>(), b.n1b.v.as<float>(), c.vit_ln_eps, m->w_xn.p, Dp, s, turn()));
         VRCHK(prof_begin(m, VR_PROF_VIT_QKV, s));
         {
             GemmArgs a = gemm_args(m->w_xn.p, Dp, b.qkv, M, m->w_qkv.p, ldqkv);
             a.col_scale = vit_qscale; a.col_scale_n = vit_qscale_n;
+            gemm_flip(a, EPI_BF16, turn());
             HIPCHK(launch_gemm(a, EPI_BF16, GEMM_VARIANT_AUTO, s));
         }
         VRCHK(prof_end(m, VR_PROF_VIT_QKV, 2.0 * M * D * 3 * D, s));
@@ -52,6 +70,7 @@
             a.v = (const char*)m->w_qkv.p + (size_t)2 * D * 2; a.ldv = ldqkv;
             a.out = m->w_att.p; a.ldo = Dp; a.cu_q = cu_tok; a.cu_kv = cu_tok; a.B = n; a.heads = c.vit_heads;
             a.head_dim = vit_hd; a.max_q = N; a.causal = 0; a.q_shared = 0; a.scale = 1.0f / sqrtf((float)vit_hd); a.q_prescaled = vit_qscale_n > 0;
+            a.unit_flip = turn(S_ATTN) && attention_route(a).kind == ATTN_ROUTE_72W;
             VRCHK(prof_begin(m, VR_PROF_VIT_ATTN, s));
             HIPCHK(launch_attention(a, s));
             VRCHK(prof_end(m, VR_PROF_VIT_ATTN, 4.0 * n * (double)N * N * D, s));
@@ -59,31 +78,34 @@
         VRCHK(prof_begin(m, VR_PROF_VIT_PROJ, s));
         {
             GemmArgs a = gemm_args(m->w_att.p, Dp, b.proj, M, h, Dp); a.resid = h;
+            gemm_flip(a, EPI_RESID, turn());
             HIPCHK(launch_gemm(a, EPI_RESID, GEMM_VARIANT_AUTO, s));
         }
         VRCHK(prof_end(m, VR_PROF_VIT_PROJ, 2.0 * M * D * D, s));
-        HIPCHK(launch_layernorm(h, M, D, Dp, b.n2w.v.as<float>(), b.n2b.v.as<float>(), c.vit_ln_eps, m->w_xn.p, Dp, s));
+        HIPCHK(launch_layernorm(h, M, D, Dp, b.n2w.v.as<float>(), b.n2b.v.as<float>(), c.vit_ln_eps, m->w_xn.p, Dp, s, turn()));
         VRCHK(prof_begin(m, VR_PROF_VIT_FC1, s));
-        { GemmArgs a = gemm_args(m->w_xn.p, Dp, b.fc1, M, m->w_mlp.p, m->Fp); HIPCHK(launch_gemm(a, EPI_GELU, GEMM_VARIANT_AUTO, s)); }
+        { GemmArgs a = gemm_args(m->w_xn.p, Dp, b.fc1, M, m->w_mlp.p, m->Fp); gemm_flip(a, EPI_GELU, turn()); HIPCHK(launch_gemm(a, EPI_GELU, GEMM_VARIANT_AUTO, s)); }
         VRCHK(prof_end(m, VR_PROF_VIT_FC1, 2.0 * M * D * m->F, s));
         VRCHK(prof_begin(m, VR_PROF_VIT_FC2, s));
         {
             GemmArgs a = gemm_args(m->w_mlp.p, m->Fp, b.fc2, M, h, Dp); a.resid = h;
+            gemm_flip(a, EPI_RESID, turn(S_FC2));
             HIPCHK(launch_gemm(a, EPI_RESID, GEMM_VARIANT_AUTO, s));
         }
         VRCHK(prof_end(m, VR_PROF_VIT_FC2, 2.0 * M * D * m->F, s));
         if (l == 0 && first_group) VRCHK(tap_store(m, "vit_block0", h, N, D, Dp, false, s));
     }
-    HIPCHK(launch_layernorm(h, M, D, Dp, m->vit_nw.v.as<float>(), m->vit_nb.v.as<float>(), c.vit_ln_eps, m->w_xn.p, Dp, s));
+    HIPCHK(launch_layernorm(h, M, D, Dp, m->vit_nw.v.as<float>(), m->vit_nb.v.as<float>(), c.vit_ln_eps, m->w_xn.p, Dp, s, turn()));
     if (first_group) VRCHK(tap_store(m, "vit_out", m->w_xn.p, N, D, Dp, true, s));
 
     VRCHK(prof_begin(m, VR_PROF_RESAMPLER, s));
-    { GemmArgs a = gemm_args(m->w_xn.p, Dp, m->r_kvproj, M, m->w_kv32.p, E); HIPCHK(launch_gemm(a, EPI_F32, GEMM_VARIANT_AUTO, s)); }
+    { GemmArgs a = gemm_args(m->w_xn.p, Dp, m->r_kvproj, M, m->w_kv32.p, E); gemm_flip(a, EPI_F32, turn()); HIPCHK(launch_gemm(a, EPI_F32, GEMM_VARIANT_AUTO, s)); }
     HIPCHK(launch_layernorm(m->w_kv32.as<float>(), M, E, E, m->r_lnkv_w.v.as<float>(), m->r_lnkv_b.v.as<float>(),
-                            c.resampler_ln_eps, m->w_xkv.p, E, s));
+                            c.resampler_ln_eps, m->w_xkv.p, E, s, turn(S_LNKV)));
     {
         GemmArgs a = gemm_args(m->w_xkv.p, E, m->r_kv, M, m->w_KV.p, 2 * E);
         a.rowbias = g->pos_k.as<float>(); a.rowbias_period = N; a.rowbias_ld = E; a.rowbias_cols = E;
+        gemm_flip(a, EPI_BF16, turn());
         HIPCHK(launch_gemm(a, EPI_BF16, GEMM_VARIANT_AUTO, s));
     }
     {
diff --git a/visrag_amd/csrc/gemm.hip b/visrag_amd/csrc/gemm.hip
--- a/visrag_amd/csrc/gemm.hip
+++ b/visrag_amd/csrc/gemm.hip
@@ -125,6 +125,7 @@
     if (a.ksplit > 1 && (!split_tile || epi != EPI_F32 || a.K % (a.ksplit * GEMM_BK) || a.rowmap || a.rowbias)) return true;
     if (a.m_dev && variant != GEMM_VARIANT_256IL) return true;
     if (a.warm && a.warm_bytes && (variant != GEMM_VARIANT_256W || a.warm_bytes >= WARM_MAX_BYTES)) return true;
+    if (a.row_flip && variant != GEMM_VARIANT_256W && variant != GEMM_VARIANT_192W) return true;
     return false;
 }
 
diff --git a/visrag_amd/csrc/gemm256w_kernel.h b/visrag_amd/csrc/gemm256w_kernel.h
--- a/visrag_amd/csrc/gemm256w_kernel.h
+++ b/visrag_amd/csrc/gemm256w_kernel.h
@@ -30,7 +30,8 @@
         const int gsz = GM * tiles_n;
         const int g = t / gsz, r = t % gsz;
         const int gm = min(GM, tiles_m - g * GM);
-        m0 = __builtin_amdgcn_readfirstlane((g * GM + r % gm) * G256_BM);
+        const int mt = g * GM + r % gm;
+        m0 = __builtin_amdgcn_readfirstlane((p.row_flip ? tiles_m - 1 - mt : mt) * G256_BM);
         n0 = __builtin_amdgcn_readfirstlane((r / gm) * BN);
         split = __builtin_amdgcn_readfirstlane(split);
     };
diff --git a/visrag_amd/csrc/kernels.h b/visrag_amd/csrc/kernels.h
--- a/visrag_amd/csrc/kernels.h
+++ b/visrag_amd/csrc/kernels.h
@@ -30,6 +30,7 @@
     float col_scale; int col_scale_n;
     const int* m_dev; int m_sub;
     const void* warm; size_t warm_bytes;
+    int row_flip;
 };
 hipError_t launch_gemm(const GemmArgs& a, int epilogue, int variant, hipStream_t s);
 bool gemm_args_refused(const GemmArgs& a, int epilogue, int variant);
@@ -47,7 +48,7 @@
                              hipStream_t s);
 
 hipError_t launch_layernorm(const float* x, int rows, int dim, int ldx, const float* w, const float* b,
-                            float eps, void* out, int ldo, hipStream_t s);
+                            float eps, void* out, int ldo, hipStream_t s, bool flip = false);
 hipError_t launch_rmsnorm_accum(float* x, int rows, int dim, int ldx, const float* partial, int nsplit,
                                 size_t split_stride, int ldp, float alpha, const float* w, float eps, void* out,
                                 int ldo, hipStream_t s);
@@ -70,6 +71,7 @@
     int q_head_stride;
     int q_prescaled;
     float* lse;
+    int unit_flip;
 };
 hipError_t launch_attention(const AttnArgs& a, hipStream_t s);
 enum AttnRouteKind { ATTN_ROUTE_REFUSED = -1, ATTN_ROUTE_NONE = 0, ATTN_ROUTE_SMALL = 1, ATTN_ROUTE_72W = 2, ATTN_ROUTE_TILED = 3 };
diff --git a/visrag_amd/csrc/model.hip b/visrag_amd/csrc/model.hip
--- a/visrag_amd/csrc/model.hip
+++ b/visrag_amd/csrc/model.hip
@@ -28,6 +28,7 @@
     if (c.vit_dim % 4 || c.hidden_size > 2560 || c.vit_dim > 2560) return fail(VR_ERR_INVALID, "dims out of range");
     if (c.max_images <= 0 || c.max_patches <= 0 || c.max_tokens <= 0 || c.max_seqs <= 0)
         return fail(VR_ERR_INVALID, "workspace limits must be positive");
+    if (c.vit_row_order < VR_ROW_ORDER_DEFAULT || c.vit_row_order > VR_ROW_ORDER_ATTN) return fail(VR_ERR_INVALID, "vit_row_order %d: VR_ROW_ORDER_*", c.vit_row_order);
     VRCHK(set_dev(device_id));
     vr_model_s* m = new vr_model_s();
     m->device = device_id;
diff --git a/visrag_amd/csrc/norm.hip b/visrag_amd/csrc/norm.hip
--- a/visrag_amd/csrc/norm.hip
+++ b/visrag_amd/csrc/norm.hip
@@ -12,9 +12,9 @@
 __global__ __launch_bounds__(256) void norm_kernel(const float* __restrict__ x, int rows, int dim, int ldx,
                                                    const float* __restrict__ w,
                                                    const float* __restrict__ b, float eps,
-                                                   bf16_t* __restrict__ out, int ldo) {
+                                                   bf16_t* __restrict__ out, int ldo, int flip) {
     const int lane = threadIdx.x & 63;
-    const int row0 = (blockIdx.x * 4 + (threadIdx.x >> 6)) * RPW;
+    const int row0 = ((flip ? gridDim.x - 1 - blockIdx.x : blockIdx.x) * 4 + (threadIdx.x >> 6)) * RPW;
     if (row0 >= rows) return;
     const int nv = dim >> 2;
     f32x4 v[RPW][MAXV];
@@ -82,15 +82,15 @@
 }
 
 hipError_t launch_layernorm(const float* x, int rows, int dim, int ldx, const float* w, const float* b,
-                            float eps, void* out, int ldo, hipStream_t s) {
+                            float eps, void* out, int ldo, hipStream_t s, bool flip) {
     if (rows <= 0) return hipSuccess;
     if (dim % 4 || ldo % 4 || ldx % 4 || ldo > 64 * 4 * NORM_MAXV || dim > ldo || dim > ldx) return hipErrorInvalidValue;
     if (ldo <= 64 * 4 * NORM_VITV)
-        hipLaunchKernelGGL((norm_kernel<false, NORM_VITV, 2>), dim3((rows + 7) / 8), dim3(256), 0, s, x, rows, dim, ldx, w, b, eps, (bf16_t*)out, ldo);
+        hipLaunchKernelGGL((norm_kernel<false, NORM_VITV, 2>), dim3((rows + 7) / 8), dim3(256), 0, s, x, rows, dim, ldx, w, b, eps, (bf16_t*)out, ldo, (int)flip);
     else if (ldo <= 64 * 4 * NORM_STDV)
-        hipLaunchKernelGGL((norm_kernel<false, NORM_STDV>), dim3((rows + 3) / 4), dim3(256), 0, s, x, rows, dim, ldx, w, b, eps, (bf16_t*)out, ldo);
+        hipLaunchKernelGGL((norm_kernel<false, NORM_STDV>), dim3((rows + 3) / 4), dim3(256), 0, s, x, rows, dim, ldx, w, b, eps, (bf16_t*)out, ldo, (int)flip);
     else
-        hipLaunchKernelGGL((norm_kernel<false, NORM_MAXV>), dim3((rows + 3) / 4), dim3(256), 0, s, x, rows, dim, ldx, w, b, eps, (bf16_t*)out, ldo);
+        hipLaunchKernelGGL((norm_kernel<false, NORM_MAXV>), dim3((rows + 3) / 4), dim3(256), 0, s, x, rows, dim, ldx, w, b, eps, (bf16_t*)out, ldo, (int)flip);
     return hipGetLastError();
 }
 
@@ -99,9 +99,9 @@
     if (rows <= 0) return hipSuccess;
     if (dim % 4 || ldo % 4 || ldx % 4 || ldo > 64 * 4 * NORM_MAXV || dim > ldo || dim > ldx) return hipErrorInvalidValue;
     if (ldo <= 64 * 4 * NORM_STDV)
-        hipLaunchKernelGGL((norm_kernel<true, NORM_STDV>), dim3((rows + 3) / 4), dim3(256), 0, s, x, rows, dim, ldx, w, (const float*)nullptr, eps, (bf16_t*)out, ldo);
+        hipLaunchKernelGGL((norm_kernel<true, NORM_STDV>), dim3((rows + 3) / 4), dim3(256), 0, s, x, rows, dim, ldx, w, (const float*)nullptr, eps, (bf16_t*)out, ldo, 0);
     else
-        hipLaunchKernelGGL((norm_kernel<true, NORM_MAXV>), dim3((rows + 3) / 4), dim3(256), 0, s, x, rows, dim, ldx, w, (const float*)nullptr, eps, (bf16_t*)out, ldo);
+        hipLaunchKernelGGL((norm_kernel<true, NORM_MAXV>), dim3((rows + 3) / 4), dim3(256), 0, s, x, rows, dim, ldx, w, (const float*)nullptr, eps, (bf16_t*)out, ldo, 0);
     return hipGetLastError();
 }
 
diff --git a/visrag_amd/csrc/ops.hip b/visrag_amd/csrc/ops.hip
--- a/visrag_amd/csrc/ops.hip
+++ b/visrag_amd/csrc/ops.hip
@@ -123,10 +123,19 @@
         a.ksplit = extras->ksplit; a.split_stride = (size_t)extras->split_stride;
         a.m_dev = extras->m_dev; a.m_sub = extras->m_sub;
         a.raster_gm = extras->raster_gm;
+        a.row_flip = extras->row_flip;
     }
     a.warm = warm; a.warm_bytes = (size_t)warm_bytes;
     HIPCHK(launch_gemm(a, epilogue, variant, (hipStream_t)stream));
     return VR_OK;
+}
+
+extern "C" int vr_op_gemm_route(int32_t lda, int32_t ldw, int32_t M, int32_t N, int32_t K, int32_t epilogue, int32_t ldo,
+                                const vr_gemm_extras_t* extras) {
+    GemmArgs a{};
+    a.lda = lda; a.ldw = ldw; a.M = M; a.N = N; a.K = K; a.ldo = ldo;
+    if (extras) { a.rowmap = extras->rowmap; a.rowbias = extras->rowbias; a.rowbias_ld = extras->rowbias_ld; }
+    return gemm_auto_variant(a, epilogue);
 }
 
 extern "C" int vr_op_gemm_ex(int device_id, const void* A, int32_t lda, const void* W, int32_t ldw, int32_t M, int32_t N,
@@ -168,16 +177,24 @@
     return a;
 }
 
+extern "C" int vr_op_attention_flip(int device_id, const void* q, int32_t ldq, const void* k, int32_t ldk, const void* v,
+                                    int32_t ldv, void* out, int32_t ldo, const int32_t* cu_q, const int32_t* cu_kv, int32_t B,
+                                    int32_t heads, int32_t head_dim, int32_t max_q, int32_t causal, int32_t q_shared,
+                                    float scale, const vr_attn_extras_t* extras, int32_t unit_flip, void* stream) {
+    if (!q || !k || !v || !out || !cu_q || !cu_kv) return fail(VR_ERR_INVALID, "NULL argument");
+    VRCHK(set_dev(device_id));
+    AttnArgs a = attn_args_of(q, ldq, k, ldk, v, ldv, out, ldo, cu_q, cu_kv, B, heads, head_dim, max_q, causal, q_shared, scale, extras);
+    a.unit_flip = unit_flip != 0;
+    HIPCHK(launch_attention(a, (hipStream_t)stream));
+    return VR_OK;
+}
+
 extern "C" int vr_op_attention_ex(int device_id, const void* q, int32_t ldq, const void* k, int32_t ldk, const void* v,
                                   int32_t ldv, void* out, int32_t ldo, const int32_t* cu_q, const int32_t* cu_kv, int32_t B,
                                   int32_t heads, int32_t head_dim, int32_t max_q, int32_t causal, int32_t q_shared,
                                   float scale, const vr_attn_extras_t* extras, void* stream) {
-    if (!q || !k || !v || !out || !cu_q || !cu_kv) return fail(VR_ERR_INVALID, "NULL argument");
-    VRCHK(set_dev(device_id));
-    const AttnArgs a = attn_args_of(q, ldq, k, ldk, v, ldv, out, ldo, cu_q, cu_kv, B, heads, head_dim, max_q, causal, q_shared, scale,
-                                    extras);
-    HIPCHK(launch_attention(a, (hipStream_t)stream));
-    return VR_OK;
+    return vr_op_attention_flip(device_id, q, ldq, k, ldk, v, ldv, out, ldo, cu_q, cu_kv, B, heads, head_dim, max_q, causal, q_shared,
+                                scale, extras, 0, stream);
 }
 
 extern "C" int vr_op_attention_route(int device_id, const void* q, int32_t ldq, const void* k, int32_t ldk, const void* v,
@@ -428,13 +445,19 @@
     return VR_OK;
 }
 
+extern "C" int vr_op_norm_flip(int device_id, int32_t kind, const float* x, int32_t rows, int32_t dim, int32_t ldx, const float* weight,
+                               const float* bias, float eps, void* out, int32_t ldo, int32_t flip, void* stream) {
+    if (!x || !weight || !out || (kind == 0 && !bias)) return fail(VR_ERR_INVALID, "NULL argument");
+    if (kind != 0 && flip) return fail(VR_ERR_INVALID, "only the LayerNorm (kind 0) walks its rows backwards");
+    VRCHK(set_dev(device_id));
+    if (kind == 0) HIPCHK(launch_layernorm(x, rows, dim, ldx, weight, bias, eps, out, ldo, (hipStream_t)stream, flip != 0));
+    else HIPCHK(launch_rmsnorm(x, rows, dim, ldx, weight, eps, out, ldo, (hipStream_t)stream));
+    return VR_OK;
+}
+
 extern "C" int vr_op_norm_ex(int device_id, int32_t kind, const float* x, int32_t rows, int32_t dim, int32_t ldx, const float* weight,
                              const float* bias, float eps, void* out, int32_t ldo, void* stream) {
-    if (!x || !weight || !out || (kind == 0 && !bias)) return fail(VR_ERR_INVALID, "NULL argument");
-    VRCHK(set_dev(device_id));
-    if (kind == 0) HIPCHK(launch_layernorm(x, rows, dim, ldx, weight, bias, eps, out, ldo, (hipStream_t)stream));
-    else HIPCHK(launch_rmsnorm(x, rows, dim, ldx, weight, eps, out, ldo, (hipStream_t)stream));
-    return VR_OK;
+    return vr_op_norm_flip(device_id, kind, x, rows, dim, ldx, weight, bias, eps, out, ldo, 0, stream);
 }
 
 extern "C" int vr_op_text_rmsnorm_split(int device_id, const float* x, int32_t rows, int32_t dim, const float* weight, float eps,
```

New measurement: 762.2 pages/s (median of 6 runs). Within noise of the previous version (+0.8%).
